# OpenDriveLab/kai0

Measured on AMD Instinct MI355X. Metric: train samples/sec pi0.5 full FT, higher is better.
Workload: dtype bf16; 1 GPU; pi0.5 full fine-tune bf16, batch 32 per MI355X, 3-cam 224x224 (BASELINE.json configs[1]); global_batch=32, seq_len=1018, parallelism=dp1

## Files before the change

### kai0_amd/csrc/gemm_bf16.hip

```cpp
#include "common.h"
#include "../../include/kai0hip.h"
#include <stdlib.h>
#include <algorithm>
#include <atomic>
#include <type_traits>

namespace {

constexpr int BK = 64;

#ifdef KAI0_ABLATE
#define KAI0_ABL(p) ((p).ablate)
#else
#define KAI0_ABL(p) 0
#endif

struct RowMap {
    int32_t rpb;
    int64_t bs, off;
    __device__ __forceinline__ int64_t operator()(int r) const {
        if (rpb == 0) return r;
        const int q = r / rpb;
        return (int64_t)q * bs + (r - q * rpb) + off;
    }
// ... 304 lines not shown
            if constexpr (A_KC) {
                off = kc_in ? a_off[j] + (uint32_t)k0 * 2 : OOB;
            } else {
                const int kr = k0 + (wave * NA + j) * A_RPP + lane / A_LPR;
                off = kr < kend ? a_off[j] + (uint32_t)p.amap(kr) * lda2 : OOB;
            }
            glds16(a_rsrc, off, sa + j * 1024);
        }
#pragma unroll
        for (int j = 0; j < NB; ++j) {
            uint32_t off;
            if constexpr (B_KC) {
                off = kc_in ? b_off[j] + (uint32_t)k0 * 2 : OOB;
            } else {
                const int kr = k0 + (wave * NB + j) * B_RPP + lane / B_LPR;
                off = kr < kend ? b_off[j] + (uint32_t)p.bmap(kr) * ldb2 : OOB;
            }
            glds16((B_KC && BK == 64 && pair && (((wave * NB + j) * KC_RPP) & 32)) ? b2_rsrc : b_rsrc, off, sb + j * 1024);
        }
    };

    auto piece_off = [&](int kt, int idx) -> uint32_t {
        const int k0 = kbeg + kt * BK;
        const bool kc_in = (k0 + kc_chunk) < kend;
        if (idx < NA) {
            if constexpr (A_KC) {
                return kc_in ? a_off[idx] + (uint32_t)k0 * 2 : OOB;
            } else {
                const int kr = k0 + (wave * NA + idx) * A_RPP + lane / A_LPR;
                return kr < kend ? a_off[idx] + (uint32_t)p.amap(kr) * lda2 : OOB;
            }
        } else {
            const int j = idx - NA;
            if constexpr (B_KC) {
                return kc_in ? b_off[j] + (uint32_t)k0 * 2 : OOB;
            } else {
                const int kr = k0 + (wave * NB + j) * B_RPP + lane / B_LPR;
                return kr < kend ? b_off[j] + (uint32_t)p.bmap(kr) * ldb2 : OOB;
            }
        }
    };
    auto piece_issue = [&](uint32_t off, int slot, int idx) {
        if (idx < NA) glds16(a_rsrc, off, smem + slot * STAGE + wave * (NA * 1024) + idx * 1024);
        else glds16(b_rsrc, off, smem + slot * STAGE + A_TILE + wave * (NB * 1024) + (idx - NA) * 1024);
    };

    const int l15 = lane & 15, g = lane >> 4;
    const int mc_keyv = (l15 >> 2) | ((g & 1) << 2);

    f32x4 acc[MT][NT];
#pragma unroll
    for (int i = 0; i < MT; ++i)
#pragma unroll
        for (int j = 0; j < NT; ++j) acc[i][j] = f32x4{0.f, 0.f, 0.f, 0.f};

    auto load_frag = [&](const char* tile, bool kc, int rowb, int col0, int ks) -> bf16x8 {
        if (kc) {
            const int row = col0 + l15;
            const int off = BK == 64 ? row * 128 + (((ks * 4 + g) ^ (row & 7)) << 4)
                                     : row * 64 + ((g ^ ((row & 8) ? 3 : 0)) << 4);
            return *reinterpret_cast<const bf16x8*>(tile + off);
        } else {
            const int chunk = (col0 >> 3) + ((l15 & 3) >> 1);
            const int sw = ((chunk ^ (mc_keyv << 1)) << 4) + (l15 & 1) * 8;
            const int r0 = ks * 32 + 8 * g + (l15 >> 2);
            bf16x4 lo = __builtin_amdgcn_ds_read_tr16_b64_v4bf16((LDS_PTR(bf16x4))(tile + r0 * rowb + sw));
            bf16x4 hi = __builtin_amdgcn_ds_read_tr16_b64_v4bf16((LDS_PTR(bf16x4))(tile + (r0 + 4) * rowb + sw));
            return __builtin_shufflevector(lo, hi, 0, 1, 2, 3, 4, 5, 6, 7);
        }
    };

    const int nk = (kend - kbeg + BK - 1) / BK;
    if constexpr (SCH == 3) {
        constexpr int NP = NA + NB;
        static_assert(NP == 4 && BK == 32, "ring schedule: 4 pieces per 32-deep sub-tile");
        const int grp = wm;
#pragma unroll
        for (int u = 0; u < 3; ++u)
#pragma unroll
            for (int pi = 0; pi < NP; ++pi) piece_issue(piece_off(u, pi), u, pi);
        asm volatile("s_waitcnt vmcnt(8)" ::: "memory");
        lds_barrier();
        if (grp == 1) lds_barrier();
        for (int u = 0; u < nk; ++u) {
            const int slot = u & 3, pslot = (u + 3) & 3;
            const char* ta = smem + slot * STAGE;
            const char* tb = ta + A_TILE;
            bf16x8 bfr[NT], af[MT];
#pragma unroll
            for (int t = 0; t < NT; ++t) bfr[t] = load_frag(tb, B_KC, B_ROWB, wn * (NT * 16) + t * 16, 0);
#pragma unroll
            for (int t = 0; t < MT; ++t) af[t] = load_frag(ta, A_KC, A_ROWB, wm * (MT * 16) + t * 16, 0);
            __builtin_amdgcn_sched_barrier(0);
            if (grp == 1) asm volatile("s_waitcnt vmcnt(4)" ::: "memory");
            lds_barrier();
            __builtin_amdgcn_s_setprio(1);
#pragma unroll
            for (int i = 0; i < MT; ++i) {
#pragma unroll
                for (int j = 0; j < NT; ++j)
                    acc[i][j] = __builtin_amdgcn_mfma_f32_16x16x32_bf16(af[i], bfr[j], acc[i][j], 0, 0, 0);
                if ((i & 1) == 0) {
                    __builtin_amdgcn_sched_barrier(0);
                    piece_issue(KAI0_ABL(p) == 1 ? OOB : piece_off(u + 3, i >> 1), pslot, i >> 1);
                    __builtin_amdgcn_sched_barrier(0);
                }
            }
            __builtin_amdgcn_s_setprio(0);
            if (grp == 0) asm volatile("s_waitcnt vmcnt(8)" ::: "memory");
            lds_barrier();
        }
        asm volatile("s_waitcnt vmcnt(0)" ::: "memory");
        if (grp == 0) lds_barrier();
        lds_barrier();
    } else if constexpr (SCH == 1) {
        const int grp = wm;
        uint32_t ha_off[4], hb_off[4];
        int ha_lds[4], hb_lds[4];
        int ha_kr[4], hb_kr[4];
#pragma unroll
        for (int h = 0; h < 2; ++h)
#pragma unroll
            for (int j = 0; j < 2; ++j) {
                const int q = 2 * wave + j, x = h * 2 + j;
                if constexpr (A_KC) {
                    const int ra = (q >> 3) * 128 + h * 64 + (q & 7) * 8, Ra = m0 + ra + (lane >> 3);
                    ha_lds[x] = ra * 128;
                    ha_kr[x] = 0;
                    ha_off[x] = Ra < p.M ? (uint32_t)((p.amap(Ra) * p.lda + kc_chunk) * 2) : OOB;
                } else {
                    const int r = q * 4 + (lane >> 4), key = (r & 3) | (((r >> 3) & 1) << 2);
                    const int col = m0 + h * 128 + (((lane & 15) ^ (key << 1)) * 8);
                    ha_lds[x] = h * 16384 + q * 1024;
                    ha_kr[x] = r;
                    ha_off[x] = col < p.M ? (uint32_t)(col * 2) : OOB;
                }
                if constexpr (B_KC) {
                    const int rb = (q >> 2) * 64 + h * 32 + (q & 3) * 8;
                    int Rb = n0 + rb + (lane >> 3);
                    bool ok = Rb < p.N;
                    if (pair) {
                        Rb = (n0 >> 1) + (q >> 2) * 32 + (q & 3) * 8 + (lane >> 3);
                        ok = Rb < (p.N >> 1);
                    }
                    hb_lds[x] = rb * 128;
                    hb_kr[x] = 0;
                    hb_off[x] = ok ? (uint32_t)((p.bmap(Rb) * p.ldb + kc_chunk) * 2) : OOB;
                } else {
                    const int r = q * 4 + (lane >> 4), key = (r & 3) | (((r >> 3) & 1) << 2);
                    const int col = n0 + h * 128 + (((lane & 15) ^ (key << 1)) * 8);
                    hb_lds[x] = h * 16384 + q * 1024;
                    hb_kr[x] = r;
                    hb_off[x] = col < p.N ? (uint32_t)(col * 2) : OOB;
                }
            }
        auto issue_half = [&](bool isb, int h, int t) {
            const int k0 = kbeg + t * BK;
            const bool kc_in = (k0 + kc_chunk) < kend;
            char* base = smem + (t & 1) * STAGE + (isb ? A_TILE : 0);
#pragma unroll
            for (int j = 0; j < 2; ++j) {
                const int x = h * 2 + j;
                const uint32_t o = isb ? hb_off[x] : ha_off[x];
                uint32_t off = OOB;
                if (isb ? B_KC : A_KC) {
                    if (kc_in && o != OOB) off = o + (uint32_t)k0 * 2;
                } else {
                    const int kr = k0 + (isb ? hb_kr[x] : ha_kr[x]);
                    if (kr < kend && o != OOB) off = o + (uint32_t)(isb ? p.bmap(kr) : p.amap(kr)) * (isb ? ldb2 : lda2);
                }
                if (KAI0_ABL(p) == 1) off = OOB;
                glds16(isb ? ((pair && h == 1) ? b2_rsrc : b_rsrc) : a_rsrc, off, base + (isb ? hb_lds[x] : ha_lds[x]));
            }
        };
        issue_half(false, 0, 0);
        issue_half(true, 1, 0);
        issue_half(true, 0, 0);
        issue_half(false, 1, 0);
        issue_half(false, 0, 1);
        issue_half(true, 1, 1);
        asm volatile("s_waitcnt vmcnt(6)" ::: "memory");
        lds_barrier();
        if (grp == 1) lds_barrier();
        bf16x8 af[4][2], bq[2][2];
        auto read_a = [&](const char* ta, int h) {
#pragma unroll
            for (int i = 0; i < 4; ++i)
#pragma unroll
                for (int ks = 0; ks < 2; ++ks)
                    af[i][ks] = A_KC ? load_frag(ta, true, A_ROWB, wm * 128 + (h * 4 + i) * 16, ks)
                                     : load_frag(ta + h * 16384, false, 256, wm * 64 + i * 16, ks);
        };
        auto read_b = [&](const char* tb, int h) {
#pragma unroll
            for (int j = 0; j < 2; ++j)
#pragma unroll
                for (int ks = 0; ks < 2; ++ks)
                    bq[j][ks] = B_KC ? load_frag(tb, true, B_ROWB, wn * 64 + (h * 2 + j) * 16, ks)
                                     : load_frag(tb + h * 16384, false, 256, wn * 32 + j * 16, ks);
        };
        auto quad = [&](auto ahc, auto bhc) {
            constexpr int ah = decltype(ahc)::value, bh = decltype(bhc)::value;
            __builtin_amdgcn_s_setprio(1);
#pragma unroll
            for (int ks = 0; ks < 2; ++ks)
#pragma unroll
                for (int i = 0; i < 4; ++i)
#pragma unroll
                    for (int j = 0; j < 2; ++j)
                        acc[ah * 4 + i][bh * 2 + j] =
                            __builtin_amdgcn_mfma_f32_16x16x32_bf16(af[i][ks], bq[j][ks], acc[ah * 4 + i][bh * 2 + j], 0, 0, 0);
            __builtin_amdgcn_s_setprio(0);
        };
        using I0 = std::integral_constant<int, 0>;
        using I1 = std::integral_constant<int, 1>;
        for (int t = 0; t < nk; ++t) {
            const char* ta = smem + (t & 1) * STAGE;
            const char* tb = ta + A_TILE;
            read_b(tb, 0);
            __builtin_amdgcn_sched_barrier(0);
            read_a(ta, 0);
            __builtin_amdgcn_sched_barrier(0);
            issue_half(true, 0, t + 1);
            lds_barrier();
            quad(I0{}, I0{});
            lds_barrier();
            read_b(tb, 1);
            __builtin_amdgcn_sched_barrier(0);
            issue_half(false, 1, t + 1);
            asm volatile("s_waitcnt vmcnt(8)" ::: "memory");
            lds_barrier();
            quad(I0{}, I1{});
            lds_barrier();
            read_a(ta, 1);
            __builtin_amdgcn_sched_barrier(0);
            issue_half(false, 0, t + 2);
            lds_barrier();
            quad(I1{}, I1{});
            lds_barrier();
            read_b(tb, 0);
            __builtin_amdgcn_sched_barrier(0);
            issue_half(true, 1, t + 2);
            asm volatile("s_waitcnt vmcnt(6)" ::: "memory");
            lds_barrier();
            quad(I1{}, I0{});
            lds_barrier();
        }
        asm volatile("s_waitcnt vmcnt(0)" ::: "memory");
        if (grp == 0) lds_barrier();
        lds_barrier();
    } else {
#pragma unroll
        for (int st = 0; st < NS - 1; ++st)
            if (st < nk) stage(st, st);
        int slot_c = 0, slot_p = NS - 1;
        for (int kt = 0; kt < nk; ++kt) {
            if constexpr (NS == 2) {
                asm volatile("s_waitcnt vmcnt(0)" ::: "memory");
            } else {
                if (kt + NS - 2 < nk) asm volatile("s_waitcnt vmcnt(%0)" ::"n"((NS - 2) * (NA + NB)) : "memory");
                else asm volatile("s_waitcnt vmcnt(0)" ::: "memory");
            }
            lds_barrier();
            if (kt + NS - 1 < nk && KAI0_ABL(p) != 1) stage(kt + NS - 1, slot_p);
            const char* ta = smem + slot_c * STAGE;
            const char* tb = ta + A_TILE;
    #pragma unroll
            for (int ks = 0; ks < BK / 32; ++ks) {
                bf16x8 bfr[NT];
    #pragma unroll
                for (int t = 0; t < NT; ++t) bfr[t] = load_frag(tb, B_KC, B_ROWB, wn * (NT * 16) + t * 16, ks);
    #pragma unroll
                for (int h = 0; h < MT / AH; ++h) {
                    bf16x8 af[AH];
    #pragma unroll
                    for (int t = 0; t < AH; ++t) af[t] = load_frag(ta, A_KC, A_ROWB, wm * (MT * 16) + (h * AH + t) * 16, ks);
    #pragma unroll
                    for (int i = 0; i < AH; ++i)
    #pragma unroll
                        for (int j = 0; j < NT; ++j)
                            acc[h * AH + i][j] = __builtin_amdgcn_mfma_f32_16x16x32_bf16(af[i], bfr[j], acc[h * AH + i][j], 0, 0, 0);
                }
            }
            slot_c = slot_c + 1 == NS ? 0 : slot_c + 1;
            slot_p = slot_p + 1 == NS ? 0 : slot_p + 1;
        }
        lds_barrier();
    }

    float* slab = reinterpret_cast<float*>(smem + wave * (AH * 4096));
    const int64_t cz = z1 * p.sC1 + z2 * p.sC2;
    const int64_t rz = z1 * p.sR1 + z2 * p.sR2;
    const int64_t vz = z1 * p.rv_s1 + z2 * p.rv_s2;
    constexpr bool ILM = SCH == 1 && !A_KC, ILN = SCH == 1 && !B_KC;
    const int ccol = ILN ? n0 + ((lane & 7) >> 2) * 128 + wn * 32 + ((lane & 7) & 3) * 8 : n0 + wn * 64 + (lane & 7) * 8;
    auto row_base = [&](int h) { return ILM ? m0 + h * 128 + wm * 64 : m0 + wm * (MT * 16) + h * 64; };
    const bool col_ok = ccol < ((p.N + 7) & ~7);
    const bool fused_fast = p.act >= 2 && p.split_k == 1 && p.bias == nullptr && p.gate == nullptr && p.residual == nullptr &&
                            !p.accumulate && !p.out_f32 && p.nseg == 0 && (p.act == 4 || p.scale == 1.0f) &&
                            (p.act != 3 || p.pre_out != nullptr);
    const bool plain_fast = p.act <= 1 && p.split_k == 1 && (p.bias != nullptr || p.residual != nullptr) && p.gate == nullptr &&
                            !p.accumulate && !p.out_f32 && p.nseg == 0 && (N_ALIGNED8(p.N));
    const bool simple_fast = MT == 8 && p.simple_epi && p.act <= 1 && p.split_k == 1 && p.gate == nullptr && !p.out_f32 && p.scale == 1.0f &&
                             p.cmap.rpb == 0 && (N_ALIGNED8(p.N));
    auto epi_half = [&](auto hc) {
        constexpr int h = decltype(hc)::value;
        if constexpr (((MT == 4 && WM == 2) || (MT == 2 && WM == 4)) && WN == 2 && A_KC && B_KC) if (p.act == 7) {
            const bool rot = n0 < p.rope_n_end;
            const int fi = ((n0 >> 7) & 1) * 64 + (lane & 7) * 8;
            const int rcol = rot ? (n0 >> 8) * 256 + wn * 128 + fi : n0 + wn * 64 + (lane & 7) * 8;
            const int rbase = row_base(h) + (lane >> 3);
            bf16x8 cs[AH * 2], sn[AH * 2];
#pragma unroll
            for (int it = 0; it < AH * 2; ++it) {
                const int64_t tr = (int64_t)min(rbase + it * 8, p.M - 1) * p.rope_half + fi;
                cs[it] = *reinterpret_cast<const bf16x8*>(p.rope_cos + (rot ? tr : 0));
                sn[it] = *reinterpret_cast<const bf16x8*>(p.rope_sin + (rot ? tr : 0));
            }
#pragma unroll
            for (int i = 0; i < AH; ++i)
#pragma unroll
                for (int j = 0; j < 4; ++j)
#pragma unroll
                    for (int r = 0; r < 4; ++r) slab[(i * 16 + 4 * g + r) * 64 + j * 16 + l15] = acc[i][j][r];
            lds_barrier();
            const float* pslab = reinterpret_cast<const float*>(smem + (wave ^ 1) * (AH * 4096));
            int si = 0;
            if (p.nseg > 1 && rcol >= p.seg_begin[1]) si = 1;
            if (p.nseg > 2 && rcol >= p.seg_begin[2]) si = 2;
            const bool rcol_ok = rcol < p.N;
#pragma unroll
            for (int it = 0; it < AH * 2; ++it) {
                const int lr = it * 8 + (lane >> 3);
                const int row = rbase + it * 8;
                const int so = lr * 64 + (lane & 7) * 8;
                const f32x4 v0 = *reinterpret_cast<const f32x4*>(slab + so), v1 = *reinterpret_cast<const f32x4*>(slab + so + 4);
                const f32x4 w0 = *reinterpret_cast<const f32x4*>(pslab + so), w1 = *reinterpret_cast<const f32x4*>(pslab + so + 4);
                if (row >= p.M || !rcol_ok) continue;
                const float x[8] = {v0[0], v0[1], v0[2], v0[3], v1[0], v1[1], v1[2], v1[3]};
                const float y[8] = {w0[0], w0[1], w0[2], w0[3], w1[0], w1[1], w1[2], w1[3]};
                bf16x8 ov;
#pragma unroll
                for (int e = 0; e < 8; ++e) {
                    const float xe = rbf(x[e]), ye = rbf(y[e]);
                    const float c = bf2f(cs[it][e]), sv = bf2f(sn[it][e]);
                    ov[e] = rot ? f2bf(rbf(xe * c) + rbf((wn == 0 ? -ye : ye) * sv)) : f2bf(xe);
                }
                const int64_t orow = p.cmap(row);
                bf16_t* cp = p.nseg > 0 ? p.seg_dst[si] + orow * p.seg_ld[si] + (rcol - p.seg_begin[si])
                                        : reinterpret_cast<bf16_t*>(p.C) + cz + orow * p.ldc + rcol;
                *reinterpret_cast<bf16x8*>(cp) = ov;
            }
            return;
        }
        if constexpr (MT != 2) if (pair) {
#pragma unroll
            for (int i = 0; i < 4; ++i)
#pragma unroll
                for (int j = 0; j < 4; ++j)
#pragma unroll
                    for (int r = 0; r < 4; ++r) slab[(i * 16 + 4 * g + r) * 64 + j * 16 + l15] = acc[h * 4 + i][j][r];
            asm volatile("s_waitcnt lgkmcnt(0)" ::: "memory");
            __builtin_amdgcn_wave_barrier();
            const int ocol = (n0 >> 1) + wn * 32 + (lane & 3) * 8;
            const bool ocol_ok = ocol < (p.N >> 1);
            bf16_t* cb = reinterpret_cast<bf16_t*>(p.C);
#pragma unroll
            for (int it = 0; it < 4; ++it) {
                const int lr = it * 16 + (lane >> 2);
                const int row = row_base(h) + lr;
                const float* sp = slab + lr * 64 + (lane & 3) * 8;
                const f32x4 g0 = *reinterpret_cast<const f32x4*>(sp), g1 = *reinterpret_cast<const f32x4*>(sp + 4);
                const f32x4 u0 = *reinterpret_cast<const f32x4*>(sp + 32), u1 = *reinterpret_cast<const f32x4*>(sp + 36);
                if (row >= p.M || !ocol_ok) continue;
                const float gv[8] = {g0[0], g0[1], g0[2], g0[3], g1[0], g1[1], g1[2], g1[3]};
                const float uv[8] = {u0[0], u0[1], u0[2], u0[3], u1[0], u1[1], u1[2], u1[3]};
                bf16x8 gb, ub, hb;
#pragma unroll
                for (int e = 0; e < 8; e += 2) {
                    const f32x2 gr = rbf2(f32x2{gv[e], gv[e + 1]}), ur = rbf2(f32x2{uv[e], uv[e + 1]});
                    const f32x2 hv = rbf2(gelu_tanh2(gr)) * ur;
                    gb[e] = f2bf(gr[0]);
                    gb[e + 1] = f2bf(gr[1]);
                    ub[e] = f2bf(ur[0]);
                    ub[e + 1] = f2bf(ur[1]);
                    hb[e] = f2bf(hv[0]);
                    hb[e + 1] = f2bf(hv[1]);
                }
                const int64_t o = cz + p.cmap(row) * p.ldc + ocol;
                *reinterpret_cast<bf16x8*>(cb + o) = hb;
                if (p.pre_out != nullptr) store_pre8(p.pre_out + o, gb, p.nt_pre);
                if (p.pre_out2 != nullptr) store_pre8(p.pre_out2 + o, ub, p.nt_pre);
            }
            asm volatile("s_waitcnt lgkmcnt(0)" ::: "memory");
            __builtin_amdgcn_wave_barrier();
            return;
        }
        if constexpr (MT != 2) if (fused_fast) {
            bf16x8 s0[8], s1[8];
            float ds[8];
            const int rbase = row_base(h) + (lane >> 3);
#pragma unroll
            for (int it = 0; it < 8; ++it) {
                const int row = rbase + it * 8;
                s0[it] = bf16x8{};
                s1[it] = bf16x8{};
                ds[it] = 0.f;
                if (row < p.M && col_ok) {
                    const int64_t o = cz + p.cmap(row) * p.ldc + ccol;
                    s0[it] = *reinterpret_cast<const bf16x8*>(p.aux1 + o);
                    if (p.act == 3) s1[it] = *reinterpret_cast<const bf16x8*>(p.aux2 + o);
                    if (p.act == 4) ds[it] = p.rowvec[vz + (int64_t)row * p.rv_ld];
                }
            }
#pragma unroll
            for (int i = 0; i < 4; ++i)
#pragma unroll
                for (int j = 0; j < 4; ++j)
#pragma unroll
                    for (int r = 0; r < 4; ++r) slab[(i * 16 + 4 * g + r) * 64 + j * 16 + l15] = acc[h * 4 + i][j][r];
            asm volatile("s_waitcnt lgkmcnt(0)" ::: "memory");
            __builtin_amdgcn_wave_barrier();
            bf16_t* cb = reinterpret_cast<bf16_t*>(p.C);
#pragma unroll
            for (int it = 0; it < 8; ++it) {
                const int row = rbase + it * 8;
                const float* sp = slab + (it * 8 + (lane >> 3)) * 64 + (lane & 7) * 8;
                const f32x4 v0 = *reinterpret_cast<const f32x4*>(sp);
                const f32x4 v1 = *reinterpret_cast<const f32x4*>(sp + 4);
                const float v[8] = {v0[0], v0[1], v0[2], v0[3], v1[0], v1[1], v1[2], v1[3]};
                if (row >= p.M || !col_ok) continue;
                const int64_t o = cz + p.cmap(row) * p.ldc + ccol;
                bf16x8 ov;
                if (p.act == 2) {
                    if (p.pre_out != nullptr) {
                        bf16x8 uv;
#pragma unroll
                        for (int e = 0; e < 8; ++e) uv[e] = f2bf(v[e]);
                        *reinterpret_cast<bf16x8*>(p.pre_out + o) = uv;
                    }
#pragma unroll
                    for (int e = 0; e < 8; e += 2) {
                        const f32x2 r = rbf2(gelu_tanh2(f32x2{bf2f(s0[it][e]), bf2f(s0[it][e + 1])})) * rbf2(f32x2{v[e], v[e + 1]});
                        ov[e] = f2bf(r[0]);
                        ov[e + 1] = f2bf(r[1]);
                    }
                } else if (p.act == 3) {
                    bf16x8 du;
#pragma unroll
                    for (int e = 0; e < 8; e += 2) {
                        const f32x2 dh = rbf2(f32x2{v[e], v[e + 1]});
                        f32x2 gl, gr;
                        gelu_tanh_both2(f32x2{bf2f(s0[it][e]), bf2f(s0[it][e + 1])}, gl, gr);
                        const f32x2 a = dh * rbf2(gl);
                        const f32x2 b = rbf2(dh * f32x2{bf2f(s1[it][e]), bf2f(s1[it][e + 1])}) * gr;
                        du[e] = f2bf(a[0]);
                        du[e + 1] = f2bf(a[1]);
                        ov[e] = f2bf(b[0]);
                        ov[e + 1] = f2bf(b[1]);
                    }
                    *reinterpret_cast<bf16x8*>(p.pre_out + o) = du;
                } else if (p.act == 5) {
#pragma unroll
                    for (int e = 0; e < 8; e += 2) {
                        f32x2 gl, gr;
                        gelu_tanh_both2(f32x2{bf2f(s0[it][e]), bf2f(s0[it][e + 1])}, gl, gr);
                        const f32x2 b = rbf2(f32x2{v[e], v[e + 1]}) * gr;
                        ov[e] = f2bf(b[0]);
                        ov[e + 1] = f2bf(b[1]);
                    }
                } else {
#pragma unroll
                    for (int e = 0; e < 8; ++e) ov[e] = f2bf((bf2f(s0[it][e]) * (v[e] - ds[it])) * p.scale);
                }
                *reinterpret_cast<bf16x8*>(cb + o) = ov;
            }
            asm volatile("s_waitcnt lgkmcnt(0)" ::: "memory");
            __builtin_amdgcn_wave_barrier();
            return;
        }
        if constexpr (MT <= 4) if (plain_fast) {
            float bv[8] = {0.f, 0.f, 0.f, 0.f, 0.f, 0.f, 0.f, 0.f};
            if (p.bias != nullptr && col_ok) {
                if (p.bias_f32) {
                    const f32x4 b0 = *reinterpret_cast<const f32x4*>(reinterpret_cast<const float*>(p.bias) + ccol);
                    const f32x4 b1 = *reinterpret_cast<const f32x4*>(reinterpret_cast<const float*>(p.bias) + ccol + 4);
#pragma unroll
                    for (int e = 0; e < 4; ++e) { bv[e] = b0[e]; bv[4 + e] = b1[e]; }
                } else {
                    const bf16x8 b = *reinterpret_cast<const bf16x8*>(reinterpret_cast<const bf16_t*>(p.bias) + ccol);
#pragma unroll
                    for (int e = 0; e < 8; ++e) bv[e] = bf2f(b[e]);
                }
            }
            bf16x8 rs[AH * 2];
            const int rbase = row_base(h) + (lane >> 3);
#pragma unroll
            for (int it = 0; it < AH * 2; ++it) {
                const int row = rbase + it * 8;
                rs[it] = bf16x8{};
                if (p.residual != nullptr && row < p.M && col_ok) rs[it] = *reinterpret_cast<const bf16x8*>(p.residual + rz + p.cmap(row) * p.ldr + ccol);
            }
#pragma unroll
            for (int i = 0; i < AH; ++i)
#pragma unroll
                for (int j = 0; j < 4; ++j)
#pragma unroll
                    for (int r = 0; r < 4; ++r) slab[(i * 16 + 4 * g + r) * 64 + j * 16 + l15] = acc[h * AH + i][j][r];
            asm volatile("s_waitcnt lgkmcnt(0)" ::: "memory");
            __builtin_amdgcn_wave_barrier();
            bf16_t* cb = reinterpret_cast<bf16_t*>(p.C);
#pragma unroll
            for (int it = 0; it < AH * 2; ++it) {
                const int row = rbase + it * 8;
                const float* sp = slab + (it * 8 + (lane >> 3)) * 64 + (lane & 7) * 8;
                const f32x4 v0 = *reinterpret_cast<const f32x4*>(sp);
                const f32x4 v1 = *reinterpret_cast<const f32x4*>(sp + 4);
                if (row >= p.M || !col_ok) continue;
                float v[8] = {v0[0], v0[1], v0[2], v0[3], v1[0], v1[1], v1[2], v1[3]};
                const int64_t o = cz + p.cmap(row) * p.ldc + ccol;
#pragma unroll
                for (int e = 0; e < 8; ++e) v[e] = rbf(v[e] + bv[e]);
                if (p.scale != 1.0f) {
#pragma unroll
                    for (int e = 0; e < 8; ++e) v[e] = rbf(v[e] * p.scale);
                }
                if (p.act == 1) {
                    if (p.pre_out != nullptr) {
                        bf16x8 pv;
#pragma unroll
                        for (int e = 0; e < 8; ++e) pv[e] = f2bf(v[e]);
                        store_pre8(p.pre_out + o, pv, p.nt_pre);
                    }
#pragma unroll
                    for (int e = 0; e < 8; e += 2) {
                        const f32x2 a = gelu_tanh2(f32x2{v[e], v[e + 1]});
                        v[e] = rbf(a[0]);
                        v[e + 1] = rbf(a[1]);
                    }
                }
                if (p.residual != nullptr) {
#pragma unroll
                    for (int e = 0; e < 8; ++e) v[e] = rbf(v[e] + bf2f(rs[it][e]));
                }
                bf16x8 ov;
#pragma unroll
                for (int e = 0; e < 8; ++e) ov[e] = f2bf(v[e]);
                *reinterpret_cast<bf16x8*>(cb + o) = ov;
            }
            asm volatile("s_waitcnt lgkmcnt(0)" ::: "memory");
            __builtin_amdgcn_wave_barrier();
            return;
        }
        if constexpr (MT == 8) if (simple_fast) {
            const bool has_bias = p.bias != nullptr, has_res = p.residual != nullptr, gelu = p.act == 1;
            const int M_ = p.M, nt_pre_ = p.nt_pre, nt_c_ = p.nt_c;
            const bf16_t* res_ = p.residual;
            bf16_t* pre_ = p.pre_out;
            const int64_t ldr_ = p.ldr, ldc_ = p.ldc;
            float bv[8] = {0.f, 0.f, 0.f, 0.f, 0.f, 0.f, 0.f, 0.f};
            if (has_bias && col_ok) {
                if (p.bias_f32) {
                    const f32x4 b0 = *reinterpret_cast<const f32x4*>(reinterpret_cast<const float*>(p.bias) + ccol);
                    const f32x4 b1 = *reinterpret_cast<const f32x4*>(reinterpret_cast<const float*>(p.bias) + ccol + 4);
#pragma unroll
                    for (int e = 0; e < 4; ++e) { bv[e] = b0[e]; bv[4 + e] = b1[e]; }
                } else {
                    const bf16x8 b = *reinterpret_cast<const bf16x8*>(reinterpret_cast<const bf16_t*>(p.bias) + ccol);
#pragma unroll
                    for (int e = 0; e < 8; ++e) bv[e] = bf2f(b[e]);
                }
            }
            bf16_t* cl = reinterpret_cast<bf16_t*>(p.C) + cz + ccol;
            int64_t ldl = p.ldc;
            if (p.nseg > 0) {
                cl = p.seg_dst[0] + (ccol - p.seg_begin[0]);
                ldl = p.seg_ld[0];
                if (p.nseg > 1 && ccol >= p.seg_begin[1]) {
                    cl = p.seg_dst[1] + (ccol - p.seg_begin[1]);
                    ldl = p.seg_ld[1];
                }
                if (p.nseg > 2 && ccol >= p.seg_begin[2]) {
                    cl = p.seg_dst[2] + (ccol - p.seg_begin[2]);
                    ldl = p.seg_ld[2];
                }
            }
            const int rbase = row_base(h) + (lane >> 3);
            auto res_row = [&](int it) -> bf16x8 {
                const int row = rbase + it * 8;
                return (has_res && row < M_ && col_ok) ? *reinterpret_cast<const bf16x8*>(res_ + rz + (int64_t)row * ldr_ + ccol) : bf16x8{};
            };
            const bool accum = p.accumulate != 0;
            auto old_row = [&](int it) -> bf16x8 {
                const int row = rbase + it * 8;
                return (accum && row < M_ && col_ok) ? *reinterpret_cast<const bf16x8*>(cl + (int64_t)row * ldl) : bf16x8{};
            };
            bf16x8 rnext = res_row(0), onext = old_row(0);
#pragma unroll
            for (int i = 0; i < 4; ++i)
#pragma unroll
                for (int j = 0; j < 4; ++j)
#pragma unroll
                    for (int r = 0; r < 4; ++r) slab[(i * 16 + 4 * g + r) * 64 + j * 16 + l15] = acc[h * 4 + i][j][r];
            asm volatile("s_waitcnt lgkmcnt(0)" ::: "memory");
            __builtin_amdgcn_wave_barrier();
#pragma unroll
            for (int it = 0; it < 8; ++it) {
                const int row = rbase + it * 8;
                const float* sp = slab + (it * 8 + (lane >> 3)) * 64 + (lane & 7) * 8;
                const f32x4 v0 = *reinterpret_cast<const f32x4*>(sp);
                const f32x4 v1 = *reinterpret_cast<const f32x4*>(sp + 4);
                const bf16x8 rv = rnext, ov0 = onext;
                if (it + 1 < 8) {
                    rnext = res_row(it + 1);
                    onext = old_row(it + 1);
                }
                if (row >= M_ || !col_ok) continue;
                float v[8] = {v0[0], v0[1], v0[2], v0[3], v1[0], v1[1], v1[2], v1[3]};
                if (has_bias) {
#pragma unroll
                    for (int e = 0; e < 8; ++e) v[e] += bv[e];
                }
#pragma unroll
                for (int e = 0; e < 8; ++e) v[e] = rbf(v[e]);
                if (gelu) {
                    if (pre_ != nullptr) {
                        bf16x8 pv;
#pragma unroll
                        for (int e = 0; e < 8; ++e) pv[e] = f2bf(v[e]);
                        store_pre8(pre_ + cz + (int64_t)row * ldc_ + ccol, pv, nt_pre_);
                    }
#pragma unroll
                    for (int e = 0; e < 8; e += 2) {
                        const f32x2 a = gelu_tanh2(f32x2{v[e], v[e + 1]});
                        v[e] = rbf(a[0]);
                        v[e + 1] = rbf(a[1]);
                    }
                }
                if (has_res) {
#pragma unroll
                    for (int e = 0; e < 8; ++e) v[e] = rbf(v[e] + bf2f(rv[e]));
                }
                if (accum) {
#pragma unroll
                    for (int e = 0; e < 8; ++e) v[e] += bf2f(ov0[e]);
                }
                bf16x8 ov;
#pragma unroll
                for (int e = 0; e < 8; ++e) ov[e] = f2bf(v[e]);
                store_pre8(cl + (int64_t)row * ldl, ov, nt_c_);
            }
            asm volatile("s_waitcnt lgkmcnt(0)" ::: "memory");
            __builtin_amdgcn_wave_barrier();
            return;
        }
#pragma unroll
        for (int i = 0; i < AH; ++i)
#pragma unroll
            for (int j = 0; j < 4; ++j)
#pragma unroll
                for (int r = 0; r < 4; ++r) slab[(i * 16 + 4 * g + r) * 64 + j * 16 + l15] = acc[h * AH + i][j][r];
        asm volatile("s_waitcnt lgkmcnt(0)" ::: "memory");
        __builtin_amdgcn_wave_barrier();
#pragma unroll 1
        for (int it = 0; it < AH * 2; ++it) {
            const int lr = it * 8 + (lane >> 3);
            const int row = row_base(h) + lr;
            if (row >= p.M || !col_ok) continue;
            const float* sp = slab + lr * 64 + (lane & 7) * 8;
            f32x4 v0 = *reinterpret_cast<const f32x4*>(sp);
            f32x4 v1 = *reinterpret_cast<const f32x4*>(sp + 4);
            float v[8] = {v0[0], v0[1], v0[2], v0[3], v1[0], v1[1], v1[2], v1[3]};
            if (p.split_k > 1) {
                float* wp = reinterpret_cast<float*>(p.ws) + ((int64_t)blockIdx.y * p.M + row) * p.N + ccol;
                *reinterpret_cast<f32x4*>(wp) = v0;
                *reinterpret_cast<f32x4*>(wp + 4) = v1;
            } else {
                epilogue8(p, v, row, ccol, cz, rz, vz, p.C, p.out_f32 != 0);
            }
        }
        asm volatile("s_waitcnt lgkmcnt(0)" ::: "memory");
        __builtin_amdgcn_wave_barrier();
    };
    epi_half(std::integral_constant<int, 0>{});
    if constexpr (MT / 4 > 1) epi_half(std::integral_constant<int, 1>{});
    if constexpr (MT / 4 > 2) epi_half(std::integral_constant<int, 2>{});
    static_assert(MT / 4 <= 3, "extend the epilogue parts");
}

constexpr int PS_SLOTS = 1024;
__device__ unsigned int g_ps_ctr[PS_SLOTS][16];

#ifdef KAI0_PS_TRACE
__device__ long long g_ps_trace[256][8];
#define PS_STAMP(i)                                              \
    do {                                                         \
        const long long n_ = __builtin_amdgcn_s_memrealtime();   \
        t_acc[i] += n_ - t_prev;                                 \
        t_prev = n_;                                             \
    } while (0)
#else
#define PS_STAMP(i) do { } while (0)
#endif

__global__ __launch_bounds__(512, 1) void gemm_nt_persistent_kernel(const GemmArgs p, unsigned int* __restrict__ ctr) {
    constexpr int TBM = 256, TBN = 256, A_TILE = TBM * BK * 2, STAGE = 2 * A_TILE, GROUP = 4, MT = 8;
    extern __shared__ __attribute__((aligned(16))) char smem[];
    const int tid = threadIdx.x, lane = tid & 63;
    const int wave = __builtin_amdgcn_readfirstlane(tid >> 6);
    const int wm = wave >> 2, wn = wave & 3, grp = wm;
    const int l15 = lane & 15, g = lane >> 4;
    int* mbox = reinterpret_cast<int*>(smem + 2 * STAGE);
    float* slab = reinterpret_cast<float*>(smem + 2 * STAGE + wave * 4096);
    const int ntile = p.tiles_m * p.tiles_n;
    const int qq = ntile >> 3, rr = ntile & 7;
    const int x0 = blockIdx.x & 7;
    auto draw = [&]() -> unsigned { return __hip_atomic_fetch_add(ctr + x0, 1u, __ATOMIC_RELAXED, __HIP_MEMORY_SCOPE_AGENT); };
    auto resolve = [&](unsigned t) -> int {
        for (int a = 0; a < 8; ++a) {
            const int x = (x0 + a) & 7;
            const int len = qq + (x < rr ? 1 : 0);
            if (a > 0) t = __hip_atomic_fetch_add(ctr + x, 1u, __ATOMIC_RELAXED, __HIP_MEMORY_SCOPE_AGENT);
            if ((int)t < len) return (x < rr ? x * (qq + 1) : rr * (qq + 1) + (x - rr) * qq) + (int)t;
        }
        return -1;
    };
    auto next_ticket = [&]() -> int { return resolve(draw()); };
    const __amdgpu_buffer_rsrc_t a_rsrc = __builtin_amdgcn_make_buffer_rsrc((void*)p.A, 0, (int)OOB, 0x00020000);
    const __amdgpu_buffer_rsrc_t b_rsrc = __builtin_amdgcn_make_buffer_rsrc((void*)p.B, 0, (int)OOB, 0x00020000);
    const bool pair = p.act == 6;
    const __amdgpu_buffer_rsrc_t b2_rsrc = __builtin_amdgcn_make_buffer_rsrc((void*)(pair ? p.B2 : p.B), 0, (int)OOB, 0x00020000);
    const int kc_chunk = ((lane & 7) ^ (lane >> 3)) * 8;
    const int nk = (p.K + BK - 1) / BK;

    const uint32_t lda2 = (uint32_t)p.lda * 2, ldb2 = (uint32_t)p.ldb * 2, kc2 = (uint32_t)kc_chunk * 2;
    auto arow_fix = [](int) -> uint32_t { return 0u; };
    int m0 = 0, n0 = 0;
    uint32_t ha_off[4], hb_off[4];
    int ha_lds[4], hb_lds[4];
#pragma unroll
    for (int h = 0; h < 2; ++h)
#pragma unroll
        for (int j = 0; j < 2; ++j) {
            const int q = 2 * wave + j, x = h * 2 + j;
            ha_lds[x] = ((q >> 3) * 128 + h * 64 + (q & 7) * 8) * 128;
            hb_lds[x] = ((q >> 2) * 64 + h * 32 + (q & 3) * 8) * 128;
        }
    auto setup = [&](int pid) {
        const int width = GROUP * p.tiles_n;
        const int group = pid / width, first_m = group * GROUP;
        const int gsz = min(p.tiles_m - first_m, GROUP);
        const int in_g = pid - group * width;
        m0 = (first_m + in_g % gsz) * TBM;
        n0 = (in_g / gsz) * TBN;
#pragma unroll
        for (int h = 0; h < 2; ++h)
#pragma unroll
            for (int j = 0; j < 2; ++j) {
                const int q = 2 * wave + j, x = h * 2 + j;
                const int Ra = m0 + (q >> 3) * 128 + h * 64 + (q & 7) * 8 + (lane >> 3);
                ha_off[x] = Ra < p.M ? (uint32_t)Ra * lda2 + kc2 + arow_fix(Ra) : OOB;
                int Rb = n0 + (q >> 2) * 64 + h * 32 + (q & 3) * 8 + (lane >> 3);
                bool ok = Rb < p.N;
                if (pair) {
                    Rb = (n0 >> 1) + (q >> 2) * 32 + (q & 3) * 8 + (lane >> 3);
                    ok = Rb < (p.N >> 1);
                }
                hb_off[x] = ok ? (uint32_t)Rb * ldb2 + kc2 : OOB;
            }
    };
    auto issue_half = [&](bool isb, int h, int t) {
        const int k0 = t * BK;
        const bool kc_in = (k0 + kc_chunk) < p.K;
        char* base = smem + (t & 1) * STAGE + (isb ? A_TILE : 0);
#pragma unroll
        for (int j = 0; j < 2; ++j) {
            const int x = h * 2 + j;
            const uint32_t o = isb ? hb_off[x] : ha_off[x];
            const uint32_t off = (kc_in && o != OOB) ? o + (uint32_t)k0 * 2 : OOB;
            glds16(isb ? ((pair && h == 1) ? b2_rsrc : b_rsrc) : a_rsrc, off, base + (isb ? hb_lds[x] : ha_lds[x]));
        }
    };
    auto prologue_issue = [&]() {
        issue_half(false, 0, 0);
        issue_half(true, 1, 0);
        issue_half(true, 0, 0);
        issue_half(false, 1, 0);
        issue_half(false, 0, 1);
        issue_half(true, 1, 1);
    };
    auto frag = [&](const char* tile, int row0, int ks) -> bf16x8 {
        const int row = row0 + l15;
        return *reinterpret_cast<const bf16x8*>(tile + row * 128 + (((ks * 4 + g) ^ (row & 7)) << 4));
    };

    if (tid == 0) {
        const int t0 = next_ticket();
        mbox[0] = t0;
        mbox[1] = t0 >= 0 ? next_ticket() : -1;
    }
    __syncthreads();
    int cur = mbox[0], nxt = mbox[1];
    __syncthreads();
    if (cur >= 0) {
        setup(cur);
        prologue_issue();
        asm volatile("s_waitcnt vmcnt(6)" ::: "memory");
        lds_barrier();
        if (grp == 1) lds_barrier();
    }
    const int64_t cz = 0, rz = 0, vz = 0;
#ifdef KAI0_PS_TRACE
    long long t_acc[5] = {0, 0, 0, 0, 0};
    long long t_prev = __builtin_amdgcn_s_memrealtime();
#endif
    while (cur >= 0) {
        f32x4 acc[MT][4];
#pragma unroll
        for (int i = 0; i < MT; ++i)
#pragma unroll
            for (int j = 0; j < 4; ++j) acc[i][j] = f32x4{0.f, 0.f, 0.f, 0.f};
        bf16x8 af[4][2], bq[2][2];
        auto read_a = [&](const char* ta, int h) {
#pragma unroll
            for (int i = 0; i < 4; ++i)
#pragma unroll
                for (int ks = 0; ks < 2; ++ks) af[i][ks] = frag(ta, wm * 128 + (h * 4 + i) * 16, ks);
        };
        auto read_b = [&](const char* tb, int h) {
#pragma unroll
            for (int j = 0; j < 2; ++j)
#pragma unroll
                for (int ks = 0; ks < 2; ++ks) bq[j][ks] = frag(tb, wn * 64 + (h * 2 + j) * 16, ks);
        };
        auto quad = [&](auto ahc, auto bhc) {
            constexpr int ah = decltype(ahc)::value, bh = decltype(bhc)::value;
            __builtin_amdgcn_s_setprio(1);
#pragma unroll
            for (int ks = 0; ks < 2; ++ks)
#pragma unroll
                for (int i = 0; i < 4; ++i)
#pragma unroll
                    for (int j = 0; j < 2; ++j)
                        acc[ah * 4 + i][bh * 2 + j] =
                            __builtin_amdgcn_mfma_f32_16x16x32_bf16(af[i][ks], bq[j][ks], acc[ah * 4 + i][bh * 2 + j], 0, 0, 0);
            __builtin_amdgcn_s_setprio(0);
        };
        using I0 = std::integral_constant<int, 0>;
        using I1 = std::integral_constant<int, 1>;
        PS_STAMP(0);
        for (int t = 0; t < nk; ++t) {
            const char* ta = smem + (t & 1) * STAGE;
            const char* tb = ta + A_TILE;
            read_b(tb, 0);
            __builtin_amdgcn_sched_barrier(0);
            read_a(ta, 0);
            __builtin_amdgcn_sched_barrier(0);
            issue_half(true, 0, t + 1);
            lds_barrier();
            quad(I0{}, I0{});
            lds_barrier();
            read_b(tb, 1);
            __builtin_amdgcn_sched_barrier(0);
            issue_half(false, 1, t + 1);
            asm volatile("s_waitcnt vmcnt(8)" ::: "memory");
            lds_barrier();
            quad(I0{}, I1{});
            lds_barrier();
            read_a(ta, 1);
            __builtin_amdgcn_sched_barrier(0);
            issue_half(false, 0, t + 2);
            lds_barrier();
            quad(I1{}, I1{});
            lds_barrier();
            read_b(tb, 0);
            __builtin_amdgcn_sched_barrier(0);
            issue_half(true, 1, t + 2);
            asm volatile("s_waitcnt vmcnt(6)" ::: "memory");
            lds_barrier();
            quad(I1{}, I0{});
            lds_barrier();
        }
        asm volatile("s_waitcnt vmcnt(0)" ::: "memory");
        if (grp == 0) lds_barrier();
        lds_barrier();

        PS_STAMP(1);
        const int m0c = m0, n0c = n0;
        int nn = -1;
        unsigned raw = 0;
        if (tid == 0 && nxt >= 0) raw = draw();
        if (nxt >= 0) {
            setup(nxt);
            prologue_issue();
        }
        const int ccol = n0c + wn * 64 + (lane & 7) * 8;
        const bool col_ok = ccol < ((p.N + 7) & ~7);
        const bool fused_fast = p.act >= 2 && p.act <= 5 && p.bias == nullptr && p.gate == nullptr && p.residual == nullptr && !p.accumulate &&
                                !p.out_f32 && p.nseg == 0 && (p.act == 4 || p.scale == 1.0f) && (p.act != 3 || p.pre_out != nullptr);
        const bool simple_fast = p.simple_epi && p.act <= 1 && p.split_k == 1 && p.gate == nullptr && !p.out_f32 && p.scale == 1.0f && p.cmap.rpb == 0 &&
                                 (N_ALIGNED8(p.N));
        auto to_slab = [&](int ti) {
            __builtin_amdgcn_wave_barrier();
#pragma unroll
            for (int j = 0; j < 4; ++j)
#pragma unroll
                for (int r = 0; r < 4; ++r) slab[(4 * g + r) * 64 + j * 16 + l15] = acc[ti][j][r];
            asm volatile("s_waitcnt lgkmcnt(0)" ::: "memory");
            __builtin_amdgcn_wave_barrier();
        };
        if (pair) {
            const int ocol = (n0c >> 1) + wn * 32 + (lane & 3) * 8;
            const bool ocol_ok = ocol < (p.N >> 1);
            bf16_t* cb = reinterpret_cast<bf16_t*>(p.C);
#pragma unroll
            for (int ti = 0; ti < MT; ++ti) {
                to_slab(ti);
                const int row = m0c + wm * 128 + ti * 16 + (lane >> 2);
                const float* sp = slab + (lane >> 2) * 64 + (lane & 3) * 8;
                const f32x4 g0 = *reinterpret_cast<const f32x4*>(sp), g1 = *reinterpret_cast<const f32x4*>(sp + 4);
                const f32x4 u0 = *reinterpret_cast<const f32x4*>(sp + 32), u1 = *reinterpret_cast<const f32x4*>(sp + 36);
                if (row < p.M && ocol_ok) {
                    const float gv[8] = {g0[0], g0[1], g0[2], g0[3], g1[0], g1[1], g1[2], g1[3]};
                    const float uv[8] = {u0[0], u0[1], u0[2], u0[3], u1[0], u1[1], u1[2], u1[3]};
                    bf16x8 gb, ub, hb;
#pragma unroll
                    for (int e = 0; e < 8; e += 2) {
                        const f32x2 gr = rbf2(f32x2{gv[e], gv[e + 1]}), ur = rbf2(f32x2{uv[e], uv[e + 1]});
                        const f32x2 hv = rbf2(gelu_tanh2(gr)) * ur;
                        gb[e] = f2bf(gr[0]); gb[e + 1] = f2bf(gr[1]);
                        ub[e] = f2bf(ur[0]); ub[e + 1] = f2bf(ur[1]);
                        hb[e] = f2bf(hv[0]); hb[e + 1] = f2bf(hv[1]);
                    }
                    const int64_t o = p.cmap(row) * p.ldc + ocol;
                    *reinterpret_cast<bf16x8*>(cb + o) = hb;
                    if (p.pre_out != nullptr) store_pre8(p.pre_out + o, gb, p.nt_pre);
                    if (p.pre_out2 != nullptr) store_pre8(p.pre_out2 + o, ub, p.nt_pre);
                }
            }
        } else if (fused_fast) {
            bf16_t* cb = reinterpret_cast<bf16_t*>(p.C);
#pragma unroll
            for (int h = 0; h < 2; ++h) {
                bf16x8 s0[8], s1[8];
                float ds[8];
                const int rbase = m0c + wm * 128 + h * 64 + (lane >> 3);
#pragma unroll
                for (int it = 0; it < 8; ++it) {
                    const int row = rbase + it * 8;
                    s0[it] = bf16x8{};
                    s1[it] = bf16x8{};
                    ds[it] = 0.f;
                    if (row < p.M && col_ok) {
                        const int64_t o = p.cmap(row) * p.ldc + ccol;
                        s0[it] = *reinterpret_cast<const bf16x8*>(p.aux1 + o);
                        if (p.act == 3) s1[it] = *reinterpret_cast<const bf16x8*>(p.aux2 + o);
                        if (p.act == 4) ds[it] = p.rowvec[(int64_t)row * p.rv_ld];
                    }
                }
#pragma unroll
                for (int i = 0; i < 4; ++i) {
                    to_slab(h * 4 + i);
#pragma unroll
                    for (int it2 = 0; it2 < 2; ++it2) {
                        const int it = 2 * i + it2;
                        const int row = rbase + it * 8;
                        const float* sp = slab + (it2 * 8 + (lane >> 3)) * 64 + (lane & 7) * 8;
                        const f32x4 v0 = *reinterpret_cast<const f32x4*>(sp), v1 = *reinterpret_cast<const f32x4*>(sp + 4);
                        const float v[8] = {v0[0], v0[1], v0[2], v0[3], v1[0], v1[1], v1[2], v1[3]};
                        if (row >= p.M || !col_ok) continue;
                        const int64_t o = p.cmap(row) * p.ldc + ccol;
                        bf16x8 ov;
                        if (p.act == 2) {
                            if (p.pre_out != nullptr) {
                                bf16x8 uv;
#pragma unroll
                                for (int e = 0; e < 8; ++e) uv[e] = f2bf(v[e]);
                                *reinterpret_cast<bf16x8*>(p.pre_out + o) = uv;
                            }
#pragma unroll
                            for (int e = 0; e < 8; e += 2) {
                                const f32x2 r = rbf2(gelu_tanh2(f32x2{bf2f(s0[it][e]), bf2f(s0[it][e + 1])})) * rbf2(f32x2{v[e], v[e + 1]});
                                ov[e] = f2bf(r[0]);
                                ov[e + 1] = f2bf(r[1]);
                            }
                        } else if (p.act == 3) {
                            bf16x8 du;
#pragma unroll
                            for (int e = 0; e < 8; e += 2) {
                                const f32x2 dh = rbf2(f32x2{v[e], v[e + 1]});
                                f32x2 gl, gr;
                                gelu_tanh_both2(f32x2{bf2f(s0[it][e]), bf2f(s0[it][e + 1])}, gl, gr);
                                const f32x2 a = dh * rbf2(gl);
                                const f32x2 b = rbf2(dh * f32x2{bf2f(s1[it][e]), bf2f(s1[it][e + 1])}) * gr;
                                du[e] = f2bf(a[0]); du[e + 1] = f2bf(a[1]);
                                ov[e] = f2bf(b[0]); ov[e + 1] = f2bf(b[1]);
                            }
                            *reinterpret_cast<bf16x8*>(p.pre_out + o) = du;
                        } else if (p.act == 5) {
#pragma unroll
                            for (int e = 0; e < 8; e += 2) {
                                f32x2 gl, gr;
                                gelu_tanh_both2(f32x2{bf2f(s0[it][e]), bf2f(s0[it][e + 1])}, gl, gr);
                                const f32x2 b = rbf2(f32x2{v[e], v[e + 1]}) * gr;
                                ov[e] = f2bf(b[0]); ov[e + 1] = f2bf(b[1]);
                            }
                        } else {
#pragma unroll
                            for (int e = 0; e < 8; ++e) ov[e] = f2bf((bf2f(s0[it][e]) * (v[e] - ds[it])) * p.scale);
                        }
                        *reinterpret_cast<bf16x8*>(cb + o) = ov;
                    }
                }
            }
        } else if (simple_fast) {
            const bool has_bias = p.bias != nullptr, has_res = p.residual != nullptr, gelu = p.act == 1;
            const int M_ = p.M, nt_pre_ = p.nt_pre, nt_c_ = p.nt_c;
            const bf16_t* res_ = p.residual;
            bf16_t* pre_ = p.pre_out;
            const int64_t ldr_ = p.ldr, ldc_ = p.ldc;
            float bv[8] = {0.f, 0.f, 0.f, 0.f, 0.f, 0.f, 0.f, 0.f};
            if (has_bias && col_ok) {
                if (p.bias_f32) {
                    const f32x4 b0 = *reinterpret_cast<const f32x4*>(reinterpret_cast<const float*>(p.bias) + ccol);
                    const f32x4 b1 = *reinterpret_cast<const f32x4*>(reinterpret_cast<const float*>(p.bias) + ccol + 4);
#pragma unroll
                    for (int e = 0; e < 4; ++e) { bv[e] = b0[e]; bv[4 + e] = b1[e]; }
                } else {
                    const bf16x8 b = *reinterpret_cast<const bf16x8*>(reinterpret_cast<const bf16_t*>(p.bias) + ccol);
#pragma unroll
                    for (int e = 0; e < 8; ++e) bv[e] = bf2f(b[e]);
                }
            }
            bf16_t* cl = reinterpret_cast<bf16_t*>(p.C) + ccol;
            int64_t ldl = p.ldc;
            if (p.nseg > 0) {
                cl = p.seg_dst[0] + (ccol - p.seg_begin[0]);
                ldl = p.seg_ld[0];
                if (p.nseg > 1 && ccol >= p.seg_begin[1]) {
                    cl = p.seg_dst[1] + (ccol - p.seg_begin[1]);
                    ldl = p.seg_ld[1];
                }
                if (p.nseg > 2 && ccol >= p.seg_begin[2]) {
                    cl = p.seg_dst[2] + (ccol - p.seg_begin[2]);
                    ldl = p.seg_ld[2];
                }
            }
            const int rbase = m0c + wm * 128 + (lane >> 3);
            auto res_row = [&](int k) -> bf16x8 {
                const int row = rbase + k * 8;
                return (has_res && row < M_ && col_ok) ? *reinterpret_cast<const bf16x8*>(res_ + (int64_t)row * ldr_ + ccol) : bf16x8{};
            };
            const bool accum = p.accumulate != 0;
            auto old_row = [&](int k) -> bf16x8 {
                const int row = rbase + k * 8;
                return (accum && row < M_ && col_ok) ? *reinterpret_cast<const bf16x8*>(cl + (int64_t)row * ldl) : bf16x8{};
            };
            bf16x8 rnext = res_row(0), onext = old_row(0);
#pragma unroll
            for (int ti = 0; ti < MT; ++ti) {
                to_slab(ti);
#pragma unroll
                for (int it2 = 0; it2 < 2; ++it2) {
                    const int k = ti * 2 + it2;
                    const int row = rbase + k * 8;
                    const float* sp = slab + (it2 * 8 + (lane >> 3)) * 64 + (lane & 7) * 8;
                    const f32x4 v0 = *reinterpret_cast<const f32x4*>(sp), v1 = *reinterpret_cast<const f32x4*>(sp + 4);
                    const bf16x8 rv = rnext, ov0 = onext;
                    if (k + 1 < 2 * MT) {
                        rnext = res_row(k + 1);
                        onext = old_row(k + 1);
                    }
                    if (row >= M_ || !col_ok) continue;
                    float v[8] = {v0[0], v0[1], v0[2], v0[3], v1[0], v1[1], v1[2], v1[3]};
                    if (has_bias) {
#pragma unroll
                        for (int e = 0; e < 8; ++e) v[e] += bv[e];
                    }
#pragma unroll
                    for (int e = 0; e < 8; ++e) v[e] = rbf(v[e]);
                    if (gelu) {
                        if (pre_ != nullptr) {
                            bf16x8 pv;
#pragma unroll
                            for (int e = 0; e < 8; ++e) pv[e] = f2bf(v[e]);
                            store_pre8(pre_ + (int64_t)row * ldc_ + ccol, pv, nt_pre_);
                        }
#pragma unroll
                        for (int e = 0; e < 8; e += 2) {
                            const f32x2 a = gelu_tanh2(f32x2{v[e], v[e + 1]});
                            v[e] = rbf(a[0]);
                            v[e + 1] = rbf(a[1]);
                        }
                    }
                    if (has_res) {
#pragma unroll
                        for (int e = 0; e < 8; ++e) v[e] = rbf(v[e] + bf2f(rv[e]));
                    }
                    if (accum) {
#pragma unroll
                        for (int e = 0; e < 8; ++e) v[e] += bf2f(ov0[e]);
                    }
                    bf16x8 ov;
#pragma unroll
                    for (int e = 0; e < 8; ++e) ov[e] = f2bf(v[e]);
                    store_pre8(cl + (int64_t)row * ldl, ov, nt_c_);
                }
            }
        } else {
#pragma unroll
            for (int ti = 0; ti < MT; ++ti) {
                to_slab(ti);
#pragma unroll 1
                for (int it2 = 0; it2 < 2; ++it2) {
                    const int lr = it2 * 8 + (lane >> 3);
                    const int row = m0c + wm * 128 + ti * 16 + lr;
                    if (row >= p.M || !col_ok) continue;
                    const float* sp = slab + lr * 64 + (lane & 7) * 8;
                    const f32x4 v0 = *reinterpret_cast<const f32x4*>(sp), v1 = *reinterpret_cast<const f32x4*>(sp + 4);
                    float v[8] = {v0[0], v0[1], v0[2], v0[3], v1[0], v1[1], v1[2], v1[3]};
                    epilogue8(p, v, row, ccol, cz, rz, vz, p.C, p.out_f32 != 0);
                }
            }
        }
        PS_STAMP(2);
        __builtin_amdgcn_wave_barrier();
        if (tid == 0) mbox[0] = nxt >= 0 ? resolve(raw) : -1;
        asm volatile("s_waitcnt vmcnt(0)" ::: "memory");
        lds_barrier();
        nn = mbox[0];
        cur = nxt;
        nxt = nn;
        lds_barrier();
        if (cur >= 0 && grp == 1) lds_barrier();
        PS_STAMP(3);
#ifdef KAI0_PS_TRACE
        t_acc[4] += 1;
#endif
    }
#ifdef KAI0_PS_TRACE
    if (tid == 0 && blockIdx.x < 256)
        for (int i = 0; i < 5; ++i) g_ps_trace[blockIdx.x][i] = t_acc[i];
#endif
    if (tid == 0) {
        __builtin_amdgcn_fence(__ATOMIC_RELEASE, "agent");
        const unsigned done = __hip_atomic_fetch_add(ctr + 8, 1u, __ATOMIC_RELAXED, __HIP_MEMORY_SCOPE_AGENT);
        if (done == gridDim.x - 1) {
#pragma unroll
            for (int i = 0; i < 9; ++i) __hip_atomic_store(ctr + i, 0u, __ATOMIC_RELAXED, __HIP_MEMORY_SCOPE_AGENT);
        }
    }
}

__global__ __launch_bounds__(256) void splitk_reduce_kernel(const GemmArgs p) {
    const int z = blockIdx.y;
    const int z1 = z / p.batch_inner, z2 = z - z1 * p.batch_inner;
    const int n8 = (p.N + 7) >> 3;
    const int64_t total = (int64_t)p.M * n8;
    const float* w0 = p.ws + (int64_t)z * p.split_k * p.M * p.N;
    const int64_t cz = z1 * p.sC1 + z2 * p.sC2, rz = z1 * p.sR1 + z2 * p.sR2, vz = z1 * p.rv_s1 + z2 * p.rv_s2;
    for (int64_t i = (int64_t)blockIdx.x * 256 + threadIdx.x; i < total; i += (int64_t)gridDim.x * 256) {
        const int row = (int)(i / n8);
        const int col = (int)(i - (int64_t)row * n8) * 8;
        float acc[8] = {0.f, 0.f, 0.f, 0.f, 0.f, 0.f, 0.f, 0.f};
        bf16x8 rpre = {};
        const bool has_res = p.residual != nullptr && p.act != 4;
        if (has_res) rpre = *reinterpret_cast<const bf16x8*>(p.residual + rz + p.cmap(row) * p.ldr + col);
        if (p.split_k <= 8) {
            f32x4 a[8], b[8];
#pragma unroll
            for (int sp = 0; sp < 8; ++sp) {
                const float* wp = w0 + ((int64_t)min(sp, p.split_k - 1) * p.M + row) * p.N + col;
                a[sp] = *reinterpret_cast<const f32x4*>(wp);
                b[sp] = *reinterpret_cast<const f32x4*>(wp + 4);
            }
#pragma unroll
            for (int sp = 0; sp < 8; ++sp) {
                const float m = sp < p.split_k ? 1.0f : 0.0f;
                acc[0] += m * a[sp][0]; acc[1] += m * a[sp][1]; acc[2] += m * a[sp][2]; acc[3] += m * a[sp][3];
                acc[4] += m * b[sp][0]; acc[5] += m * b[sp][1]; acc[6] += m * b[sp][2]; acc[7] += m * b[sp][3];
            }
        } else
        for (int sp = 0; sp < p.split_k; ++sp) {
            const float* wp = w0 + ((int64_t)sp * p.M + row) * p.N + col;
            f32x4 a = *reinterpret_cast<const f32x4*>(wp);
            f32x4 b = *reinterpret_cast<const f32x4*>(wp + 4);
            acc[0] += a[0]; acc[1] += a[1]; acc[2] += a[2]; acc[3] += a[3];
            acc[4] += b[0]; acc[5] += b[1]; acc[6] += b[2]; acc[7] += b[3];
        }
        epilogue8(p, acc, row, col, cz, rz, vz, p.C, p.out_f32 != 0, has_res ? &rpre : nullptr);
    }
}

template <int KIND>
__global__ __launch_bounds__(256) void splitk_reduce_norm_kernel(const GemmArgs p) {
    __shared__ float red[4];
    const int row = blockIdx.x;
    const int n8 = p.N >> 3;
    const bool live = (int)threadIdx.x < n8;
    const int col = min((int)threadIdx.x, n8 - 1) * 8;
    float wv[8], bv[8];
    if constexpr (KIND == 1) {
        const f32x4 w0 = *reinterpret_cast<const f32x4*>(reinterpret_cast<const float*>(p.norm_w) + col);
        const f32x4 w1 = *reinterpret_cast<const f32x4*>(reinterpret_cast<const float*>(p.norm_w) + col + 4);
#pragma unroll
        for (int e = 0; e < 4; ++e) { wv[e] = w0[e]; wv[4 + e] = w1[e]; bv[e] = bv[4 + e] = 0.f; }
    } else {
        const bf16x8 w8 = *reinterpret_cast<const bf16x8*>(reinterpret_cast<const bf16_t*>(p.norm_w) + col);
        const bf16x8 b8 = *reinterpret_cast<const bf16x8*>(p.norm_b + col);
#pragma unroll
        for (int e = 0; e < 8; ++e) { wv[e] = bf2f(w8[e]); bv[e] = bf2f(b8[e]); }
    }
    bf16x8 rpre = {};
    const bool has_res = p.residual != nullptr;
    if (has_res) rpre = *reinterpret_cast<const bf16x8*>(p.residual + p.cmap(row) * p.ldr + col);
    float acc[8] = {0.f, 0.f, 0.f, 0.f, 0.f, 0.f, 0.f, 0.f};
    if (p.split_k <= 8) {
        f32x4 a[8], b[8];
#pragma unroll
        for (int sp = 0; sp < 8; ++sp) {
            const float* wp = p.ws + ((int64_t)min(sp, p.split_k - 1) * p.M + row) * p.N + col;
            a[sp] = *reinterpret_cast<const f32x4*>(wp);
            b[sp] = *reinterpret_cast<const f32x4*>(wp + 4);
        }
#pragma unroll
        for (int sp = 0; sp < 8; ++sp) {
            const float m = sp < p.split_k ? 1.0f : 0.0f;
            acc[0] += m * a[sp][0]; acc[1] += m * a[sp][1]; acc[2] += m * a[sp][2]; acc[3] += m * a[sp][3];
            acc[4] += m * b[sp][0]; acc[5] += m * b[sp][1]; acc[6] += m * b[sp][2]; acc[7] += m * b[sp][3];
        }
    } else {
        for (int sp = 0; sp < p.split_k; ++sp) {
            const float* wp = p.ws + ((int64_t)sp * p.M + row) * p.N + col;
            const f32x4 a = *reinterpret_cast<const f32x4*>(wp), b = *reinterpret_cast<const f32x4*>(wp + 4);
            acc[0] += a[0]; acc[1] += a[1]; acc[2] += a[2]; acc[3] += a[3];
            acc[4] += b[0]; acc[5] += b[1]; acc[6] += b[2]; acc[7] += b[3];
        }
    }
    if (live) epilogue8(p, acc, row, col, 0, 0, 0, p.C, false, has_res ? &rpre : nullptr);
    float x[8];
#pragma unroll
    for (int e = 0; e < 8; ++e) x[e] = live ? rbf(acc[e]) : 0.f;
    float y[8];
    if constexpr (KIND == 1) {
        float ss = 0.f;
#pragma unroll
        for (int e = 0; e < 8; ++e) ss += x[e] * x[e];
        const float rstd = rsqrtf(block_sum<4>(ss, red) / (float)p.N + p.norm_eps);
#pragma unroll
        for (int e = 0; e < 8; ++e) y[e] = (x[e] * rstd) * (1.0f + wv[e]);
    } else {
        float sm = 0.f;
#pragma unroll
        for (int e = 0; e < 8; ++e) sm += x[e];
        const float mean = block_sum<4>(sm, red) / (float)p.N;
        float vs = 0.f;
#pragma unroll
        for (int e = 0; e < 8; ++e) {
            const float d = x[e] - mean;
            vs += live ? d * d : 0.f;
        }
        const float rstd = rsqrtf(block_sum<4>(vs, red) / (float)p.N + p.norm_eps);
#pragma unroll
        for (int e = 0; e < 8; ++e) y[e] = (x[e] - mean) * rstd * wv[e] + bv[e];
    }
    if (live) {
        bf16x8 o;
#pragma unroll
        for (int e = 0; e < 8; ++e) o[e] = f2bf(y[e]);
        *reinterpret_cast<bf16x8*>(p.norm_out + (int64_t)row * p.N + col) = o;
    }
}

constexpr int layout_bit(bool a_kc, bool b_kc) { return 1 << (2 * a_kc + b_kc); }
constexpr int L_NT = layout_bit(true, true), L_NN = layout_bit(true, false), L_TT = layout_bit(false, true), L_TN = layout_bit(false, false);
constexpr int L_ALL = L_NT | L_NN | L_TT | L_TN;

template <int LAYOUTS, int WM, int WN, int MT, int NT, bool PP, int NS = 2, int BKT = 64, int SCH = 0>
int launch_cfg(const kai0_gemm_desc* d, GemmArgs& p, int batch, hipStream_t s) {
    constexpr int TBM = WM * MT * 16, TBN = WN * NT * 16;
    constexpr int LDS = NS * (TBM + TBN) * BKT * 2;
    p.tiles_m = (d->M + TBM - 1) / TBM;
    p.tiles_n = (p.N + TBN - 1) / TBN;
    dim3 grid(p.tiles_m * p.tiles_n, batch * p.split_k, 1), block(WM * WN * 64, 1, 1);
#define KAI0_LAUNCH(AK, BK_)                                                                                      \
    if constexpr ((LAYOUTS & layout_bit(AK, BK_)) != 0)                                                          \
        if ((d->a_kc != 0) == AK && (d->b_kc != 0) == BK_) {                                                      \
            static bool attr_set = false;                                                                         \
            auto kern = gemm_bf16_kernel<AK, BK_, WM, WN, MT, NT, PP, NS, BKT, SCH>;                              \
            if (!attr_set) {                                                                                      \
                hipError_t e = hipFuncSetAttribute((const void*)kern, hipFuncAttributeMaxDynamicSharedMemorySize, LDS); \
                if (e != hipSuccess) {                                                                            \
                    kai0_set_error("kai0_gemm_bf16: cannot reserve %d B of LDS: %s", LDS, hipGetErrorString(e));  \
                    return -2;                                                                                    \
                }                                                                                                 \
                attr_set = true;                                                                                  \
            }                                                                                                     \
            hipLaunchKernelGGL(kern, grid, block, LDS, s, p);                                                     \
            return 0;                                                                                             \
        }
    KAI0_LAUNCH(true, true)
    KAI0_LAUNCH(true, false)
    KAI0_LAUNCH(false, true)
    KAI0_LAUNCH(false, false)
#undef KAI0_LAUNCH
    kai0_set_error("kai0_gemm_bf16: the %d x %d tile configuration (%d waves, %d stages) is not built for a_kc=%d b_kc=%d", TBM, TBN,
                   WM * WN, NS, d->a_kc, d->b_kc);
    return -3;
}

}

#ifdef KAI0_PS_TRACE
KAI0_API int kai0_debug_ps_trace(long long* host_out) {
    return (int)hipMemcpyFromSymbol(host_out, HIP_SYMBOL(g_ps_trace), sizeof(long long) * 256 * 8);
}
#endif

KAI0_API int kai0_gemm_bf16(const kai0_gemm_desc* d, kai0_stream_t stream) {
    KAI0_REQUIRE(d != nullptr, "kai0_gemm_bf16: null descriptor");
    KAI0_REQUIRE(d->M > 0 && d->N > 0 && d->K > 0, "kai0_gemm_bf16: empty problem M=%d N=%d K=%d", d->M, d->N,
                 d->K);
    KAI0_REQUIRE(d->A && d->B && d->C, "kai0_gemm_bf16: null operand");
    KAI0_REQUIRE((d->lda % 8) == 0 && (d->ldb % 8) == 0 && (d->ldc % 8) == 0,
                 "kai0_gemm_bf16: leading dims must be multiples of 8 (lda=%lld ldb=%lld ldc=%lld)",
                 (long long)d->lda, (long long)d->ldb, (long long)d->ldc);
    KAI0_REQUIRE((d->N % 8) == 0 || (d->b_kc && d->ldc >= ((d->N + 7) & ~7) && !d->bias && !d->gate && !d->residual &&
                                     !d->pre_out && !d->accumulate),
                 "kai0_gemm_bf16: N=%d not a multiple of 8 needs b_kc, padded C rows and a plain epilogue", d->N);
    KAI0_REQUIRE((d->K % 8) == 0 || (!d->a_kc && !d->b_kc), "kai0_gemm_bf16: K=%d must be a multiple of 8 for "
                 "K-contiguous operands", d->K);
    KAI0_REQUIRE(d->a_kc || (d->M % 8) == 0, "kai0_gemm_bf16: M=%d must be a multiple of 8 when A is [K][M]",
                 d->M);
    KAI0_REQUIRE(((uintptr_t)d->A % 16) == 0 && ((uintptr_t)d->B % 16) == 0 && ((uintptr_t)d->C % 16) == 0,
                 "kai0_gemm_bf16: operands must be 16-byte aligned");
    KAI0_REQUIRE(d->batch <= 1 || (((d->sA1 | d->sA2 | d->sB1 | d->sB2) & 7) == 0 && ((d->sC1 | d->sC2) & (d->out_f32 ? 3 : 7)) == 0),
                 "kai0_gemm_bf16: batch strides must be multiples of 8 elements (16 B)");
    KAI0_REQUIRE(d->gate == nullptr || d->gate_rpb > 0, "kai0_gemm_bf16: gate needs gate_rpb > 0");
    KAI0_REQUIRE(d->act >= 0 && d->act <= 7, "kai0_gemm_bf16: unknown act %d", d->act);
    KAI0_REQUIRE(d->persist >= 0 && d->persist <= 2 && d->small_w8 >= 0 && d->small_w8 <= 2 && d->general_epilogue >= 0 &&
                     d->general_epilogue <= 1,
                 "kai0_gemm_bf16: hook out of range (persist=%d, small_w8=%d: 0..2; general_epilogue=%d: 0..1)", d->persist, d->small_w8,
                 d->general_epilogue);
    KAI0_REQUIRE(d->act != 7 || (d->rope_cos && d->rope_sin && d->rope_half == 128 && d->rope_n_end > 0 && (d->rope_n_end % 256) == 0 &&
                                 d->rope_n_end <= d->N && (d->N % 128) == 0 && d->a_kc && d->b_kc && d->batch <= 1 && d->split_k <= 1 &&
                                 !d->out_f32 && !d->accumulate && !d->bias && !d->gate && !d->residual && !d->pre_out &&
                                 (d->scale == 0.0f || d->scale == 1.0f) && d->b_rpb == 0 && ((uintptr_t)d->rope_cos % 16) == 0 &&
                                 ((uintptr_t)d->rope_sin % 16) == 0),
                 "kai0_gemm_bf16: act=7 (RoPE epilogue) needs bf16 cos / sin tables [M][128], rope_n_end %% 256 == 0, N %% 128 == 0, K-contiguous "
                 "operands, one batch entry, no split-K, a plain bf16 output");
    KAI0_REQUIRE(d->act != 6 || (d->B2 && d->a_kc && d->b_kc && d->batch <= 1 && d->split_k <= 1 && !d->out_f32 && !d->accumulate &&
                                 d->nseg == 0 && !d->bias && !d->gate && !d->residual && (d->scale == 0.0f || d->scale == 1.0f) &&
                                 (d->N % 32) == 0 && d->b_rpb == 0 && ((uintptr_t)d->B2 % 16) == 0),
                 "kai0_gemm_bf16: act=6 (GeGLU pair) needs B2 = up weight, K-contiguous operands, N %% 32 == 0, one batch entry, a "
                 "plain bf16 output");
    KAI0_REQUIRE(d->norm_kind == 0 ||
                     ((d->norm_kind == 1 || d->norm_kind == 2) && d->split_k > 1 && d->norm_out && d->norm_w && (d->norm_kind == 1 || d->norm_b) &&
                      d->batch <= 1 && !d->out_f32 && d->nseg == 0 && (d->N % 8) == 0 && d->N <= 2048 && d->act == 0 && !d->gate &&
                      !d->rowvec && ((uintptr_t)d->norm_out % 16) == 0 && ((uintptr_t)d->norm_w % 16) == 0),
                 "kai0_gemm_bf16: a fused norm (norm_kind=%d) needs split_k > 1, norm_out / norm_w (/ norm_b), one batch entry, a plain "
                 "bf16 output with N %% 8 == 0, N <= 2048, no activation / gate", d->norm_kind);
    KAI0_REQUIRE(d->act != 5 || (d->aux1 && !d->out_f32 && !d->accumulate && d->nseg == 0 && (d->N % 8) == 0),
                 "kai0_gemm_bf16: act=5 (fused GELU backward) needs aux1 = pre-activation, plain bf16 output");
    KAI0_REQUIRE(d->act != 4 || (d->aux1 && d->rowvec && !d->out_f32 && !d->accumulate && d->nseg == 0 && (d->N % 8) == 0),
                 "kai0_gemm_bf16: act=4 (fused softmax backward) needs aux1 = P, rowvec = D, plain bf16 output");
    KAI0_REQUIRE(d->act < 2 || d->act >= 4 || ((d->pre_out || d->act == 2) && d->aux1 && (d->act == 2 || d->aux2) && !d->out_f32 && (d->N % 8) == 0),
                 "kai0_gemm_bf16: act=%d (fused GeGLU) needs pre_out and aux inputs, bf16 output", d->act);
    KAI0_REQUIRE(d->nseg >= 0 && d->nseg <= 3, "kai0_gemm_bf16: nseg=%d", d->nseg);
    if (d->nseg > 0) {
        KAI0_REQUIRE(!d->out_f32 && !d->accumulate && (d->batch <= 1) && (d->act < 2 || d->act == 7) && !d->pre_out && (d->N % 8) == 0,
                     "kai0_gemm_bf16: column segments need a plain bf16 epilogue, batch 1");
        KAI0_REQUIRE(d->act != 4, "kai0_gemm_bf16: column segments and act=4 are exclusive");
        for (int i = 0; i < d->nseg; ++i)
            KAI0_REQUIRE(d->seg[i].dst && (d->seg[i].ld % 8) == 0 && (d->seg[i].n_begin % 8) == 0 &&
                             ((uintptr_t)d->seg[i].dst % 16) == 0 && d->seg[i].n_begin == (i ? d->seg[i].n_begin : 0) &&
                             (i == 0 || d->seg[i].n_begin > d->seg[i - 1].n_begin),
                         "kai0_gemm_bf16: segment %d (dst, ld %% 8, ascending n_begin %% 8, first at 0)", i);
    }
    {
        const int64_t a_rows = d->a_rpb ? ((int64_t)((d->a_kc ? d->M : d->K) / d->a_rpb) + 1) * d->a_bs + d->a_off
                                        : (d->a_kc ? d->M : d->K);
        const int64_t b_rows = d->b_rpb ? ((int64_t)((d->b_kc ? d->N : d->K) / d->b_rpb) + 1) * d->b_bs + d->b_off
                                        : (d->b_kc ? d->N : d->K);
        KAI0_REQUIRE(a_rows * d->lda * 2 < (int64_t)0x7FFF0000 && b_rows * d->ldb * 2 < (int64_t)0x7FFF0000,
                     "kai0_gemm_bf16: an operand spans more than 2 GiB per batch entry (A %lld rows, B %lld rows)",
                     (long long)a_rows, (long long)b_rows);
    }
    const int batch = d->batch > 0 ? d->batch : 1;
    GemmArgs p;
    p.A = (const bf16_t*)d->A;
    p.B = (const bf16_t*)d->B;
    p.C = d->C;
    p.M = d->M; p.N = d->act == 6 ? 2 * d->N : d->N; p.K = d->K;
    p.B2 = (const bf16_t*)d->B2;
    p.pre_out2 = (bf16_t*)d->pre_out2;
    p.norm_out = (bf16_t*)d->norm_out;
    p.norm_w = d->norm_w;
    p.norm_b = (const bf16_t*)d->norm_b;
    p.norm_eps = d->norm_eps;
    p.norm_kind = d->norm_kind;
    p.rope_cos = (const bf16_t*)d->rope_cos;
    p.rope_sin = (const bf16_t*)d->rope_sin;
    p.rope_half = d->rope_half;
    p.rope_n_end = d->rope_n_end;
    p.lda = d->lda; p.ldb = d->ldb; p.ldc = d->ldc;
    p.batch_inner = d->batch_inner > 0 ? d->batch_inner : 1;
    p.sA1 = d->sA1; p.sA2 = d->sA2; p.sB1 = d->sB1; p.sB2 = d->sB2; p.sC1 = d->sC1; p.sC2 = d->sC2;
    p.amap = RowMap{d->a_rpb, d->a_bs, d->a_off};
    p.bmap = RowMap{d->b_rpb, d->b_bs, d->b_off};
// ... 97 lines not shown
```

### kai0_amd/model.py

```python

from __future__ import annotations

import dataclasses

import contextlib
import os

import logging
import math

import torch
from torch import nn

from . import _lib, ops
from .config import Pi0Config, SiglipConfig, get_config
from .preprocessing import IMAGE_KEYS, preprocess_observation

BF16, F32 = torch.bfloat16, torch.float32
INT_MAX = 2**31 - 1
logger = logging.getLogger("kai0_amd")


class Linear(nn.Module):

    def __init__(self, in_features: int, out_features: int, bias: bool = True):
        super().__init__()
        self.in_features, self.out_features = in_features, out_features
        self.weight = nn.Parameter(torch.empty(out_features, in_features))
        self.bias = nn.Parameter(torch.empty(out_features)) if bias else None
        nn.init.normal_(self.weight, std=0.02)
        if bias:
            nn.init.zeros_(self.bias)


class Embedding(nn.Module):
    def __init__(self, num: int, dim: int):
        super().__init__()
        self.weight = nn.Parameter(torch.empty(num, dim))
        nn.init.normal_(self.weight, std=0.02)


class Conv2dParams(nn.Module):
    def __init__(self, cin: int, cout: int, k: int):
        super().__init__()
        self.weight = nn.Parameter(torch.empty(cout, cin, k, k))
        self.bias = nn.Parameter(torch.zeros(cout))
        nn.init.normal_(self.weight, std=0.02)


class LayerNormParams(nn.Module):
    def __init__(self, dim: int, eps: float):
        super().__init__()
        self.eps = eps
        self.weight = nn.Parameter(torch.ones(dim))
        self.bias = nn.Parameter(torch.zeros(dim))


class GemmaRMSNorm(nn.Module):

    def __init__(self, dim: int, eps: float = 1e-6, cond_dim: int | None = None):
        super().__init__()
        self.eps, self.dim, self.cond_dim = eps, dim, cond_dim
        if cond_dim is not None:
            self.dense = Linear(cond_dim, dim * 3, bias=True)
            nn.init.zeros_(self.dense.weight)
        else:
            self.weight = nn.Parameter(torch.zeros(dim))
            self.dense = None


class GemmaMLP(nn.Module):
    def __init__(self, width: int, mlp_dim: int):
        super().__init__()
        self.gate_proj = Linear(width, mlp_dim, bias=False)
        self.up_proj = Linear(width, mlp_dim, bias=False)
        self.down_proj = Linear(mlp_dim, width, bias=False)


class GemmaAttention(nn.Module):
    def __init__(self, cfg):
        super().__init__()
        self.head_dim = cfg.head_dim
        self.num_heads = cfg.num_heads
        self.num_key_value_groups = cfg.num_heads // cfg.num_kv_heads
        self.scaling = cfg.head_dim**-0.5
        self.q_proj = Linear(cfg.width, cfg.num_heads * cfg.head_dim, bias=False)
        self.k_proj = Linear(cfg.width, cfg.num_kv_heads * cfg.head_dim, bias=False)
        self.v_proj = Linear(cfg.width, cfg.num_kv_heads * cfg.head_dim, bias=False)
        self.o_proj = Linear(cfg.num_heads * cfg.head_dim, cfg.width, bias=False)


class GemmaDecoderLayer(nn.Module):
    def __init__(self, cfg, cond_dim):
        super().__init__()
        self.self_attn = GemmaAttention(cfg)
        self.mlp = GemmaMLP(cfg.width, cfg.mlp_dim)
        self.input_layernorm = GemmaRMSNorm(cfg.width, cond_dim=cond_dim)
        self.post_attention_layernorm = GemmaRMSNorm(cfg.width, cond_dim=cond_dim)


class GemmaModel(nn.Module):
    def __init__(self, cfg, vocab: int, use_adarms: bool, with_embed: bool):
        super().__init__()
        self.cfg = cfg
        cond_dim = cfg.width if use_adarms else None
        self.embed_tokens = Embedding(vocab, cfg.width) if with_embed else None
        self.layers = nn.ModuleList([GemmaDecoderLayer(cfg, cond_dim) for _ in range(cfg.depth)])
        self.norm = GemmaRMSNorm(cfg.width, cond_dim=cond_dim)
        self.gradient_checkpointing = False
        hd = cfg.head_dim
        inv = 1.0 / (10000.0 ** (torch.arange(0, hd, 2, dtype=torch.int64).to(dtype=torch.float) / hd))
        self.register_buffer("inv_freq", inv, persistent=False)

    def rope_inv_freq(self) -> torch.Tensor:
        return self.inv_freq.to(torch.float32).contiguous()


class GemmaForCausalLM(nn.Module):
    def __init__(self, cfg, vocab: int, use_adarms: bool):
        super().__init__()
        self.model = GemmaModel(cfg, vocab, use_adarms, with_embed=False)
        self.lm_head = Linear(cfg.width, vocab, bias=False)


class SiglipVisionEmbeddings(nn.Module):
    def __init__(self, c: SiglipConfig):
        super().__init__()
        self.patch_size = c.patch_size
        self.patch_embedding = Conv2dParams(3, c.hidden_size, c.patch_size)
        self.num_patches = (c.image_size // c.patch_size) ** 2
        self.position_embedding = Embedding(self.num_patches, c.hidden_size)


class SiglipAttention(nn.Module):
    def __init__(self, c: SiglipConfig):
        super().__init__()
        self.num_heads = c.num_heads
        self.head_dim = c.hidden_size // c.num_heads
        self.k_proj = Linear(c.hidden_size, c.hidden_size)
        self.v_proj = Linear(c.hidden_size, c.hidden_size)
        self.q_proj = Linear(c.hidden_size, c.hidden_size)
        self.out_proj = Linear(c.hidden_size, c.hidden_size)


class SiglipMLP(nn.Module):
    def __init__(self, c: SiglipConfig):
        super().__init__()
        self.fc1 = Linear(c.hidden_size, c.intermediate_size)
        self.fc2 = Linear(c.intermediate_size, c.hidden_size)


class SiglipEncoderLayer(nn.Module):
    def __init__(self, c: SiglipConfig):
        super().__init__()
        self.layer_norm1 = LayerNormParams(c.hidden_size, c.layer_norm_eps)
        self.self_attn = SiglipAttention(c)
        self.layer_norm2 = LayerNormParams(c.hidden_size, c.layer_norm_eps)
        self.mlp = SiglipMLP(c)


class SiglipEncoder(nn.Module):
    def __init__(self, c: SiglipConfig):
        super().__init__()
        self.layers = nn.ModuleList([SiglipEncoderLayer(c) for _ in range(c.num_layers)])


class SiglipVisionTransformer(nn.Module):
    def __init__(self, c: SiglipConfig):
        super().__init__()
        self.embeddings = SiglipVisionEmbeddings(c)
        self.encoder = SiglipEncoder(c)
        self.post_layernorm = LayerNormParams(c.hidden_size, c.layer_norm_eps)


class SiglipVisionModel(nn.Module):
    def __init__(self, c: SiglipConfig):
        super().__init__()
        self.vision_model = SiglipVisionTransformer(c)
        self.gradient_checkpointing = False


class PaliGemmaMultiModalProjector(nn.Module):
    def __init__(self, c: SiglipConfig):
        super().__init__()
        self.linear = Linear(c.hidden_size, c.projection_dim, bias=True)


class PaliGemmaModel(nn.Module):
    def __init__(self, cfg, vocab: int, sc: SiglipConfig):
        super().__init__()
        self.vision_tower = SiglipVisionModel(sc)
        self.multi_modal_projector = PaliGemmaMultiModalProjector(sc)
        self.language_model = GemmaModel(cfg, vocab, use_adarms=False, with_embed=True)


class PaliGemmaForConditionalGeneration(nn.Module):
    def __init__(self, cfg, vocab: int, sc: SiglipConfig):
        super().__init__()
        self.model = PaliGemmaModel(cfg, vocab, sc)
        self.lm_head = Linear(cfg.width, vocab, bias=False)
        self.lm_head.weight = self.model.language_model.embed_tokens.weight

    @property
    def language_model(self):
        return self.model.language_model

    @property
    def vision_tower(self):
        return self.model.vision_tower


KEEP_F32_SELECTORS = (
    "vision_tower.vision_model.embeddings.patch_embedding.weight",
    "vision_tower.vision_model.embeddings.patch_embedding.bias",
    "vision_tower.vision_model.embeddings.position_embedding.weight",
    "input_layernorm",
    "post_attention_layernorm",
    "model.norm",
)


def _lin(x, mod: Linear, residual=None, act=0):
    return ops.linear(x, mod.weight, mod.bias, residual, act)


def build_mask_codes(pad_masks: torch.Tensor, att_masks: torch.Tensor):
    cum = torch.cumsum(att_masks.to(torch.int32), dim=1)
    pad = pad_masks.to(torch.bool)
    qcode = torch.where(pad, cum, torch.full_like(cum, -1)).to(torch.int32).contiguous()
    kcode = torch.where(pad, cum, torch.full_like(cum, INT_MAX)).to(torch.int32).contiguous()
    pos = (torch.cumsum(pad.to(torch.int32), dim=1) - 1).to(torch.int32).contiguous()
    return qcode, kcode, pos


_EXPERT_STREAM = os.environ.get("KAI0_EXPERT_STREAM", "1") != "0"
_SKIP_DEAD_PREFIX = True


def set_expert_stream(on: bool) -> bool:
    global _EXPERT_STREAM
    old, _EXPERT_STREAM = _EXPERT_STREAM, bool(on)
    return old


def set_skip_dead_prefix(on: bool) -> bool:
    global _SKIP_DEAD_PREFIX
    old, _SKIP_DEAD_PREFIX = _SKIP_DEAD_PREFIX, bool(on)
    return old


class _NoUnitHooks:

    def pre_forward(self, unit: str) -> bool:
        return False

    def post_forward(self, unit: str, *tensors):
        return tensors


class PaliGemmaWithExpertModel(nn.Module):

    def __init__(self, vlm_config, action_expert_config, use_adarms=None, precision: str = "bfloat16",
                 vocab: int = 257_152, siglip: SiglipConfig | None = None):
        super().__init__()
        if use_adarms is None:
            use_adarms = [False, False]
        if use_adarms[0]:
            raise NotImplementedError("adaRMS on the PaliGemma tower is not part of pi0.5")
        self.vlm_cfg, self.exp_cfg = vlm_config, action_expert_config
        self.siglip_cfg = siglip or SiglipConfig()
        if self.siglip_cfg.projection_dim != vlm_config.width:
            self.siglip_cfg = dataclasses.replace(self.siglip_cfg, projection_dim=vlm_config.width)
        self.paligemma = PaliGemmaForConditionalGeneration(vlm_config, vocab, self.siglip_cfg)
        self.gemma_expert = GemmaForCausalLM(action_expert_config, vocab, use_adarms[1])
        self.remat = False
        self.unit_hooks = _NoUnitHooks()
        self.to_bfloat16_for_selected_params(precision)

    def to_bfloat16_for_selected_params(self, precision: str = "bfloat16"):
        if precision == "bfloat16":
            self.to(dtype=BF16)
        elif precision == "float32":
            self.to(dtype=F32)
            return
        else:
            raise ValueError(f"Invalid precision: {precision}")
        for name, param in self.named_parameters():
            if any(sel in name for sel in KEEP_F32_SELECTORS):
                param.data = param.data.to(dtype=F32)

    def embed_image(self, image: torch.Tensor) -> torch.Tensor:
        n = image.shape[0]
        vt = self.paligemma.model.vision_tower.vision_model
        sc = self.siglip_cfg
        S = vt.embeddings.num_patches
        NH, HD = sc.num_heads, sc.hidden_size // sc.num_heads
        emb = vt.embeddings
        hk = self.unit_hooks
        hk.pre_forward("siglip.embed")
        x = ops.patch_embed(image.contiguous(), emb.patch_embedding.weight, emb.patch_embedding.bias,
                            emb.position_embedding.weight, sc.patch_size)
        (x,) = hk.post_forward("siglip.embed", x)

        def layer_fn(x, layer):
            x, h = ops.layernorm_res(x, layer.layer_norm1.weight, layer.layer_norm1.bias, layer.layer_norm1.eps)
            at = layer.self_attn
            q, k, v = ops.linear_multi(h, [at.q_proj.weight, at.k_proj.weight, at.v_proj.weight],
                                       [at.q_proj.bias, at.k_proj.bias, at.v_proj.bias])
            a = ops.siglip_attention(q, k, v, n, S, NH, HD)
            x = _lin(a, at.out_proj, residual=x)
            x, h = ops.layernorm_res(x, layer.layer_norm2.weight, layer.layer_norm2.bias, layer.layer_norm2.eps)
            m = layer.mlp
            return ops.gelu_mlp(h, m.fc1.weight, m.fc1.bias, m.fc2.weight, m.fc2.bias, residual=x)

        for l, layer in enumerate(vt.encoder.layers):
            hk.pre_forward(f"siglip.{l}")
            x = self._maybe_remat(layer_fn, x, layer)
            (x,) = hk.post_forward(f"siglip.{l}", x)
        hk.pre_forward("prefix")
        x = ops.layernorm(x, vt.post_layernorm.weight, vt.post_layernorm.bias, vt.post_layernorm.eps)
        x = _lin(x, self.paligemma.model.multi_modal_projector.linear)
        return x.view(n, S, -1)

    def embed_language_tokens(self, tokens: torch.Tensor) -> torch.Tensor:
        table = self.paligemma.model.language_model.embed_tokens.weight
        return ops.embed(table, tokens, 1.0).view(*tokens.shape, -1)

    def _maybe_remat(self, fn, *args):
        if self.remat and self.training and torch.is_grad_enabled():
            return torch.utils.checkpoint.checkpoint(fn, *args, use_reentrant=False, preserve_rng_state=False)
        return fn(*args)

    def forward_joint(self, prefix: torch.Tensor, suffix: torch.Tensor, qcode, kcode, pos, cond: torch.Tensor,
                      B: int, P: int, Hs: int) -> torch.Tensor:
        lm, ex = self.paligemma.model.language_model, self.gemma_expert.model
        cfg = self.vlm_cfg
        H, HD = cfg.num_heads, cfg.head_dim
        inv_freq = lm.rope_inv_freq()

        dual = (_EXPERT_STREAM and prefix.is_cuda and not (self.remat and self.training)
                and getattr(self.unit_hooks, "mode", "zero2") != "fsdp")
        main = torch.cuda.current_stream() if dual else None
        side = ops.side_stream(prefix.device) if dual else None

        def on_side():
            return torch.cuda.stream(side) if dual else contextlib.nullcontext()

        def hand(ts, to):
            if dual:
                for t in ts:
                    t.record_stream(to)

        n_layers = len(lm.layers)

        def layer_fn(xp, xs, lp, le, last=False):
            ap, ae = lp.self_attn, le.self_attn
            with on_side():
                mod1 = ops.linear_f32(cond, le.input_layernorm.dense.weight, le.input_layernorm.dense.bias)
                xs, hs, gate1 = ops.adarms_res(xs, mod1, Hs, le.input_layernorm.eps)
                qkv_s = ops.linear_multi(hs, [ae.q_proj.weight, ae.k_proj.weight, ae.v_proj.weight])
            xp, hp = ops.rmsnorm_res(xp, lp.input_layernorm.weight, lp.input_layernorm.eps)
            qkv_p = ops.linear_multi(hp, [ap.q_proj.weight, ap.k_proj.weight, ap.v_proj.weight])
            if dual:
                main.wait_stream(side)
                hand(qkv_s, main)
            att_p, att_s = ops.joint_attention(pos, qcode, kcode, inv_freq, H, HD, (P, Hs), (*qkv_p, *qkv_s))
            if dual:
                side.wait_stream(main)
                hand((att_s,), side)
            with on_side():
                xs = ops.gated_residual(xs, _lin(att_s, ae.o_proj), gate1, Hs)
                mod2 = ops.linear_f32(cond, le.post_attention_layernorm.dense.weight, le.post_attention_layernorm.dense.bias)
                xs, hs, gate2 = ops.adarms_res(xs, mod2, Hs, le.post_attention_layernorm.eps)
                ys = ops.geglu_mlp(hs, le.mlp.gate_proj.weight, le.mlp.up_proj.weight, le.mlp.down_proj.weight)
                xs = ops.gated_residual(xs, ys, gate2, Hs)
            if last and _SKIP_DEAD_PREFIX:
                return xp, xs
            xp = _lin(att_p, ap.o_proj, residual=xp)
            xp, hp = ops.rmsnorm_res(xp, lp.post_attention_layernorm.weight, lp.post_attention_layernorm.eps)
            xp = ops.geglu_mlp(hp, lp.mlp.gate_proj.weight, lp.mlp.up_proj.weight, lp.mlp.down_proj.weight, residual=xp)
            return xp, xs

        xp, xs = prefix, suffix
        hk = self.unit_hooks
        if dual:
            side.wait_stream(main)
            hand((xs, cond), side)
        for l, (lp, le) in enumerate(zip(lm.layers, ex.layers, strict=True)):
            gathered = hk.pre_forward(f"joint.{l}")
            if dual and gathered:
                side.wait_stream(main)
            xp, xs = self._maybe_remat(layer_fn, xp, xs, lp, le, l == n_layers - 1)
            xp, xs = hk.post_forward(f"joint.{l}", xp, xs)
        hk.pre_forward("head")
        if dual:
            main.wait_stream(side)
            hand((xs,), main)
        modf = ops.linear_f32(cond, ex.norm.dense.weight, ex.norm.dense.bias)
        out, _ = ops.adarms(xs, modf, Hs, ex.norm.eps)
        return out


class PI0Pytorch(nn.Module):

    def __init__(self, config: Pi0Config):
        super().__init__()
        self.config = config
        self.pi05 = config.pi05
        if not self.pi05:
            raise NotImplementedError("only the pi0.5 branch (pi05=True) is on the hot path")
        vlm = get_config(config.paligemma_variant)
        exp = get_config(config.action_expert_variant)
        siglip = getattr(config, "siglip", None) or SiglipConfig()
        self.paligemma_with_expert = PaliGemmaWithExpertModel(
            vlm, exp, use_adarms=[False, True], precision=config.dtype, vocab=getattr(config, "vocab_size", 257_152),
            siglip=siglip,
        )
        self.action_in_proj = Linear(config.action_dim, exp.width)
        self.action_out_proj = Linear(exp.width, config.action_dim)
        self.time_mlp_in = Linear(exp.width, exp.width)
        self.time_mlp_out = Linear(exp.width, exp.width)
        self.gradient_checkpointing_enabled = False
        self.train_augmentation = True
        self.trim_prompt_padding = False
        self.trim_prompt_padding_infer = False
        self.trim_prompt_granule_infer = 64
        self._engine = None

    _ENGINE_SLOTS = 4

    @property
    def _engine(self):
        return self.__dict__.get("_engine_cur")

    @_engine.setter
    def _engine(self, eng):
        if eng is None:
            self.__dict__["_engine_lru"] = {}
        self.__dict__["_engine_cur"] = eng

    def invalidate_inference_engine(self):
        self._engine = None

    def inference_is_stale(self) -> bool:
        eng = self._engine
        return eng is not None and eng.stale()

    def train(self, mode: bool = True):
        if mode:
            self._engine = None
        return super().train(mode)

    def _apply(self, fn, recurse=True):
        self._engine = None
        return super()._apply(fn, recurse)

    def load_state_dict(self, *args, **kwargs):
        self._engine = None
        return super().load_state_dict(*args, **kwargs)

    def sharding_units(self):
        pe = self.paligemma_with_expert
        vt = pe.paligemma.model.vision_tower.vision_model
        lm, ex = pe.paligemma.model.language_model, pe.gemma_expert.model
        units = [("siglip.embed", list(vt.embeddings.parameters()))]
        def siglip_layer(layer):
            at = layer.self_attn
            first = [at.q_proj.weight, at.k_proj.weight, at.v_proj.weight, at.q_proj.bias, at.k_proj.bias, at.v_proj.bias]
            ids = {id(p) for p in first}
            return first + [p for p in layer.parameters() if id(p) not in ids]

        units += [(f"siglip.{l}", siglip_layer(layer)) for l, layer in enumerate(vt.encoder.layers)]
        units.append(("prefix", [*vt.post_layernorm.parameters(), *pe.paligemma.model.multi_modal_projector.parameters(),
                                 lm.embed_tokens.weight, *self.action_in_proj.parameters(), *self.time_mlp_in.parameters(),
                                 *self.time_mlp_out.parameters()]))
        units += [(f"joint.{l}", [*lp.parameters(), *le.parameters()]) for l, (lp, le) in enumerate(zip(lm.layers, ex.layers))]
        taken = {id(p) for _, ps in units for p in ps}
        dead = pe.gemma_expert.lm_head.weight
        units.append(("head", [p for p in self.parameters() if id(p) not in taken and p is not dead]))
        return units

    def set_unit_hooks(self, hooks):
        self.paligemma_with_expert.unit_hooks = hooks if hooks is not None else _NoUnitHooks()

    def gradient_checkpointing_enable(self):
        self.gradient_checkpointing_enabled = True
        self.paligemma_with_expert.remat = True
        pe = self.paligemma_with_expert
        pe.paligemma.model.language_model.gradient_checkpointing = True
        pe.paligemma.model.vision_tower.gradient_checkpointing = True
        pe.gemma_expert.model.gradient_checkpointing = True
        logger.info("Enabled gradient checkpointing for PI0Pytorch model")

    def gradient_checkpointing_disable(self):
        self.gradient_checkpointing_enabled = False
        self.paligemma_with_expert.remat = False
        pe = self.paligemma_with_expert
        pe.paligemma.model.language_model.gradient_checkpointing = False
        pe.paligemma.model.vision_tower.gradient_checkpointing = False
        pe.gemma_expert.model.gradient_checkpointing = False

    def is_gradient_checkpointing_enabled(self):
        return self.gradient_checkpointing_enabled

    def sample_noise(self, shape, device):
        return torch.normal(mean=0.0, std=1.0, size=shape, dtype=F32, device=device)

    def sample_time(self, bsize, device):
        a = torch.as_tensor(1.5, dtype=F32, device=device)
        b = torch.as_tensor(1.0, dtype=F32, device=device)
        t = torch.distributions.Beta(a, b).sample((bsize,))
        return (t * 0.999 + 0.001).to(dtype=F32, device=device)

    def _preprocess_observation(self, observation, *, train=True):
        res = self.paligemma_with_expert.siglip_cfg.image_size
        obs = preprocess_observation(observation, train=train, image_resolution=(res, res))
        return (list(obs.images.values()), list(obs.image_masks.values()), obs.tokenized_prompt,
                obs.tokenized_prompt_mask, obs.state)

    @staticmethod
    def _trim_prompt(lang_tokens, lang_masks, granule: int = 8):
        m = lang_masks.to(torch.bool)
        T = m.shape[1]
        idx = torch.arange(1, T + 1, device=m.device, dtype=torch.int32)
        last = int((m * idx).max().item()) if m.numel() else 0
        keep = min(T, max(granule, (last + granule - 1) // granule * granule))
        if keep == T:
            return lang_tokens, lang_masks
        return lang_tokens[:, :keep].contiguous(), lang_masks[:, :keep].contiguous()

    def embed_prefix(self, images, img_masks, lang_tokens, lang_masks):
        pe = self.paligemma_with_expert
        B = lang_tokens.shape[0]
        ncam = len(images)
        feats = pe.embed_image(torch.cat(images, dim=0))
        n_img = feats.shape[1]
        D = feats.shape[2]
        lang = ops.embed(pe.paligemma.model.language_model.embed_tokens.weight, lang_tokens, ops.sqrt_scale(D))
        T = lang_tokens.shape[1]
        P = ncam * n_img + T
        embs = PrefixAssembleFn.apply(feats.reshape(ncam * B * n_img, D), lang, B, ncam, n_img, T)
        pad = torch.cat([m[:, None].expand(B, n_img) for m in img_masks] + [lang_masks.to(torch.bool)], dim=1)
        att = torch.zeros((B, P), dtype=torch.bool, device=pad.device)
        return embs.view(B, P, D), pad, att

    def embed_suffix(self, state, noisy_actions, timestep):
        B, Hs, A = noisy_actions.shape
        De = self.action_in_proj.out_features
        te = torch.empty((B, De), dtype=F32, device=noisy_actions.device)
        _lib.call("kai0_time_sincos", timestep.contiguous().data_ptr(), te.data_ptr(), B, De, 4e-3, 4.0, ops._stream())
        x = ops.silu_f32(ops.linear_f32(te, self.time_mlp_in.weight, self.time_mlp_in.bias))
        cond = ops.silu_f32(ops.linear_f32(x, self.time_mlp_out.weight, self.time_mlp_out.bias))
        a = ops.linear_f32(noisy_actions.reshape(B * Hs, A).contiguous(), self.action_in_proj.weight, self.action_in_proj.bias)
        pad = torch.ones((B, Hs), dtype=torch.bool, device=a.device)
        att = torch.zeros((B, Hs), dtype=torch.bool, device=a.device)
        att[:, 0] = True
        return a.view(B, Hs, De), pad, att, cond

    def _trunk(self, images, img_masks, lang_tokens, lang_masks, state, actions, noise, time, x_t=None):
        u_t = None
        if x_t is None:
            actions = actions.to(F32).contiguous()
            x_t, u_t = ops.flow_mix(noise.to(F32).contiguous(), actions, time.to(F32).contiguous())
        else:
            x_t = x_t.to(F32).contiguous()
        if self.trim_prompt_padding:
            lang_tokens, lang_masks = self._trim_prompt(lang_tokens, lang_masks)
        prefix, ppad, patt = self.embed_prefix(images, img_masks, lang_tokens, lang_masks)
        suffix, spad, satt, cond = self.embed_suffix(state, x_t, time)
        prefix, suffix, cond = self.paligemma_with_expert.unit_hooks.post_forward("prefix", prefix, suffix, cond)
        B, P, Dp = prefix.shape
        Hs, De = suffix.shape[1], suffix.shape[2]
        qcode, kcode, pos = build_mask_codes(torch.cat([ppad, spad], dim=1), torch.cat([patt, satt], dim=1))
        suffix_bf = ops.cast_ag(suffix.reshape(B * Hs, De), BF16)
        out = self.paligemma_with_expert.forward_joint(prefix.reshape(B * P, Dp), suffix_bf, qcode, kcode, pos, cond, B, P, Hs)
        out32 = ops.cast_ag(out, F32)
        v_t = ops.linear_f32(out32, self.action_out_proj.weight, self.action_out_proj.bias)
        return (u_t.view(B * Hs, -1) if u_t is not None else None), out32, v_t

    def forward(self, observation, actions, noise=None, time=None) -> torch.Tensor:
        images, img_masks, lang_tokens, lang_masks, state = self._preprocess_observation(
            observation, train=self.train_augmentation
        )
        if noise is None:
            noise = self.sample_noise(actions.shape, actions.device)
        if time is None:
            time = self.sample_time(actions.shape[0], actions.device)
        B, Hs = actions.shape[0], actions.shape[1]
        u_t, _, v_t = self._trunk(images, img_masks, lang_tokens, lang_masks, state, actions, noise, time)
        return ops.mse_loss(u_t, v_t).view(B, Hs, -1)

    @torch.no_grad()
    def sample_actions(self, device, observation, noise=None, num_steps=10) -> torch.Tensor:
        from .infer import InferenceEngine

        bsize = observation.state.shape[0]
        if noise is None:
            noise = self.sample_noise((bsize, self.config.action_horizon, self.config.action_dim), device)
        images, img_masks, lang_tokens, lang_masks, state = self._preprocess_observation(observation, train=False)
        wait = getattr(self.paligemma_with_expert.unit_hooks, "wait_params", None)
        if wait is not None:
            wait()
        if self.trim_prompt_padding_infer:
            lang_tokens, lang_masks = self._trim_prompt(lang_tokens, lang_masks, granule=self.trim_prompt_granule_infer)
        key = (bsize, lang_tokens.shape[1], len(images))
        eng = self._engine
        if eng is not None and eng.stale():
            self._engine = eng = None
            self.__dict__.pop("_engine_lru", None)
        if eng is not None and eng.shape_matches(*key):
            out = eng.replay_then_verify(images, img_masks, lang_tokens, lang_masks, noise.to(F32), num_steps)
            if out is not None:
                return out
        if eng is None or not eng.compatible(*key):
            lru = self.__dict__.setdefault("_engine_lru", {})
            eng = lru.pop(key, None)
            if eng is None or not eng.compatible(*key):
                eng = InferenceEngine(self, *key)
            lru[key] = eng
            while len(lru) > self._ENGINE_SLOTS:
                lru.pop(next(iter(lru)))
            self.__dict__["_engine_cur"] = eng
        return eng.sample_actions(images, img_masks, lang_tokens, lang_masks, noise.to(F32), num_steps)


class AdvantageEstimator(PI0Pytorch):

    def __init__(self, config):
        super().__init__(config)
        self.loss_value_weight = getattr(config, "loss_value_weight", 0.0)
        self.loss_action_weight = getattr(config, "loss_action_weight", 1.0)
        w = self.action_in_proj.out_features
        self.value_head = nn.Sequential(Linear(w, w), nn.Identity(), Linear(w, w), nn.Identity(), Linear(w, 1), nn.Identity())

    def _preprocess_observation(self, observation, *, train=True, return_full_obs=False):
        from .preprocessing import preprocess_observation_custom

        res = self.paligemma_with_expert.siglip_cfg.image_size
        obs = preprocess_observation_custom(observation, train=train, image_resolution=(res, res), apply_aug=False)
        full = (list(obs.images.values()), list(obs.image_masks.values()), obs.tokenized_prompt, obs.tokenized_prompt_mask,
                obs.state, obs)
        return full if return_full_obs else full[:-1]

    def _value(self, out32, B: int, Hs: int):
        vh = self.value_head
        deep = out32.view(B, Hs, -1)[:, 0, :].contiguous()
        x = ops.silu_f32(ops.linear_f32(deep, vh[0].weight, vh[0].bias))
        x = ops.silu_f32(ops.linear_f32(x, vh[2].weight, vh[2].bias))
        return torch.tanh(ops.linear_f32(x, vh[4].weight, vh[4].bias))

    def forward(self, observation, actions, noise=None, time=None, return_loss_dict=False):
        images, img_masks, lang_tokens, lang_masks, state, obs_full = self._preprocess_observation(
            observation, train=self.training, return_full_obs=True
        )
        if noise is None:
            noise = self.sample_noise(actions.shape, actions.device)
        if time is None:
            time = self.sample_time(actions.shape[0], actions.device)
        B, Hs = actions.shape[0], actions.shape[1]
        u_t, out32, v_t = self._trunk(images, img_masks, lang_tokens, lang_masks, state, actions, noise, time)
        loss_action = ops.mse_loss(u_t, v_t).view(B, Hs, -1).mean(dim=-1)
        loss = loss_action * self.loss_action_weight
        value = self._value(out32, B, Hs)
        target = torch.clamp(obs_full.progress.float(), -1.0, 1.0).unsqueeze(1)
        value_loss = (value - target) ** 2 * self.loss_value_weight
        aux = {"loss_action": loss_action.detach().mean(), "loss_value": value_loss.detach().mean()}
        loss = loss + value_loss
        return (loss, aux) if return_loss_dict else loss

# ... 42 lines not shown
```

### kai0_amd/ops.py

```python

from __future__ import annotations

import contextlib
import ctypes as C
import os
import math

import torch

from . import _lib
from ._lib import AttnBwdDesc, AttnDesc, GemmDesc

BF16 = torch.bfloat16
F32 = torch.float32

NORM_PARTIAL_BLOCKS = 512
COLSUM_BLOCKS = 256


def _stream() -> int:
    return torch.cuda.current_stream().cuda_stream


def _p(t: torch.Tensor | None) -> int | None:
    return None if t is None else t.data_ptr()


def _chk(t: torch.Tensor, dtype, name: str) -> None:
    if not t.is_cuda:
        raise _lib.Kai0HipError(f"{name}: expected a CUDA (HIP) tensor; the product path has no CPU fallback")
    if t.dtype != dtype:
        raise TypeError(f"{name}: expected {dtype}, got {t.dtype}")
    if not t.is_contiguous():
        raise ValueError(f"{name}: expected a contiguous tensor")


GEMM_TUNING = {"persist": {"0": 1, "2": 2}.get(os.environ.get("KAI0_GEMM_PERSIST", "1"), 0), "general_epilogue": 0,
               "small_w8": {"0": 1, "2": 2}.get(os.environ.get("KAI0_GEMM_W8", "1"), 0)}


@contextlib.contextmanager
def gemm_tuning(**kw):
    unknown = set(kw) - set(GEMM_TUNING)
    if unknown:
        raise KeyError(f"gemm_tuning: unknown hook(s) {sorted(unknown)}")
    old = dict(GEMM_TUNING)
    GEMM_TUNING.update(kw)
    try:
        yield
    finally:
        GEMM_TUNING.update(old)


def gemm(
    A: torch.Tensor, B: torch.Tensor, out: torch.Tensor, *, M: int, N: int, K: int, a_kc: bool = True,
    b_kc: bool = True, lda: int, ldb: int, ldc: int, batch: int = 1, batch_inner: int = 1,
    sA=(0, 0), sB=(0, 0), sC=(0, 0), a_map=None, b_map=None, c_map=None, bias: torch.Tensor | None = None,
    scale: float = 1.0, act: int = 0, pre_out: torch.Tensor | None = None, gate: torch.Tensor | None = None,
    gate_rpb: int = 0, gate_ld: int = 0, residual: torch.Tensor | None = None, ldr: int = 0, sR=(0, 0),
    accumulate: bool = False, a_off_elems: int = 0, b_off_elems: int = 0, c_off_elems: int = 0, split_k: int = 1,
    aux1: torch.Tensor | None = None, aux2: torch.Tensor | None = None, segs=None, rowvec=None, rv=(0, 0, 1),
    B2: torch.Tensor | None = None, pre_out2: torch.Tensor | None = None, norm=None, nt_out: bool = False, rope=None,
) -> torch.Tensor:
    for t in (A, B, out):
        if not t.is_cuda:
            raise _lib.Kai0HipError("gemm: expected CUDA (HIP) tensors; the product path has no CPU fallback")
    if A.dtype != BF16 or B.dtype != BF16:
        raise TypeError(f"gemm: bf16 operands expected, got {A.dtype} / {B.dtype}")
    d = GemmDesc()
    d.A = A.data_ptr() + 2 * a_off_elems
    d.B = B.data_ptr() + 2 * b_off_elems
    out_f32 = out.dtype == F32
    d.C = out.data_ptr() + (4 if out_f32 else 2) * c_off_elems
    d.M, d.N, d.K = M, N, K
    d.a_kc, d.b_kc = int(a_kc), int(b_kc)
    d.lda, d.ldb, d.ldc = lda, ldb, ldc
    d.batch, d.batch_inner = batch, batch_inner
    d.sA1, d.sA2 = sA
    d.sB1, d.sB2 = sB
    d.sC1, d.sC2 = sC
    if a_map:
        d.a_rpb, d.a_bs, d.a_off = a_map
    if b_map:
        d.b_rpb, d.b_bs, d.b_off = b_map
    if c_map:
        d.c_rpb, d.c_bs, d.c_off = c_map
    if bias is not None:
        d.bias = bias.data_ptr()
        d.bias_f32 = int(bias.dtype == F32)
    d.scale = scale
    d.act = act
    d.out_f32 = int(out_f32)
    d.pre_out = _p(pre_out)
    d.aux1, d.aux2 = _p(aux1), _p(aux2)
    if rope is not None:
        rc, rs, half, n_end = rope
        if rc.dtype != BF16 or rs.dtype != BF16 or not rc.is_contiguous() or not rs.is_contiguous() or rc.shape != (M, half) or rs.shape != (M, half):
            raise TypeError("gemm: rope tables must be contiguous bf16 [M, half]")
        d.rope_cos, d.rope_sin, d.rope_half, d.rope_n_end = rc.data_ptr(), rs.data_ptr(), half, n_end
    if B2 is not None:
        if B2.dtype != BF16 or not B2.is_cuda:
            raise TypeError("gemm: B2 must be a bf16 HIP tensor")
        d.B2 = B2.data_ptr()
    d.pre_out2 = _p(pre_out2)
    if gate is not None:
        d.gate = gate.data_ptr()
        d.gate_rpb = gate_rpb
        d.gate_ld = gate_ld
    if residual is not None:
        d.residual = residual.data_ptr()
        d.ldr = ldr
        d.sR1, d.sR2 = sR
    d.accumulate = int(accumulate)
    d.c_nontemporal = int(nt_out)
    if rowvec is not None:
        if rowvec.dtype != F32:
            raise TypeError("gemm: rowvec must be f32")
        d.rowvec = rowvec.data_ptr()
        d.rv_s1, d.rv_s2, d.rv_ld = rv
    if segs:
        d.nseg = len(segs)
        for i, (dst, ld, nb) in enumerate(segs):
            d.seg[i].dst, d.seg[i].ld, d.seg[i].n_begin = dst.data_ptr(), ld, nb
    if split_k > 1:
        ws = _workspace(batch * split_k * M * N * 4, A.device)
        d.split_k, d.workspace, d.workspace_bytes = split_k, ws.data_ptr(), ws.numel()
    if norm is not None:
        kind, nout, nw, nb, neps = norm
        _chk(nout, BF16, "gemm: norm_out")
        _chk(nw, F32 if kind == 1 else BF16, "gemm: norm weight")
        d.norm_kind, d.norm_out, d.norm_w, d.norm_eps = int(kind), nout.data_ptr(), nw.data_ptr(), float(neps)
        if nb is not None:
            _chk(nb, BF16, "gemm: norm bias")
            d.norm_b = nb.data_ptr()
    d.persist, d.general_epilogue, d.small_w8 = GEMM_TUNING["persist"], GEMM_TUNING["general_epilogue"], GEMM_TUNING["small_w8"]
    _lib.call("kai0_gemm_bf16", C.byref(d), _stream())
    return out


def skinny_split_k(N: int, K: int) -> int:
    if K % 512:
        raise _lib.Kai0HipError(f"skinny gemm: K={K} must be a multiple of 512")
    tiles = N // 32
    if K % 1024 == 0 and tiles * (K // 1024) >= 190:
        return K // 1024
    return K // 512


def skinny_workspace(M: int, N: int, split_k: int, device) -> torch.Tensor:
    return torch.empty((max(split_k, 1), M, N), dtype=F32, device=device)


def skinny_gemm(A, W, *, M: int, N: int, K: int, lda: int, ldw: int, mode: int = 0, pair_stride: int = 16, segs=None,
                split_k: int = 1, workspace=None, a_map=None, c_map=None, gate=None, gate_rpb: int = 0, gate_ld: int = 0,
                residual=None, ldr: int = 0, rope_cos=None, rope_sin=None, rope_half: int = 0, mod=None, mod_ld: int = 0,
                mod_rpb: int = 0, eps: float = 1e-6, w_packed: bool = False, rowsq_in=None, rowsq_parts: int = 0, cvec=None,
                rowsq_out=None):
    for t in (A, W):
        if not t.is_cuda or t.dtype != BF16:
            raise _lib.Kai0HipError("skinny_gemm: expected bf16 CUDA (HIP) tensors; the product path has no CPU fallback")
    d = _lib.SkinnyDesc()
    d.A, d.W, d.lda, d.ldw = A.data_ptr(), W.data_ptr(), lda, ldw
    d.M, d.N, d.K = M, N, K
    d.pair_stride, d.mode, d.split_k = pair_stride, mode, split_k
    d.w_packed = int(w_packed)
    if a_map:
        d.a_rpb, d.a_bs, d.a_off = a_map
    if c_map:
        d.c_rpb, d.c_bs, d.c_off = c_map
    d.nseg = len(segs or ())
    for i, (dst, ld, nb, ne, rope) in enumerate(segs or ()):
        if not dst.is_cuda or dst.dtype != BF16:
            raise _lib.Kai0HipError("skinny_gemm: destinations must be bf16 CUDA (HIP) tensors")
        d.seg[i].dst, d.seg[i].ld, d.seg[i].n_begin, d.seg[i].n_end, d.seg[i].rope = dst.data_ptr(), ld, nb, ne, int(rope)
    if gate is not None:
        d.gate, d.gate_rpb, d.gate_ld = gate.data_ptr(), gate_rpb, gate_ld
    if residual is not None:
        d.residual, d.ldr = residual.data_ptr(), ldr
    if rope_cos is not None:
        d.rope_cos, d.rope_sin, d.rope_half = rope_cos.data_ptr(), rope_sin.data_ptr(), rope_half
    if split_k > 1:
        if workspace is None or workspace.dtype != F32:
            raise _lib.Kai0HipError("skinny_gemm: split_k > 1 writes f32 partial products into `workspace` (skinny_workspace)")
        d.workspace, d.workspace_bytes = workspace.data_ptr(), workspace.numel() * 4
    elif split_k == -1 and workspace is not None:
        d.workspace, d.workspace_bytes = workspace.data_ptr(), workspace.numel() * workspace.element_size()
    if mod is not None:
        if mod.dtype != F32 or not mod.is_cuda or mod.stride(-1) != 1:
            raise _lib.Kai0HipError("skinny_gemm: mod must be an f32 CUDA (HIP) tensor with unit inner stride")
        d.mod, d.mod_ld, d.mod_rpb, d.eps = mod.data_ptr(), mod_ld, mod_rpb, eps
    if rowsq_in is not None:
        _chk(rowsq_in, F32, "rowsq_in")
        _chk(cvec, F32, "cvec")
        d.rowsq_in, d.cvec, d.rowsq_parts, d.rowsq_ld, d.eps = rowsq_in.data_ptr(), cvec.data_ptr(), rowsq_parts, rowsq_in.stride(0), eps
    if rowsq_out is not None:
        _chk(rowsq_out, F32, "rowsq_out")
        d.rowsq_out, d.rowsq_out_ld = rowsq_out.data_ptr(), rowsq_out.stride(0)
    _lib.call("kai0_gemm_skinny_bf16", C.byref(d), _stream())


def pack_skinny_weight(w: torch.Tensor) -> torch.Tensor:
    N, K = w.shape
    if N % 16 or K % 32:
        raise ValueError(f"pack_skinny_weight: N % 16 == 0 and K % 32 == 0 required, got {tuple(w.shape)}")
    return w.view(N // 16, 16, K // 32, 4, 8).permute(0, 2, 3, 1, 4).contiguous().view(N, K)


def adarms_combine(partials, gate_prev, residual, mod, rows_per_batch: int, eps: float = 1e-6):
    S, rows, D = partials.shape
    Bn = rows // rows_per_batch
    dev = partials.device
    x = torch.empty((rows, D), dtype=BF16, device=dev)
    y = torch.empty((rows, D), dtype=BF16, device=dev)
    gate = torch.empty((Bn, D), dtype=BF16, device=dev)
    _lib.call("kai0_adarms_combine", partials.data_ptr(), S, rows * D, _p(gate_prev), _p(residual), x.data_ptr(),
              mod.data_ptr(), y.data_ptr(), gate.data_ptr(), rows, rows_per_batch, D, eps, _stream())
    return x, y, gate


def attn_decode(Q, K, Vt, O, qcode, kcode, *, batch, rows, H, HD, Sk, q0, q_bs, k_bs, k_ld, k_rows, vt_bs, vt_ld, scale):
    for t in (Q, K, Vt, O):
        if not t.is_cuda or t.dtype != BF16:
            raise _lib.Kai0HipError("attn_decode: expected bf16 CUDA (HIP) tensors; the product path has no CPU fallback")
    ws = _workspace(int(_lib.load().kai0_attn_decode_workspace_bytes(batch, rows)), Q.device)
    _lib.call("kai0_attn_decode", Q.data_ptr(), K.data_ptr(), Vt.data_ptr(), O.data_ptr(), _p(qcode), _p(kcode), batch, rows,
              H, HD, Sk, q0, q_bs, k_bs, k_ld, k_rows, vt_bs, vt_ld, qcode.stride(0) if qcode is not None else 0,
              kcode.stride(0) if kcode is not None else 0, scale, ws.data_ptr(), ws.numel(), _stream())


def transpose_strided(src, dst, *, R, C, src_ld, dst_ld, batch=1, src_bs=0, dst_bs=0):
    _lib.call("kai0_transpose_strided_bf16", src.data_ptr(), dst.data_ptr(), R, C, src_ld, dst_ld, batch, src_bs, dst_bs,
              _stream())


def rowdot(a, b, D: int):
    if a.dtype != BF16 or b.dtype != BF16 or not a.is_contiguous() or not b.is_contiguous() or a.numel() != b.numel():
        raise _lib.Kai0HipError("rowdot: two contiguous bf16 tensors of the same size expected")
    rows = a.numel() // D
    out = torch.empty((rows,), dtype=F32, device=a.device)
    _lib.call("kai0_rowdot_bf16", a.data_ptr(), b.data_ptr(), out.data_ptr(), rows, D, _stream())
    return out


def rope_permutation(n_total: int, n_rope_end: int, half: int = 128) -> torch.Tensor:
    if half != 128 or n_rope_end % 256 != 0 or n_rope_end > n_total:
        raise ValueError("rope_permutation: head_dim 256 (half 128), rotated range a whole number of heads")
    pc = torch.arange(n_total)
    real = (pc // 256) * 256 + ((pc % 128) // 64) * 128 + 64 * ((pc % 256) // 128) + pc % 64
    return torch.where(pc < n_rope_end, real, pc)


def rope_table(pos, inv_freq, bf16: bool = False):
    pos = pos.contiguous()
    if pos.dtype != torch.int32:
        raise TypeError("rope_table: pos must be int32")
    rows, half = pos.numel(), inv_freq.numel()
    cos = torch.empty((rows, half), dtype=BF16 if bf16 else F32, device=pos.device)
    sin = torch.empty((rows, half), dtype=BF16 if bf16 else F32, device=pos.device)
    _lib.call("kai0_rope_table", pos.data_ptr(), inv_freq.data_ptr(), cos.data_ptr(), sin.data_ptr(), rows, half, int(bf16), _stream())
    return cos, sin


def prefix_codes(img_masks, lang_mask, n_img: int, Hs: int):
    B, T = lang_mask.shape
    ms = [m.contiguous() for m in img_masks]
    lm = lang_mask.contiguous()
    for m in (*ms, lm):
        if m.dtype != torch.bool or not m.is_cuda:
            raise TypeError("prefix_codes: bool CUDA (HIP) masks expected")
    if any(m.shape != (B,) for m in ms):
        raise ValueError("prefix_codes: camera masks must be [B]")
    S = len(ms) * n_img + T + Hs
    q, k, p = (torch.empty((B, S), dtype=torch.int32, device=lm.device) for _ in range(3))
    ptrs = (C.c_void_p * len(ms))(*[m.data_ptr() for m in ms])
    _lib.call("kai0_prefix_codes", C.addressof(ptrs), len(ms), lm.data_ptr(), B, n_img, T, Hs, q.data_ptr(), k.data_ptr(), p.data_ptr(), _stream())
    return q, k, p


_WS: dict = {}


def _workspace(nbytes: int, device) -> torch.Tensor:
    key = (device.index, _stream())
    ws = _WS.get(key)
    if ws is None or ws.numel() < nbytes:
        ws = torch.empty(max(nbytes, 64 << 20), dtype=torch.uint8, device=device)
        _WS[key] = ws
    return ws


def pick_split_k(M: int, N: int, K: int, batch: int = 1) -> int:
    tiles = ((M + 127) // 128) * ((N + 127) // 128) * batch
    if tiles >= 384 or K < 512:
        return 1
    if M <= 128:
        return max(1, min(32, 768 // tiles, K // 128))
    return max(1, min(round(400 / tiles), K // 768))


_WGRAD_SPLIT = {(1152, 4304, 24576): 3, (4304, 1152, 24576): 3, (3456, 1152, 24576): 2, (1152, 1152, 24576): 6,
                (2560, 2048, 30976): 3, (2048, 2048, 30976): 4}


def pick_split_k_wgrad(M: int, N: int, K: int) -> int:
    t256 = ((M + 255) // 256) * ((N + 255) // 256)
    if t256 >= 200 or K < 4096:
        return pick_split_k(M, N, K)
    return _WGRAD_SPLIT.get((M, N, K)) or max(1, min(6, 256 // t256, K // 2048))


def linear_fwd(x, w, bias=None, residual=None, act=0, want_pre=False, gate=None, gate_rpb=0, out=None):
    M, K = x.shape
    N = w.shape[0]
    if out is None:
        out = torch.empty((M, N), dtype=BF16, device=x.device)
    pre = torch.empty((M, N), dtype=BF16, device=x.device) if want_pre else None
    gemm(x, w, out, M=M, N=N, K=K, lda=K, ldb=K, ldc=N, bias=bias, act=act, pre_out=pre, residual=residual, ldr=N,
         gate=gate, gate_rpb=gate_rpb, gate_ld=N, split_k=pick_split_k(M, N, K))
    return (out, pre) if want_pre else out


def gemm_f32(A, sam, sak, Bm, sbk, sbn, out, M, N, K, bias=None, accumulate=False, split_k=None):
    for t in (A, Bm, out):
        if not t.is_cuda or t.dtype != F32:
            raise _lib.Kai0HipError("gemm_f32: expected f32 CUDA (HIP) tensors; the product path has no CPU fallback")
    if split_k is None:
        tiles = ((M + 63) // 64) * ((N + 63) // 64)
        split_k = 1 if (tiles >= 512 or K < 512) else max(1, min(64, 1024 // tiles, K // 128))
    ws = _workspace(split_k * M * N * 4, A.device) if split_k > 1 else None
    _lib.call("kai0_gemm_f32", A.data_ptr(), sam, sak, Bm.data_ptr(), sbk, sbn, out.data_ptr(), out.stride(0), M, N, K,
              _p(bias), int(accumulate), split_k, _p(ws), ws.numel() if ws is not None else 0, _stream())
    return out


def _grad_dst(param, dtype):
    dst = getattr(param, "_kai0_grad_out", None)
    if dst is not None and dst.shape == param.shape and dst.dtype == dtype:
        ensure = getattr(param, "_kai0_grad_ensure", None)
        if ensure is not None:
            ensure()
        return dst
    return torch.empty(param.shape, dtype=dtype, device=param.device)


def _grad_ret(param, g):
    if g is None or param is None:
        return g
    dst = getattr(param, "_kai0_grad_out", None)
    if dst is not None and g.data_ptr() == dst.data_ptr():
        if _DUAL:
            _note_side_gradient(param)
        param._kai0_grad_done()
        return None
    return g


_DUAL: dict = {}
_JOIN_PENDING: dict = {}


def side_stream(device):
    idx = device.index if device.index is not None else torch.cuda.current_device()
    main = torch.cuda.current_stream(idx)
    pair = _DUAL.get(idx)
    if pair is None or pair[0] != main:
        pair = _DUAL[idx] = (main, pair[1] if pair is not None else torch.cuda.Stream(device=idx))
    return pair[1]


def stream_pair(device):
    idx = device.index if device.index is not None else torch.cuda.current_device()
    return _DUAL.get(idx)


def join_streams(device) -> None:
    pair = stream_pair(device)
    if pair is not None:
        cur = torch.cuda.current_stream(pair[0].device_index)
        for st in pair:
            if st != cur:
                cur.wait_stream(st)
    flush_deferred(device.index if device.index is not None else torch.cuda.current_device())


def reset_backward_state() -> None:
    _DEFERRED.clear()
    for idx in list(_JOIN_PENDING):
        if _JOIN_PENDING[idx]:
            _JOIN_PENDING[idx] = False
            pair = _DUAL.get(idx)
            if pair is not None:
                pair[0].wait_stream(pair[1])


def _note_side_gradient(param) -> None:
    pair = stream_pair(param.device)
    if pair is None or torch.cuda.current_stream(pair[0].device_index) != pair[1]:
        return
    idx = pair[0].device_index
    if _JOIN_PENDING.get(idx):
        return

    def join():
        _JOIN_PENDING[idx] = False
        pair[0].wait_stream(pair[1])

    try:
        torch.autograd.Variable._execution_engine.queue_callback(join)
        _JOIN_PENDING[idx] = True
    except RuntimeError:
        pair[0].wait_stream(pair[1])


_DEFER_REDUCE = True
_DEFERRED: dict = {}


def _reduce_partials(param, part, nb: int, ncols: int, ld: int, out, col0: int = 0):
    src = part.data_ptr() + 4 * col0
    f32 = int(out.dtype == F32)
    dst = getattr(param, "_kai0_grad_out", None)
    if not (_DEFER_REDUCE and dst is not None and out.data_ptr() == dst.data_ptr() and out.is_cuda):
        _lib.call("kai0_reduce_partials", src, nb, ncols, ld, out.data_ptr(), f32, _stream())
        return
    idx = out.device.index
    q = _DEFERRED.setdefault(idx, [])
    q.append(((src, out.data_ptr(), ld, nb, ncols, f32, 0), (part, out), torch.cuda.current_stream(idx)))
    if len(q) == 1:
        try:
            torch.autograd.Variable._execution_engine.queue_callback(lambda: flush_deferred(idx))
        except RuntimeError:
            flush_deferred(idx)


def flush_deferred(idx=None) -> None:
    for i in list(_DEFERRED) if idx is None else [idx]:
        q = _DEFERRED.get(i)
        if not q:
            continue
        _DEFERRED[i] = []
        cur = torch.cuda.current_stream(i)
        for st in {e[2] for e in q}:
            if st != cur:
                cur.wait_stream(st)
        items = (_lib.ReduceItem * len(q))(*[_lib.ReduceItem(*e[0]) for e in q])
        with torch.cuda.device(i):
            _lib.call("kai0_reduce_partials_batch", C.addressof(items), len(q), cur.cuda_stream)
        for e in q:
            if e[2] != cur:
                e[1][0].record_stream(cur)


def _bias_grads(dy, M: int, N: int, ld: int, biases):
    scratch = torch.empty((COLSUM_BLOCKS, N), dtype=F32, device=dy.device)
    used = C.c_int(0)
    _lib.call("kai0_colsum_partials_bf16", dy.data_ptr(), M, N, ld, scratch.data_ptr(), COLSUM_BLOCKS, C.addressof(used), _stream())
    out = []
    for b, c0, width in biases:
        db = _grad_dst(b, b.dtype)
        _reduce_partials(b, scratch, used.value, width, N, db, col0=c0)
        out.append(_grad_ret(b, db))
    return out


class LinearFn(torch.autograd.Function):

    @staticmethod
    def forward(ctx, x, w, bias, residual, act: int):
        _chk(x, BF16, "linear.x")
        _chk(w, BF16, "linear.w")
        need_pre = act == 1 and (x.requires_grad or w.requires_grad)
        r = linear_fwd(x, w, bias, residual, act, want_pre=need_pre)
        out, pre = r if need_pre else (r, None)
        ctx.save_for_backward(x, w, pre)
        ctx.bias = bias
        ctx.has_bias = bias is not None
        ctx.bias_dtype = bias.dtype if bias is not None else None
        ctx.has_res = residual is not None
        ctx.act = act
        return out

    @staticmethod
    def backward(ctx, dout):
        x, w, pre = ctx.saved_tensors
        dout = dout.contiguous()
        M, K = x.shape
        N = w.shape[0]
        dres = dout if ctx.has_res else None
        dy = dout
        if ctx.act == 1:
            dy = torch.empty_like(dout)
            _lib.call("kai0_gelu_bwd", dout.data_ptr(), pre.data_ptr(), dy.data_ptr(), dout.numel(), _stream())
        dx = dw = db = None
        if ctx.needs_input_grad[0]:
            dx = torch.empty((M, K), dtype=BF16, device=x.device)
            if M >= 4096 and N % 8 == 0 and K % 8 == 0:
                wt = transpose(w)
                gemm(dy, wt, dx, M=M, N=K, K=N, a_kc=True, b_kc=True, lda=N, ldb=N, ldc=K)
                del wt
            else:
                gemm(dy, w, dx, M=M, N=K, K=N, a_kc=True, b_kc=False, lda=N, ldb=K, ldc=K, split_k=pick_split_k(M, K, N))
        if ctx.needs_input_grad[1]:
            dw = _grad_dst(w, BF16)
            gemm(dy, x, dw, M=N, N=K, K=M, a_kc=False, b_kc=False, lda=N, ldb=K, ldc=K, split_k=pick_split_k_wgrad(N, K, M), nt_out=True)
        if ctx.has_bias and ctx.needs_input_grad[2]:
            (db,) = _bias_grads(dy, M, N, N, [(ctx.bias, 0, N)])
        return dx, _grad_ret(w, dw), db, dres, None


def transpose(x: torch.Tensor) -> torch.Tensor:
    _chk(x, BF16, "transpose.x")
    R, Cc = x.shape
    y = torch.empty((Cc, R), dtype=BF16, device=x.device)
    _lib.call("kai0_transpose_bf16", x.data_ptr(), y.data_ptr(), R, Cc, _stream())
    return y


def linear(x, w, bias=None, residual=None, act=0):
    return LinearFn.apply(x, w, bias, residual, act)


def fused_columns(rows: int, widths, device):
    buf = torch.empty((rows, sum(widths)), dtype=BF16, device=device)
    out, c = [], 0
    for w in widths:
        out.append(buf[:, c : c + w])
        c += w
    return out


def _as_fused(ts, widths):
    t0 = ts[0]
    if t0 is None or t0.dim() != 2:
        return None
    total = sum(widths)
    off = t0.storage_offset()
    for t, w in zip(ts, widths):
        if (t is None or t.dtype != t0.dtype or t.dim() != 2 or t.shape != (t0.shape[0], w) or t.stride() != (total, 1)
                or t.untyped_storage().data_ptr() != t0.untyped_storage().data_ptr() or t.storage_offset() != off):
            return None
        off += w
    return t0.as_strided((t0.shape[0], total), (total, 1), t0.storage_offset())


_FUSE_MULTI = True


class LinearMultiFn(torch.autograd.Function):

    @staticmethod
    def forward(ctx, x, n: int, *wb):
        _chk(x, BF16, "linear_multi.x")
        ws, bs = wb[:n], wb[n:]
        widths = tuple(int(w.shape[0]) for w in ws)
        has_b = [b is not None for b in bs]
        fuse = (_FUSE_MULTI and 2 <= n <= 3 and all(w % 8 == 0 for w in widths) and (all(has_b) or not any(has_b))
                and (not any(has_b) or len({b.dtype for b in bs}) == 1))
        ctx.n, ctx.biases, ctx.widths, ctx.fuse = n, bs, widths, fuse
        if not fuse:
            outs = tuple(linear_fwd(x, w, b) for w, b in zip(ws, bs))
            ctx.save_for_backward(x, *ws)
            return outs
        M, K = x.shape
        Nt = sum(widths)
        wcat = _as_rows([w.detach() for w in ws])
        if wcat is None:
            wcat = torch.cat(ws, dim=0)
        bcat = None
        if all(has_b):
            bcat = _as_rows([b.detach() for b in bs])
            if bcat is None:
                bcat = torch.cat(bs, dim=0)
        outs = tuple(torch.empty((M, w), dtype=BF16, device=x.device) for w in widths)
        segs, c = [], 0
        for o, w in zip(outs, widths):
            segs.append((o, w, c))
            c += w
        gemm(x, wcat, outs[0], M=M, N=Nt, K=K, lda=K, ldb=K, ldc=widths[0], bias=bcat, segs=segs, split_k=pick_split_k(M, Nt, K))
        ctx.save_for_backward(x, wcat, *ws)
        return outs

    @staticmethod
    def backward(ctx, *douts):
        n, bs, widths = ctx.n, ctx.biases, ctx.widths
        if not ctx.fuse or any(d is None for d in douts):
            x, *rest = ctx.saved_tensors
            ws = rest[1:] if ctx.fuse else rest
            return LinearMultiFn._backward_separate(ctx, x, ws, douts)
        x, wcat, *ws = ctx.saved_tensors
        M, K = x.shape
        Nt = sum(widths)
        dev = x.device
        dy = _as_fused(douts, widths)
        if dy is None:
            dy = torch.cat([d if d.dtype == BF16 else d.to(BF16) for d in douts], dim=1)
        dx = None
        if ctx.needs_input_grad[0]:
            dx = torch.empty((M, K), dtype=BF16, device=dev)
            if M >= 4096:
                wt = transpose(wcat)
                gemm(dy, wt, dx, M=M, N=K, K=Nt, lda=Nt, ldb=Nt, ldc=K)
                del wt
            else:
                gemm(dy, wcat, dx, M=M, N=K, K=Nt, a_kc=True, b_kc=False, lda=Nt, ldb=K, ldc=K)
        dws, dbs = [None] * n, [None] * n
        if any(ctx.needs_input_grad[2 + i] for i in range(n)):
            dsts = [_grad_dst(w, BF16) for w in ws]
            dwcat = _as_rows(dsts)
            tmp = dwcat is None
            if tmp:
                dwcat = torch.empty((Nt, K), dtype=BF16, device=dev)
            gemm(dy, x, dwcat, M=Nt, N=K, K=M, a_kc=False, b_kc=False, lda=Nt, ldb=K, ldc=K, split_k=pick_split_k_wgrad(Nt, K, M))
            r = 0
            for i, (w, dst) in enumerate(zip(ws, dsts)):
                if tmp:
                    dst.copy_(dwcat[r : r + widths[i]])
                r += widths[i]
                dws[i] = _grad_ret(w, dst)
        if bs[0] is not None and any(ctx.needs_input_grad[2 + n + i] for i in range(n)):
            offs = [sum(widths[:i]) for i in range(n)]
            dbs = _bias_grads(dy, M, Nt, Nt, [(b, offs[i], widths[i]) for i, b in enumerate(bs)])
        return (dx, None, *dws, *dbs)

    @staticmethod
    def _backward_separate(ctx, x, ws, douts):
        n, bs = ctx.n, ctx.biases
        M, K = x.shape
        dev = x.device
        dws, dbs = [None] * n, [None] * n
        dx = torch.empty((M, K), dtype=BF16, device=dev) if ctx.needs_input_grad[0] else None
        first = True
        for i, (w, b, dy) in enumerate(zip(ws, bs, douts)):
            if dy is None:
                continue
            dy = dy.contiguous()
            N = w.shape[0]
            if dx is not None:
                if M >= 4096 and N % 8 == 0:
                    wt = transpose(w)
                    gemm(dy, wt, dx, M=M, N=K, K=N, lda=N, ldb=N, ldc=K, accumulate=not first)
                    del wt
                else:
                    gemm(dy, w, dx, M=M, N=K, K=N, a_kc=True, b_kc=False, lda=N, ldb=K, ldc=K, accumulate=not first)
                first = False
            if ctx.needs_input_grad[2 + i]:
                dw = _grad_dst(w, BF16)
                gemm(dy, x, dw, M=N, N=K, K=M, a_kc=False, b_kc=False, lda=N, ldb=K, ldc=K, split_k=pick_split_k_wgrad(N, K, M), nt_out=True)
                dws[i] = _grad_ret(w, dw)
            if b is not None and ctx.needs_input_grad[2 + n + i]:
                (dbs[i],) = _bias_grads(dy, M, N, N, [(b, 0, N)])
        if dx is not None and first:
            dx.zero_()
        return (dx, None, *dws, *dbs)


def _as_rows(ts):
    t0 = ts[0]
    ptr = t0.data_ptr()
    for t in ts:
        if (not t.is_contiguous() or t.dtype != t0.dtype or t.shape[1:] != t0.shape[1:] or t.data_ptr() != ptr
                or t.untyped_storage().data_ptr() != t0.untyped_storage().data_ptr()):
            return None
        ptr += t.numel() * t.element_size()
    return t0.as_strided((sum(t.shape[0] for t in ts), *t0.shape[1:]), t0.stride(), t0.storage_offset())


def linear_multi(x, weights, biases=None):
    n = len(weights)
    biases = list(biases) if biases is not None else [None] * n
    return LinearMultiFn.apply(x, n, *weights, *biases)


class LinearF32Fn(torch.autograd.Function):

    @staticmethod
    def forward(ctx, x, w, bias):
        _chk(x, F32, "linear_f32.x")
        _chk(w, F32, "linear_f32.w")
        M, K = x.shape
        N = w.shape[0]
        out = torch.empty((M, N), dtype=F32, device=x.device)
        if M <= 16 and K % 4 == 0:
            _lib.call("kai0_linear_rows_f32", x.data_ptr(), w.data_ptr(), _p(bias), out.data_ptr(), N, M, N, K, _stream())
        else:
            gemm_f32(x, K, 1, w, 1, K, out, M, N, K, bias=bias)
        ctx.save_for_backward(x, w)
        ctx.bias = bias
        ctx.has_bias = bias is not None
        return out

    @staticmethod
    def backward(ctx, dout):
        x, w = ctx.saved_tensors
        dout = dout.contiguous()
        M, K = x.shape
        N = w.shape[0]
        dx = dw = db = None
        if ctx.needs_input_grad[0]:
            dx = torch.empty((M, K), dtype=F32, device=x.device)
            gemm_f32(dout, N, 1, w, K, 1, dx, M, K, N)
        if ctx.needs_input_grad[1]:
            dw = _grad_dst(w, F32)
            gemm_f32(dout, 1, N, x, K, 1, dw, N, K, M)
        if ctx.has_bias and ctx.needs_input_grad[2]:
            db = _grad_dst(ctx.bias, F32)
            ones = torch.ones((1, M), dtype=F32, device=x.device)
            gemm_f32(ones, M, 1, dout, N, 1, db.view(1, N), 1, N, M)
        return dx, _grad_ret(w, dw), _grad_ret(ctx.bias, db)


def linear_f32(x, w, bias=None):
    return LinearF32Fn.apply(x, w, bias)


class RMSNormFn(torch.autograd.Function):

    @staticmethod
    def forward(ctx, x, w, eps: float):
        _chk(x, BF16, "rmsnorm.x")
        _chk(w, F32, "rmsnorm.w")
        rows, D = x.shape
        y = torch.empty_like(x)
        rstd = torch.empty((rows,), dtype=F32, device=x.device)
        _lib.call("kai0_rmsnorm_fwd", x.data_ptr(), w.data_ptr(), y.data_ptr(), rstd.data_ptr(), rows, D, eps, _stream())
        ctx.save_for_backward(x, w, rstd)
        return x.view_as(x), y

    @staticmethod
    def backward(ctx, dres, dy):
        x, w, rstd = ctx.saved_tensors
        rows, D = x.shape
        if dy is None:
            return dres, None, None
        dy = dy.contiguous()
        dres = dres.contiguous() if dres is not None else None
        dx = torch.empty_like(x)
        nb = NORM_PARTIAL_BLOCKS
        part = torch.empty((nb, D), dtype=F32, device=x.device)
        _lib.call("kai0_rmsnorm_bwd", dy.data_ptr(), x.data_ptr(), w.data_ptr(), rstd.data_ptr(), dx.data_ptr(),
                  part.data_ptr(), nb, _p(dres), rows, D, _stream())
        dw = None
        if ctx.needs_input_grad[1]:
            dw = _grad_dst(w, F32)
            _reduce_partials(w, part, nb, D, D, dw)
        return dx, _grad_ret(w, dw), None


def rmsnorm_res(x, w, eps=1e-6):
    return RMSNormFn.apply(x, w, eps)


def rmsnorm(x, w, eps=1e-6):
    return RMSNormFn.apply(x, w, eps)[1]


class AdaRMSFn(torch.autograd.Function):

    @staticmethod
    def forward(ctx, x, mod, rows_per_batch: int, eps: float):
        _chk(x, BF16, "adarms.x")
        _chk(mod, F32, "adarms.mod")
        rows, D = x.shape
        Bn = rows // rows_per_batch
        y = torch.empty_like(x)
        gate = torch.empty((Bn, D), dtype=BF16, device=x.device)
        rstd = torch.empty((rows,), dtype=F32, device=x.device)
        _lib.call("kai0_adarms_fwd", x.data_ptr(), mod.data_ptr(), y.data_ptr(), gate.data_ptr(), rstd.data_ptr(), rows,
                  rows_per_batch, D, eps, _stream())
        ctx.save_for_backward(x, mod, rstd)
        ctx.rpb = rows_per_batch
        return x.view_as(x), y, gate

    @staticmethod
    def backward(ctx, dres, dy, dgate):
        x, mod, rstd = ctx.saved_tensors
        rows, D = x.shape
        if dy is None:
            dy = torch.zeros_like(x)
        dy = dy.contiguous()
        dgate = dgate.contiguous() if dgate is not None else None
        dres = dres.contiguous() if dres is not None else None
        dx = torch.empty_like(x)
        dmod = torch.empty_like(mod)
        _lib.call("kai0_adarms_bwd", dy.data_ptr(), _p(dgate), x.data_ptr(), mod.data_ptr(), rstd.data_ptr(),
                  dx.data_ptr(), dmod.data_ptr(), _p(dres), rows, ctx.rpb, D, _stream())
        return dx, dmod, None, None


def adarms_res(x, mod, rows_per_batch, eps=1e-6):
    return AdaRMSFn.apply(x, mod, rows_per_batch, eps)


def adarms(x, mod, rows_per_batch, eps=1e-6):
    _, y, gate = AdaRMSFn.apply(x, mod, rows_per_batch, eps)
    return y, gate


class LayerNormFn(torch.autograd.Function):

    @staticmethod
    def forward(ctx, x, w, b, eps: float):
        _chk(x, BF16, "layernorm.x")
        rows, D = x.shape
        y = torch.empty_like(x)
        mean = torch.empty((rows,), dtype=F32, device=x.device)
        rstd = torch.empty((rows,), dtype=F32, device=x.device)
        _lib.call("kai0_layernorm_fwd", x.data_ptr(), w.data_ptr(), b.data_ptr(), y.data_ptr(), mean.data_ptr(),
                  rstd.data_ptr(), rows, D, eps, _stream())
        ctx.save_for_backward(x, w, b, mean, rstd)
        return x.view_as(x), y

    @staticmethod
    def backward(ctx, dres, dy):
        x, w, b, mean, rstd = ctx.saved_tensors
        if dy is None:
            return dres, None, None, None
        dy = dy.contiguous()
        dres = dres.contiguous() if dres is not None else None
        rows, D = x.shape
        dx = torch.empty_like(x)
        nb = NORM_PARTIAL_BLOCKS
        part = torch.empty((nb, 2 * D), dtype=F32, device=x.device)
        _lib.call("kai0_layernorm_bwd", dy.data_ptr(), x.data_ptr(), w.data_ptr(), mean.data_ptr(), rstd.data_ptr(),
                  dx.data_ptr(), part.data_ptr(), nb, _p(dres), rows, D, _stream())
        dw, db = _grad_dst(w, w.dtype), _grad_dst(b, b.dtype)
        _reduce_partials(w, part, nb, D, 2 * D, dw)
        _reduce_partials(b, part, nb, D, 2 * D, db, col0=D)
        return dx, _grad_ret(w, dw), _grad_ret(b, db), None


def layernorm_res(x, w, b, eps=1e-6):
    return LayerNormFn.apply(x, w, b, eps)


def layernorm(x, w, b, eps=1e-6):
    return LayerNormFn.apply(x, w, b, eps)[1]


class GegluFn(torch.autograd.Function):
    @staticmethod
    def forward(ctx, g, u):
        _chk(g, BF16, "geglu.g")
        _chk(u, BF16, "geglu.u")
        h = torch.empty_like(g)
        _lib.call("kai0_geglu_fwd", g.data_ptr(), u.data_ptr(), h.data_ptr(), g.numel(), _stream())
        ctx.save_for_backward(g, u)
        return h

    @staticmethod
    def backward(ctx, dh):
        g, u = ctx.saved_tensors
        dh = dh.contiguous()
        dg = torch.empty_like(g)
        du = torch.empty_like(u)
        _lib.call("kai0_geglu_bwd", dh.data_ptr(), g.data_ptr(), u.data_ptr(), dg.data_ptr(), du.data_ptr(), g.numel(),
                  _stream())
        return dg, du


def geglu(g, u):
    return GegluFn.apply(g, u)


_GEGLU_PAIR = True


def set_geglu_pair(on: bool) -> bool:
    global _GEGLU_PAIR
    old, _GEGLU_PAIR = _GEGLU_PAIR, bool(on)
    return old


class GegluMlpFn(torch.autograd.Function):

    @staticmethod
    def forward(ctx, x, wg, wu, wd, residual):
        _chk(x, BF16, "geglu_mlp.x")
        M, D = x.shape
        F = wg.shape[0]
        u = torch.empty((M, F), dtype=BF16, device=x.device)
        h = torch.empty((M, F), dtype=BF16, device=x.device)
        if _GEGLU_PAIR and F % 32 == 0:
            g = torch.empty((M, F), dtype=BF16, device=x.device)
            gemm(x, wg, h, M=M, N=F, K=D, lda=D, ldb=D, ldc=F, act=6, B2=wu, pre_out=g, pre_out2=u)
        else:
            g = linear_fwd(x, wg)
            gemm(x, wu, h, M=M, N=F, K=D, lda=D, ldb=D, ldc=F, act=2, pre_out=u, aux1=g, split_k=1)
        out = linear_fwd(h, wd, residual=residual)
        ctx.save_for_backward(x, wg, wu, wd, g, u, h)
        ctx.has_res = residual is not None
        return out

    @staticmethod
    def backward(ctx, dout):
        x, wg, wu, wd, g, u, h = ctx.saved_tensors
        dout = dout.contiguous()
        M, D = x.shape
        F = wg.shape[0]
        dev = x.device

        def wgrad(dy, inp, w, n, k):
            dw = _grad_dst(w, BF16)
            gemm(dy, inp, dw, M=n, N=k, K=M, a_kc=False, b_kc=False, lda=n, ldb=k, ldc=k, split_k=pick_split_k_wgrad(n, k, M), nt_out=True)
            return dw

        dwd = wgrad(dout, h, wd, D, F) if ctx.needs_input_grad[3] else None
        dg = torch.empty((M, F), dtype=BF16, device=dev)
        du = torch.empty((M, F), dtype=BF16, device=dev)
        wdt = transpose(wd)
        gemm(dout, wdt, dg, M=M, N=F, K=D, lda=D, ldb=D, ldc=F, act=3, pre_out=du, aux1=g, aux2=u)
        del wdt
        dwg = wgrad(dg, x, wg, F, D) if ctx.needs_input_grad[1] else None
        dwu = wgrad(du, x, wu, F, D) if ctx.needs_input_grad[2] else None
        dx = None
        if ctx.needs_input_grad[0]:
            dx = torch.empty((M, D), dtype=BF16, device=dev)
            wgt = transpose(wg)
            gemm(dg, wgt, dx, M=M, N=D, K=F, lda=F, ldb=F, ldc=D, split_k=1)
            wut = transpose(wu)
            gemm(du, wut, dx, M=M, N=D, K=F, lda=F, ldb=F, ldc=D, accumulate=True, split_k=1)
            del wgt, wut
        return dx, _grad_ret(wg, dwg), _grad_ret(wu, dwu), _grad_ret(wd, dwd), (dout if ctx.has_res else None)


_PAD_MLP_ROWS = True


class GeluMlpFn(torch.autograd.Function):

    @staticmethod
    def forward(ctx, x, w1, b1, w2, b2, residual):
        _chk(x, BF16, "gelu_mlp.x")
        M, D = x.shape
        F = w1.shape[0]
        ldh = round_up(F, 64) if _PAD_MLP_ROWS else F
        dev = x.device
        pre = torch.empty((M, ldh), dtype=BF16, device=dev)
        h = torch.empty((M, ldh), dtype=BF16, device=dev)
        gemm(x, w1, h, M=M, N=F, K=D, lda=D, ldb=D, ldc=ldh, bias=b1, act=1, pre_out=pre, split_k=1)
        out = torch.empty((M, w2.shape[0]), dtype=BF16, device=dev)
        gemm(h, w2, out, M=M, N=w2.shape[0], K=F, lda=ldh, ldb=F, ldc=w2.shape[0], bias=b2, residual=residual,
             ldr=w2.shape[0], split_k=pick_split_k(M, w2.shape[0], F))
        ctx.save_for_backward(x, w1, w2, pre, h)
        ctx.biases = (b1, b2)
        ctx.has_res = residual is not None
        return out

    @staticmethod
    def backward(ctx, dout):
        x, w1, w2, pre, h = ctx.saved_tensors
        b1, b2 = ctx.biases
        dout = dout.contiguous()
        M, D = x.shape
        F, Do = w1.shape[0], w2.shape[0]
        ldh = pre.shape[1]
        dev = x.device
        big = M >= 4096

        def colsum(dy, N, ld, b):
            return _bias_grads(dy, M, N, ld, [(b, 0, N)])[0]

        dw2 = db2 = dw1 = db1 = dx = None
        if ctx.needs_input_grad[3]:
            dw2 = _grad_dst(w2, BF16)
            gemm(dout, h, dw2, M=Do, N=F, K=M, a_kc=False, b_kc=False, lda=Do, ldb=ldh, ldc=F, split_k=pick_split_k_wgrad(Do, F, M), nt_out=True)
            dw2 = _grad_ret(w2, dw2)
        if b2 is not None and ctx.needs_input_grad[4]:
            db2 = colsum(dout, Do, Do, b2)
        dpre = torch.empty((M, ldh), dtype=BF16, device=dev)
        if big:
            w2t = transpose(w2)
            gemm(dout, w2t, dpre, M=M, N=F, K=Do, lda=Do, ldb=Do, ldc=ldh, act=5, aux1=pre)
            del w2t
# ... 5 lines not shown
            dw1 = _grad_ret(w1, dw1)
        if b1 is not None and ctx.needs_input_grad[2]:
            db1 = colsum(dpre, F, ldh, b1)
        if ctx.needs_input_grad[0]:
            dx = torch.empty((M, D), dtype=BF16, device=dev)
            if big:
                w1t = transpose(w1)
                gemm(dpre, w1t, dx, M=M, N=D, K=F, lda=ldh, ldb=F, ldc=D)
                del w1t
            else:
                gemm(dpre, w1, dx, M=M, N=D, K=F, a_kc=True, b_kc=False, lda=ldh, ldb=D, ldc=D, split_k=pick_split_k(M, D, F))
        return dx, dw1, db1, dw2, db2, (dout if ctx.has_res else None)


def gelu_mlp(x, w1, b1, w2, b2, residual=None):
    return GeluMlpFn.apply(x, w1, b1, w2, b2, residual)


def geglu_mlp(x, wg, wu, wd, residual=None):
    return GegluMlpFn.apply(x, wg, wu, wd, residual)


class GatedResidualFn(torch.autograd.Function):

    @staticmethod
    def forward(ctx, x, y, gate, rows_per_batch: int):
        rows, D = x.shape
        out = torch.empty_like(x)
        _lib.call("kai0_gated_fwd", x.data_ptr(), y.data_ptr(), gate.data_ptr(), out.data_ptr(), rows, rows_per_batch, D,
                  _stream())
        ctx.save_for_backward(y, gate)
        ctx.rpb = rows_per_batch
        return out

    @staticmethod
    def backward(ctx, dout):
        y, gate = ctx.saved_tensors
        dout = dout.contiguous()
        rows, D = y.shape
        dy = torch.empty_like(y)
        dgate = torch.empty_like(gate)
        _lib.call("kai0_gated_bwd", dout.data_ptr(), y.data_ptr(), gate.data_ptr(), dy.data_ptr(), dgate.data_ptr(), rows,
                  ctx.rpb, D, _stream())
        return dout, dy, dgate, None


def gated_residual(x, y, gate, rows_per_batch):
    return GatedResidualFn.apply(x, y, gate, rows_per_batch)


class SiluF32Fn(torch.autograd.Function):
    @staticmethod
    def forward(ctx, x):
        _chk(x, F32, "silu.x")
        y = torch.empty_like(x)
        _lib.call("kai0_silu_fwd_f32", x.data_ptr(), y.data_ptr(), x.numel(), _stream())
        ctx.save_for_backward(x)
        return y

    @staticmethod
    def backward(ctx, dy):
        (x,) = ctx.saved_tensors
        dy = dy.contiguous()
        dx = torch.empty_like(x)
        _lib.call("kai0_silu_bwd_f32", dy.data_ptr(), x.data_ptr(), dx.data_ptr(), x.numel(), _stream())
        return dx


def silu_f32(x):
    return SiluF32Fn.apply(x)


class CastFn(torch.autograd.Function):

    @staticmethod
    def forward(ctx, x, to_bf16: bool):
        ctx.to_bf16 = to_bf16
        return cast(x, BF16 if to_bf16 else F32)

    @staticmethod
    def backward(ctx, dy):
        return cast(dy.contiguous(), F32 if ctx.to_bf16 else BF16), None


def cast(x: torch.Tensor, dtype) -> torch.Tensor:
    if x.dtype == dtype:
        return x
    y = torch.empty(x.shape, dtype=dtype, device=x.device)
    if dtype == BF16:
        _chk(x, F32, "cast.x")
        _lib.call("kai0_cast_f32_to_bf16", x.data_ptr(), y.data_ptr(), x.numel(), _stream())
    else:
        _chk(x, BF16, "cast.x")
        _lib.call("kai0_cast_bf16_to_f32", x.data_ptr(), y.data_ptr(), x.numel(), _stream())
    return y


def cast_ag(x, dtype):
    if x.dtype == dtype:
        return x
    return CastFn.apply(x, dtype == BF16)


class EmbedFn(torch.autograd.Function):

    @staticmethod
    def forward(ctx, table, tokens, scale: float):
        _chk(table, BF16, "embed.table")
        if tokens.dtype != torch.int64:
            raise TypeError("embed.tokens must be int64")
        Bn, T = tokens.shape
        D = table.shape[1]
        out = torch.empty((Bn * T, D), dtype=BF16, device=table.device)
        _lib.call("kai0_embed_gather", table.data_ptr(), tokens.data_ptr(), out.data_ptr(), Bn, T, D, scale, T * D, 0, D,
                  _stream())
        ctx.save_for_backward(tokens)
        ctx.table = table
        ctx.shape = table.shape
        ctx.scale = scale
        return out

    @staticmethod
    def backward(ctx, dout):
        (tokens,) = ctx.saved_tensors
        dout = dout.contiguous()
        Bn, T = tokens.shape
        V, D = ctx.shape
        dst = getattr(ctx.table, "_kai0_grad_out", None)
        if dst is not None and dst.shape == (V, D) and dst.dtype == BF16:
            dtable = _grad_dst(ctx.table, BF16)
            ctx.table._kai0_grad_accumulates = True
        else:
            dtable = torch.zeros((V, D), dtype=BF16, device=dout.device)
        _lib.call("kai0_embed_grad", dout.data_ptr(), tokens.data_ptr(), dtable.data_ptr(), Bn, T, D, ctx.scale, T * D, 0,
                  D, _stream())
        return _grad_ret(ctx.table, dtable), None, None


def embed(table, tokens, scale):
    if tokens.dtype in (torch.int32, torch.int16, torch.uint8):
        tokens = tokens.to(torch.int64)
    return EmbedFn.apply(table, tokens.contiguous(), scale)


class PatchEmbedFn(torch.autograd.Function):

    @staticmethod
    def forward(ctx, img, w, b, pos, patch: int):
        _chk(img, F32, "patch_embed.img")
        _chk(w, F32, "patch_embed.weight")
        n, Cc, HW, _ = img.shape
        D = w.shape[0]
        G = HW // patch
        Kd = Cc * patch * patch
        rows = n * G * G
        cols = torch.empty((rows, Kd), dtype=F32, device=img.device)
        _lib.call("kai0_patch_im2col", img.data_ptr(), cols.data_ptr(), n, Cc, HW, patch, _stream())
        pe = torch.empty((rows, D), dtype=F32, device=img.device)
        w2 = w.view(D, Kd)
        gemm_f32(cols, Kd, 1, w2, 1, Kd, pe, rows, D, Kd, bias=b)
        out = torch.empty((rows, D), dtype=BF16, device=img.device)
        _lib.call("kai0_add_pos_cast", pe.data_ptr(), pos.data_ptr(), out.data_ptr(), rows, G * G, D, _stream())
        ctx.save_for_backward(cols)
        ctx.params = (w, b, pos)
        ctx.dims = (n, G, D, Kd, tuple(w.shape))
        return out

    @staticmethod
    def backward(ctx, dout):
        (cols,) = ctx.saved_tensors
        n, G, D, Kd, wshape = ctx.dims
        rows = n * G * G
        d32 = cast(dout.contiguous(), F32)
        pw, pb, ppos = ctx.params
        dw = _grad_dst(pw, F32).view(D, Kd)
        gemm_f32(d32, 1, D, cols, Kd, 1, dw, D, Kd, rows)
        db = _grad_dst(pb, F32)
        ones = torch.ones((1, rows), dtype=F32, device=dout.device)
        gemm_f32(ones, rows, 1, d32, D, 1, db.view(1, D), 1, D, rows)
        GG = G * G
        dpos = _grad_dst(ppos, F32)
        if n == 1:
            dpos.copy_(d32)
        else:
            ones_n = torch.ones((1, n), dtype=F32, device=dout.device)
            gemm_f32(ones_n, n, 1, d32.view(n, GG * D), GG * D, 1, dpos.view(1, GG * D), 1, GG * D, n)
        return None, _grad_ret(pw, dw.view(wshape)), _grad_ret(pb, db), _grad_ret(ppos, dpos), None


def patch_embed(img, w, b, pos, patch):
    return PatchEmbedFn.apply(img, w, b, pos, patch)


def _copy_rows(src, dst, Bn, rows, D, sbs, sr0, sld, dbs, dr0, dld):
    _lib.call("kai0_copy_rows_bf16", src.data_ptr(), dst.data_ptr(), Bn, rows, D, sbs, sr0, sld, dbs, dr0, dld, _stream())


def rope_(x, pos, inv_freq, Bn, S, s_ld, row0, H, HD, inverse=False):
    _lib.call("kai0_rope_inplace", x.data_ptr(), pos.data_ptr(), inv_freq.data_ptr(), Bn, S, s_ld, row0, H, HD,
              int(inverse), _stream())


def rope2_(x, H, x2, H2, pos, inv_freq, Bn, S, s_ld, row0, HD):
    _lib.call("kai0_rope_inplace2", x.data_ptr(), H, x2.data_ptr(), H2, pos.data_ptr(), inv_freq.data_ptr(), Bn, S, s_ld, row0, HD,
              _stream())


def rope_copy(src_t, dst_t, pos, inv_freq, Bn, S, H, HD, *, src, dst, pos_bs, pos_off=0, inverse=False):
    sbs, sld, sr0 = src
    dbs, dld, dr0 = dst
    _lib.call("kai0_rope_copy", src_t.data_ptr() + 2 * sr0 * sld, dst_t.data_ptr() + 2 * dr0 * dld, pos.data_ptr() + 4 * pos_off,
              inv_freq.data_ptr(), Bn, S, H, HD, sbs, sld, dbs, dld, pos_bs, int(inverse), _stream())


def pack_rows(parts, HD: int, pos=None, pos_bs: int = 0, inv_freq=None):
    for c0 in range(0, len(parts), 12):
        chunk = parts[c0 : c0 + 12]
        arr = (_lib.PackPart * len(chunk))()
        for a, (src, soff, dst, doff, (sbs, sld), (dbs, dld), Bn, rows, cols, mode, pos_off) in zip(arr, chunk):
            a.src = None if src is None else src.data_ptr() + 2 * soff
            a.dst = dst.data_ptr() + 2 * doff
            a.src_bs, a.src_ld, a.dst_bs, a.dst_ld = sbs, sld, dbs, dld
            a.B, a.rows, a.cols, a.mode, a.pos_off = Bn, rows, cols, mode, pos_off
        _lib.call("kai0_pack_rows", C.addressof(arr), len(chunk), _p(pos), pos_bs, _p(inv_freq), HD, _stream())


def round_up(x: int, m: int) -> int:
    return (x + m - 1) // m * m


def attn_fwd_keysplit(Q, K, V, O, *, rows, Sk, HD, H, q0, ldk, ldv, qcode, kcode, scale, q_off, o_off, parts: int = 4):
    if Sk % parts != 0:
        raise ValueError("attn_fwd_keysplit: Sk must be a multiple of the number of key ranges")
    rng = Sk // parts
    dev = Q.device
    o_parts = torch.empty((parts, rows, HD), dtype=BF16, device=dev)
    lse = torch.empty((parts, rows), dtype=torch.float32, device=dev)
    d = AttnDesc()
    d.Q, d.K, d.V, d.O = Q.data_ptr() + 2 * q_off, K.data_ptr(), V.data_ptr(), o_parts.data_ptr()
    d.qcode, d.kcode = _p(qcode), _p(kcode)
    d.rows, d.Sk, d.HD, d.H, d.q0, d.batch, d.batch_inner = rows, rng, HD, H, q0, parts, 1
    d.ldq, d.ldk, d.ldv, d.ldo = HD, ldk, ldv, HD
    d.sQ1, d.sK1, d.sV1, d.sO1 = 0, rng * ldk, rng * ldv, rows * HD
    d.qcode_ld, d.kcode_ld = 0, rng
    d.scale = scale
    d.online = 1
    d.lse, d.s_lse = lse.data_ptr(), rows
    _lib.call("kai0_attn_fwd", C.byref(d), _stream())
    _lib.call("kai0_attn_combine", o_parts.data_ptr(), lse.data_ptr(), O.data_ptr() + 2 * o_off, parts, rows, HD, HD, rows * HD, rows, _stream())


def attn_fwd(Q, K, V, O, P, *, rows, Sk, HD, H=1, q0=0, batch=1, batch_inner=1, ldq, ldk, ldv, ldo, ldp=0, sQ=(0, 0),
             sK=(0, 0), sV=(0, 0), sO=(0, 0), sP=0, qcode=None, kcode=None, scale, q_off=0, o_off=0, lse=None, online=0):
    d = AttnDesc()
    d.Q, d.K, d.V, d.O = Q.data_ptr() + 2 * q_off, K.data_ptr(), V.data_ptr(), O.data_ptr() + 2 * o_off
    d.P = _p(P)
    d.qcode, d.kcode = _p(qcode), _p(kcode)
    d.rows, d.Sk, d.HD, d.H, d.q0, d.batch, d.batch_inner = rows, Sk, HD, H, q0, batch, batch_inner
    d.ldq, d.ldk, d.ldv, d.ldo, d.ldp = ldq, ldk, ldv, ldo, ldp
    d.sQ1, d.sQ2 = sQ
    d.sK1, d.sK2 = sK
    d.sV1, d.sV2 = sV
    d.sO1, d.sO2 = sO
    d.sP = sP
    if qcode is not None:
        d.qcode_ld, d.kcode_ld = qcode.stride(0), kcode.stride(0)
    d.scale = scale
    d.online = online
    if lse is not None:
        _chk(lse, torch.float32, "lse")
        d.lse, d.s_lse = lse.data_ptr(), lse.stride(0)
    _lib.call("kai0_attn_fwd", C.byref(d), _stream())


_ATTN_STORE_P = os.environ.get("KAI0_ATTN_STORE_P", "0") == "1"


def mqa_attention_fwd(q_all, k_all, v_all, qcode, kcode, Bn, Sq, q0, Sk, S_ld, H, HD, scale, want_probs=True, want_lse=False):
    dev = q_all.device
    M = Sq * H
    if want_lse:
        lse = torch.empty((Bn, M), dtype=torch.float32, device=dev)
        att = torch.empty((Bn, S_ld, H * HD), dtype=BF16, device=dev)
        attn_fwd(q_all, k_all, v_all, att, None, rows=M, Sk=Sk, HD=HD, H=H, q0=q0, batch=Bn, ldq=HD, ldk=HD, ldv=HD, ldo=HD,
                 sQ=(S_ld * H * HD, 0), sK=(S_ld * HD, 0), sV=(S_ld * HD, 0), sO=(S_ld * H * HD, 0), qcode=qcode, kcode=kcode,
                 scale=scale, q_off=q0 * H * HD, o_off=q0 * H * HD, lse=lse)
        return att, lse
    probs = torch.empty((Bn, M, S_ld), dtype=BF16, device=dev) if want_probs else None
    att = torch.empty((Bn, S_ld, H * HD), dtype=BF16, device=dev)
    attn_fwd(q_all, k_all, v_all, att, probs, rows=M, Sk=Sk, HD=HD, H=H, q0=q0, batch=Bn, ldq=HD, ldk=HD, ldv=HD, ldo=HD,
             ldp=S_ld, sQ=(S_ld * H * HD, 0), sK=(S_ld * HD, 0), sV=(S_ld * HD, 0), sO=(S_ld * H * HD, 0), sP=M * S_ld,
             qcode=qcode, kcode=kcode, scale=scale, q_off=q0 * H * HD, o_off=q0 * H * HD)
    return att, probs


def _attn_bwd_split(Bn: int, S_ld: int, HD: int, M: int) -> int:
    t256 = ((S_ld + 255) // 256) * ((HD + 255) // 256) * Bn
    if t256 >= 160 or M < 4096:
        return 1
    return max(1, min(8, -(-256 // t256), M // 2048))


def _joint_attention_grads(cfg, pos, inv_freq, dq_all, dk_all, dv_all):
    Bn, S, S_ld, H, HD, seg_lens, scale, recompute = cfg
    dev = dq_all.device
    grads, parts = [], []
    r0 = 0
    for Li in seg_lens:
        W3 = (H + 2) * HD
        dq, dk, dv = fused_columns(Bn * Li, (H * HD, HD, HD), dev)
        parts.append((dq_all, r0 * H * HD, dq, 0, (S_ld * H * HD, H * HD), (Li * W3, W3), Bn, Li, H * HD, 2, r0))
        parts.append((dk_all, r0 * HD, dk, 0, (dk_all.stride(0), HD), (Li * W3, W3), Bn, Li, HD, 2, r0))
        parts.append((dv_all, r0 * HD, dv, 0, (dv_all.stride(0), HD), (Li * W3, W3), Bn, Li, HD, 0, 0))
        grads += [dq, dk, dv]
        r0 += Li
    pack_rows(parts, HD, pos, S, inv_freq)
    return (None, None, None, None, None, None, None, *grads)


class JointAttentionFn(torch.autograd.Function):

    @staticmethod
    def forward(ctx, pos, qcode, kcode, inv_freq, H: int, HD: int, seg_lens: tuple, *qkv):
        nseg = len(seg_lens)
        qs, ks, vs = qkv[0::3], qkv[1::3], qkv[2::3]
        dev = qs[0].device
        S = sum(seg_lens)
        Bn = qs[0].shape[0] // seg_lens[0]
        S_ld = round_up(S, 8)
        q_all = torch.empty((Bn, S_ld, H * HD), dtype=BF16, device=dev)
        k_all = torch.empty((Bn, S_ld, HD), dtype=BF16, device=dev)
        v_all = torch.empty((Bn, S_ld, HD), dtype=BF16, device=dev)
        parts = []
        r0 = 0
        for i in range(nseg):
            Li = seg_lens[i]
            parts.append((qs[i], 0, q_all, r0 * H * HD, (Li * qs[i].stride(0), qs[i].stride(0)), (S_ld * H * HD, H * HD), Bn, Li, H * HD, 1, r0))
            parts.append((ks[i], 0, k_all, r0 * HD, (Li * ks[i].stride(0), ks[i].stride(0)), (S_ld * HD, HD), Bn, Li, HD, 1, r0))
            parts.append((vs[i], 0, v_all, r0 * HD, (Li * vs[i].stride(0), vs[i].stride(0)), (S_ld * HD, HD), Bn, Li, HD, 0, 0))
            r0 += Li
        if S_ld > S:
            parts.append((None, 0, q_all, S * H * HD, (0, 0), (S_ld * H * HD, H * HD), Bn, S_ld - S, H * HD, 3, 0))
            parts.append((None, 0, k_all, S * HD, (0, 0), (S_ld * HD, HD), Bn, S_ld - S, HD, 3, 0))
            parts.append((None, 0, v_all, S * HD, (0, 0), (S_ld * HD, HD), Bn, S_ld - S, HD, 3, 0))
        pack_rows(parts, HD, pos, S, inv_freq)
        scale = HD**-0.5
        recompute = not _ATTN_STORE_P and S <= 2048
        att, probs = mqa_attention_fwd(q_all, k_all, v_all, qcode, kcode, Bn, S, 0, S, S_ld, H, HD, scale, want_lse=recompute)
        outs, parts = [], []
        r0 = 0
        for i in range(nseg):
            Li = seg_lens[i]
            o = torch.empty((Bn * Li, H * HD), dtype=BF16, device=dev)
            parts.append((att, r0 * H * HD, o, 0, (S_ld * H * HD, H * HD), (Li * H * HD, H * HD), Bn, Li, H * HD, 0, 0))
            outs.append(o)
            r0 += Li
        pack_rows(parts, HD)
        ctx.save_for_backward(q_all, k_all, v_all, probs, pos, inv_freq, att, qcode, kcode)
        ctx.cfg = (Bn, S, S_ld, H, HD, seg_lens, scale, recompute)
        return tuple(outs)

    @staticmethod
    def backward(ctx, *douts):
        q_all, k_all, v_all, probs, pos, inv_freq, att, qcode, kcode = ctx.saved_tensors
        Bn, S, S_ld, H, HD, seg_lens, scale, recompute = ctx.cfg
        dev = q_all.device
        M = S * H
        dq_all = torch.empty((Bn, S_ld, H * HD), dtype=BF16, device=dev)
        if recompute:
            pd = torch.empty((2, Bn, M, S_ld), dtype=BF16, device=dev)
            lse, probs, dscores = probs, pd[0], pd[1]
        datt = torch.empty((Bn, S_ld, H * HD), dtype=BF16, device=dev)
        parts = []
        r0 = 0
        for i, Li in enumerate(seg_lens):
            parts.append((douts[i].contiguous(), 0, datt, r0 * H * HD, (Li * H * HD, H * HD), (S_ld * H * HD, H * HD), Bn, Li, H * HD, 0, 0))
            r0 += Li
        if S_ld > S:
            parts.append((None, 0, datt, S * H * HD, (0, 0), (S_ld * H * HD, H * HD), Bn, S_ld - S, H * HD, 3, 0))
        pack_rows(parts, HD)
        if recompute:
            d = AttnBwdDesc()
            d.dO, d.O, d.Q, d.K, d.V = datt.data_ptr(), att.data_ptr(), q_all.data_ptr(), k_all.data_ptr(), v_all.data_ptr()
            d.lse, d.qcode, d.kcode = lse.data_ptr(), _p(qcode), _p(kcode)
            d.P, d.dS, d.dQ = probs.data_ptr(), dscores.data_ptr(), dq_all.data_ptr()
            d.batch, d.rows, d.Sk, d.HD, d.H = Bn, M, S, HD, H
            d.ldo, d.ldk, d.ldv, d.ldp = HD, HD, HD, S_ld
            d.sO, d.sK, d.sV, d.sP, d.s_lse = S_ld * H * HD, S_ld * HD, S_ld * HD, M * S_ld, lse.stride(0)
            if qcode is not None:
                d.qcode_ld, d.kcode_ld = qcode.stride(0), kcode.stride(0)
            d.scale = scale
            _lib.call("kai0_attn_bwd_dq2", C.byref(d), _stream())
        if recompute and (q_all.data_ptr() - datt.data_ptr()) % 16 == 0:
            dkv = torch.empty((2, Bn, S_ld, HD), dtype=BF16, device=dev)
            gemm(pd, datt, dkv, M=S_ld, N=HD, K=M, a_kc=False, b_kc=False, lda=S_ld, ldb=HD, ldc=HD, batch=2 * Bn, batch_inner=Bn,
                 sA=(Bn * M * S_ld, M * S_ld), sB=((q_all.data_ptr() - datt.data_ptr()) // 2, S_ld * H * HD),
                 sC=(Bn * S_ld * HD, S_ld * HD), split_k=_attn_bwd_split(2 * Bn, S_ld, HD, M))
            dv_all, dk_all = dkv[0], dkv[1]
            return _joint_attention_grads(ctx.cfg, pos, inv_freq, dq_all, dk_all, dv_all)
        kv_split = _attn_bwd_split(Bn, S_ld, HD, M)
        dv_all = torch.empty((Bn, S_ld, HD), dtype=BF16, device=dev)
        gemm(probs, datt, dv_all, M=S_ld, N=HD, K=M, a_kc=False, b_kc=False, lda=S_ld, ldb=HD, ldc=HD, batch=Bn,
             sA=(M * S_ld, 0), sB=(S_ld * H * HD, 0), sC=(S_ld * HD, 0), split_k=kv_split)
        if not recompute:
            dscores = torch.empty_like(probs)
            _lib.call("kai0_attn_bwd_dq", datt.data_ptr(), att.data_ptr(), probs.data_ptr(), k_all.data_ptr(), v_all.data_ptr(),
                      dscores.data_ptr(), dq_all.data_ptr(), Bn, M, S, HD, HD, HD, HD, S_ld, S_ld * H * HD, S_ld * HD, S_ld * HD,
                      M * S_ld, scale, _stream())
        dk_all = torch.empty((Bn, S_ld, HD), dtype=BF16, device=dev)
        gemm(dscores, q_all, dk_all, M=S_ld, N=HD, K=M, a_kc=False, b_kc=False, lda=S_ld, ldb=HD, ldc=HD, batch=Bn,
             sA=(M * S_ld, 0), sB=(S_ld * H * HD, 0), sC=(S_ld * HD, 0), split_k=kv_split)
        return _joint_attention_grads(ctx.cfg, pos, inv_freq, dq_all, dk_all, dv_all)


def joint_attention(pos, qcode, kcode, inv_freq, H, HD, seg_lens, qkv):
    return JointAttentionFn.apply(pos, qcode, kcode, inv_freq, H, HD, tuple(seg_lens), *qkv)


_SIGLIP_BWD_FUSED = True
_SIGLIP_FWD_DEDICATED = True


def siglip_attn_fwd(q, k, v, out, *, n_img, S, NH, HD, ld_qkv, ld_out, lse=None):
    _lib.call("kai0_siglip_attn_fwd", q.data_ptr(), k.data_ptr(), v.data_ptr(), out.data_ptr(), _p(lse), n_img, S, NH, HD, ld_qkv,
              ld_qkv, ld_qkv, ld_out, S * ld_qkv, S * ld_qkv, S * ld_qkv, S * ld_out, HD**-0.5, _stream())


class SiglipAttentionFn(torch.autograd.Function):

    @staticmethod
    def forward(ctx, q, k, v, n_img: int, S: int, NH: int, HD: int):
        dev = q.device
        E = NH * HD
        S_ld = round_up(S, 8)
        scale = HD**-0.5
        out = torch.empty((n_img * S, E), dtype=BF16, device=dev)
        recompute = S == 256 and HD == 72 and S_ld == 256 and _SIGLIP_BWD_FUSED and not _ATTN_STORE_P
        if recompute and _SIGLIP_FWD_DEDICATED and q.stride(0) == k.stride(0) == v.stride(0):
            probs = torch.empty((n_img * NH, S), dtype=torch.float32, device=dev)
            siglip_attn_fwd(q, k, v, out, n_img=n_img, S=S, NH=NH, HD=HD, ld_qkv=q.stride(0), ld_out=E, lse=probs)
        elif recompute:
            probs = torch.empty((n_img * NH, S), dtype=torch.float32, device=dev)
            attn_fwd(q, k, v, out, None, rows=S, Sk=S, HD=HD, H=1, batch=n_img * NH, batch_inner=NH, ldq=E, ldk=E, ldv=E, ldo=E,
                     sQ=(S * E, HD), sK=(S * E, HD), sV=(S * E, HD), sO=(S * E, HD), scale=scale, lse=probs)
        else:
            probs = torch.empty((n_img * NH, S, S_ld), dtype=BF16, device=dev)
            attn_fwd(q, k, v, out, probs, rows=S, Sk=S, HD=HD, H=1, batch=n_img * NH, batch_inner=NH, ldq=E, ldk=E, ldv=E,
                     ldo=E, ldp=S_ld, sQ=(S * E, HD), sK=(S * E, HD), sV=(S * E, HD), sO=(S * E, HD), sP=S * S_ld, scale=scale)
        ctx.save_for_backward(q, k, v, probs, out)
        ctx.cfg = (n_img, S, S_ld, NH, HD, scale, recompute)
        return out

    @staticmethod
    def backward(ctx, dout):
        q, k, v, probs, out = ctx.saved_tensors
        n_img, S, S_ld, NH, HD, scale, recompute = ctx.cfg
        dev = q.device
        E = NH * HD
        dout = dout.contiguous()
        if recompute:
            dq, dk, dv = fused_columns(q.shape[0], (E, E, E), dev)
            _lib.call("kai0_siglip_attn_bwd2", q.data_ptr(), k.data_ptr(), v.data_ptr(), dout.data_ptr(), out.data_ptr(),
                      probs.data_ptr(), dq.data_ptr(), dk.data_ptr(), dv.data_ptr(), n_img, S, NH, HD, 3 * E, scale, _stream())
            return dq, dk, dv, None, None, None, None
        if S == 256 and HD == 72 and S_ld == 256 and _SIGLIP_BWD_FUSED:
            dq, dk, dv = fused_columns(q.shape[0], (E, E, E), dev)
            _lib.call("kai0_siglip_attn_bwd", q.data_ptr(), k.data_ptr(), v.data_ptr(), dout.data_ptr(), out.data_ptr(),
                      probs.data_ptr(), dq.data_ptr(), dk.data_ptr(), dv.data_ptr(), n_img, S, NH, HD, S_ld, 3 * E, scale,
                      _stream())
            return dq, dk, dv, None, None, None, None
        nb = n_img * NH
        sP = (NH * S * S_ld, S * S_ld)
        sE = (S * E, HD)
        dv = torch.empty_like(v)
        gemm(probs, dout, dv, M=S, N=HD, K=S, a_kc=False, b_kc=False, lda=S_ld, ldb=E, ldc=E, batch=nb, batch_inner=NH,
             sA=sP, sB=sE, sC=sE)
        dsum = rowdot(dout, out, HD)
        dprobs = torch.zeros_like(probs) if S_ld != S else torch.empty_like(probs)
        gemm(dout, v, dprobs, M=S, N=S, K=HD, lda=E, ldb=E, ldc=S_ld, batch=nb, batch_inner=NH, sA=sE, sB=sE, sC=sP, act=4,
             aux1=probs, rowvec=dsum, rv=(S * NH, 1, NH), scale=scale)
        dq = torch.empty_like(q)
        gemm(dprobs, k, dq, M=S, N=HD, K=S, a_kc=True, b_kc=False, lda=S_ld, ldb=E, ldc=E, batch=nb, batch_inner=NH,
             sA=sP, sB=sE, sC=sE)
        dk = torch.empty_like(k)
        gemm(dprobs, q, dk, M=S, N=HD, K=S, a_kc=False, b_kc=False, lda=S_ld, ldb=E, ldc=E, batch=nb, batch_inner=NH,
             sA=sP, sB=sE, sC=sE)
        return dq, dk, dv, None, None, None, None


def siglip_attention(q, k, v, n_img, S, NH, HD):
    return SiglipAttentionFn.apply(q, k, v, n_img, S, NH, HD)


def flow_mix(noise, actions, time):
    Bn = actions.shape[0]
    HA = actions.numel() // Bn
    x_t = torch.empty_like(actions)
    u_t = torch.empty_like(actions)
    _lib.call("kai0_flow_mix", noise.data_ptr(), actions.data_ptr(), time.data_ptr(), x_t.data_ptr(), u_t.data_ptr(), Bn,
              HA, _stream())
    return x_t, u_t


class MseFn(torch.autograd.Function):

    @staticmethod
    def forward(ctx, u, v):
        _chk(u, F32, "mse.u")
        _chk(v, F32, "mse.v")
        loss = torch.empty_like(v)
        _lib.call("kai0_mse_fwd", u.data_ptr(), v.data_ptr(), loss.data_ptr(), v.numel(), _stream())
        ctx.save_for_backward(u, v)
        return loss

    @staticmethod
    def backward(ctx, dl):
        u, v = ctx.saved_tensors
        dl = dl.contiguous()
        dv = torch.empty_like(v)
        _lib.call("kai0_mse_bwd", u.data_ptr(), v.data_ptr(), dl.data_ptr(), dv.data_ptr(), v.numel(), _stream())
        return None, dv


def mse_loss(u, v):
    return MseFn.apply(u, v)


def denoise_glue(x_t, *, xs=None, mod=None, mod_ld=0, rows_per_batch=1, eps=1e-6, w_out=None, b_out=None, dt=0.0, w_in=None,
                 b_in=None, xs_next=None, rowsq_next=None):
    rows, A = x_t.shape[0], x_t.shape[1]
    D = (xs if xs is not None else xs_next).shape[1]
    for t in (x_t, w_out, b_out, w_in, b_in, mod):
        if t is not None and t.dtype != F32:
            raise TypeError("denoise_glue: x_t, weights, biases and modulations are f32")
    _lib.call("kai0_denoise_glue", _p(xs), _p(mod), mod_ld, rows_per_batch, eps, _p(w_out), _p(b_out), x_t.data_ptr(), dt, _p(w_in),
              _p(b_in), _p(xs_next), rows, D, A, _p(rowsq_next), _stream())


def euler_step_(x, v, dt: float):
    _lib.call("kai0_euler_step", x.data_ptr(), v.data_ptr(), dt, x.numel(), _stream())
    return x


def sqrt_scale(dim: int) -> float:
    return float(torch.tensor(math.sqrt(dim), dtype=torch.float32))
```

Baseline: 68.84 samples/s.

## Skip dead prefix queries in last layer and write joint attention outputs in place

Result: no change. 69.24 samples/s, median of 6 (+0.6%).

```diff
diff --git a/kai0_amd/csrc/gemm_bf16.hip b/kai0_amd/csrc/gemm_bf16.hip
--- a/kai0_amd/csrc/gemm_bf16.hip
+++ b/kai0_amd/csrc/gemm_bf16.hip
@@ -630,7 +630,7 @@
     const bool plain_fast = p.act <= 1 && p.split_k == 1 && (p.bias != nullptr || p.residual != nullptr) && p.gate == nullptr &&
                             !p.accumulate && !p.out_f32 && p.nseg == 0 && (N_ALIGNED8(p.N));
     const bool simple_fast = MT == 8 && p.simple_epi && p.act <= 1 && p.split_k == 1 && p.gate == nullptr && !p.out_f32 && p.scale == 1.0f &&
-                             p.cmap.rpb == 0 && (N_ALIGNED8(p.N));
+                             (N_ALIGNED8(p.N));
     auto epi_half = [&](auto hc) {
         constexpr int h = decltype(hc)::value;
         if constexpr (((MT == 4 && WM == 2) || (MT == 2 && WM == 4)) && WN == 2 && A_KC && B_KC) if (p.act == 7) {
@@ -914,16 +914,21 @@
                 }
             }
             const int rbase = row_base(h) + (lane >> 3);
-            auto res_row = [&](int it) -> bf16x8 {
+            const int crpb_ = p.cmap.rpb;
+            const int64_t cdel_ = crpb_ != 0 ? p.cmap.bs - crpb_ : 0, coff_ = crpb_ != 0 ? p.cmap.off : 0;
+            auto map_q = [&](int it) -> int { return crpb_ != 0 ? (rbase + it * 8) / crpb_ : 0; };
+            auto map_row = [&](int it, int q) -> int64_t { return (int64_t)(rbase + it * 8) + q * cdel_ + coff_; };
+            auto res_row = [&](int it, int64_t orow) -> bf16x8 {
                 const int row = rbase + it * 8;
-                return (has_res && row < M_ && col_ok) ? *reinterpret_cast<const bf16x8*>(res_ + rz + (int64_t)row * ldr_ + ccol) : bf16x8{};
+                return (has_res && row < M_ && col_ok) ? *reinterpret_cast<const bf16x8*>(res_ + rz + orow * ldr_ + ccol) : bf16x8{};
             };
             const bool accum = p.accumulate != 0;
-            auto old_row = [&](int it) -> bf16x8 {
+            auto old_row = [&](int it, int64_t orow) -> bf16x8 {
                 const int row = rbase + it * 8;
-                return (accum && row < M_ && col_ok) ? *reinterpret_cast<const bf16x8*>(cl + (int64_t)row * ldl) : bf16x8{};
+                return (accum && row < M_ && col_ok) ? *reinterpret_cast<const bf16x8*>(cl + orow * ldl) : bf16x8{};
             };
-            bf16x8 rnext = res_row(0), onext = old_row(0);
+            int qnext = map_q(0);
+            bf16x8 rnext = res_row(0, map_row(0, qnext)), onext = old_row(0, map_row(0, qnext));
 #pragma unroll
             for (int i = 0; i < 4; ++i)
 #pragma unroll
@@ -939,9 +944,12 @@
                 const f32x4 v0 = *reinterpret_cast<const f32x4*>(sp);
                 const f32x4 v1 = *reinterpret_cast<const f32x4*>(sp + 4);
                 const bf16x8 rv = rnext, ov0 = onext;
+                const int64_t orow = map_row(it, qnext);
                 if (it + 1 < 8) {
-                    rnext = res_row(it + 1);
-                    onext = old_row(it + 1);
+                    qnext = map_q(it + 1);
+                    const int64_t mnext = map_row(it + 1, qnext);
+                    rnext = res_row(it + 1, mnext);
+                    onext = old_row(it + 1, mnext);
                 }
                 if (row >= M_ || !col_ok) continue;
                 float v[8] = {v0[0], v0[1], v0[2], v0[3], v1[0], v1[1], v1[2], v1[3]};
@@ -956,7 +964,7 @@
                         bf16x8 pv;
 #pragma unroll
                         for (int e = 0; e < 8; ++e) pv[e] = f2bf(v[e]);
-                        store_pre8(pre_ + cz + (int64_t)row * ldc_ + ccol, pv, nt_pre_);
+                        store_pre8(pre_ + cz + orow * ldc_ + ccol, pv, nt_pre_);
                     }
 #pragma unroll
                     for (int e = 0; e < 8; e += 2) {
@@ -976,7 +984,7 @@
                 bf16x8 ov;
 #pragma unroll
                 for (int e = 0; e < 8; ++e) ov[e] = f2bf(v[e]);
-                store_pre8(cl + (int64_t)row * ldl, ov, nt_c_);
+                store_pre8(cl + orow * ldl, ov, nt_c_);
             }
             asm volatile("s_waitcnt lgkmcnt(0)" ::: "memory");
             __builtin_amdgcn_wave_barrier();
@@ -1226,8 +1234,7 @@
         const bool col_ok = ccol < ((p.N + 7) & ~7);
         const bool fused_fast = p.act >= 2 && p.act <= 5 && p.bias == nullptr && p.gate == nullptr && p.residual == nullptr && !p.accumulate &&
                                 !p.out_f32 && p.nseg == 0 && (p.act == 4 || p.scale == 1.0f) && (p.act != 3 || p.pre_out != nullptr);
-        const bool simple_fast = p.simple_epi && p.act <= 1 && p.split_k == 1 && p.gate == nullptr && !p.out_f32 && p.scale == 1.0f && p.cmap.rpb == 0 &&
-                                 (N_ALIGNED8(p.N));
+        const bool simple_fast = p.simple_epi && p.act <= 1 && p.split_k == 1 && p.gate == nullptr && !p.out_f32 && p.scale == 1.0f && (N_ALIGNED8(p.N));
         auto to_slab = [&](int ti) {
             __builtin_amdgcn_wave_barrier();
 #pragma unroll
@@ -1375,16 +1382,21 @@
                 }
             }
             const int rbase = m0c + wm * 128 + (lane >> 3);
-            auto res_row = [&](int k) -> bf16x8 {
+            const int crpb_ = p.cmap.rpb;
+            const int64_t cdel_ = crpb_ != 0 ? p.cmap.bs - crpb_ : 0, coff_ = crpb_ != 0 ? p.cmap.off : 0;
+            auto map_q = [&](int k) -> int { return crpb_ != 0 ? (rbase + k * 8) / crpb_ : 0; };
+            auto map_row = [&](int k, int q) -> int64_t { return (int64_t)(rbase + k * 8) + q * cdel_ + coff_; };
+            auto res_row = [&](int k, int64_t orow) -> bf16x8 {
                 const int row = rbase + k * 8;
-                return (has_res && row < M_ && col_ok) ? *reinterpret_cast<const bf16x8*>(res_ + (int64_t)row * ldr_ + ccol) : bf16x8{};
+                return (has_res && row < M_ && col_ok) ? *reinterpret_cast<const bf16x8*>(res_ + orow * ldr_ + ccol) : bf16x8{};
             };
             const bool accum = p.accumulate != 0;
-            auto old_row = [&](int k) -> bf16x8 {
+            auto old_row = [&](int k, int64_t orow) -> bf16x8 {
                 const int row = rbase + k * 8;
-                return (accum && row < M_ && col_ok) ? *reinterpret_cast<const bf16x8*>(cl + (int64_t)row * ldl) : bf16x8{};
+                return (accum && row < M_ && col_ok) ? *reinterpret_cast<const bf16x8*>(cl + orow * ldl) : bf16x8{};
             };
-            bf16x8 rnext = res_row(0), onext = old_row(0);
+            int qnext = map_q(0);
+            bf16x8 rnext = res_row(0, map_row(0, qnext)), onext = old_row(0, map_row(0, qnext));
 #pragma unroll
             for (int ti = 0; ti < MT; ++ti) {
                 to_slab(ti);
@@ -1395,9 +1407,12 @@
                     const float* sp = slab + (it2 * 8 + (lane >> 3)) * 64 + (lane & 7) * 8;
                     const f32x4 v0 = *reinterpret_cast<const f32x4*>(sp), v1 = *reinterpret_cast<const f32x4*>(sp + 4);
                     const bf16x8 rv = rnext, ov0 = onext;
+                    const int64_t orow = map_row(k, qnext);
                     if (k + 1 < 2 * MT) {
-                        rnext = res_row(k + 1);
-                        onext = old_row(k + 1);
+                        qnext = map_q(k + 1);
+                        const int64_t mnext = map_row(k + 1, qnext);
+                        rnext = res_row(k + 1, mnext);
+                        onext = old_row(k + 1, mnext);
                     }
                     if (row >= M_ || !col_ok) continue;
                     float v[8] = {v0[0], v0[1], v0[2], v0[3], v1[0], v1[1], v1[2], v1[3]};
@@ -1412,7 +1427,7 @@
                             bf16x8 pv;
 #pragma unroll
                             for (int e = 0; e < 8; ++e) pv[e] = f2bf(v[e]);
-                            store_pre8(pre_ + (int64_t)row * ldc_ + ccol, pv, nt_pre_);
+                            store_pre8(pre_ + orow * ldc_ + ccol, pv, nt_pre_);
                         }
 #pragma unroll
                         for (int e = 0; e < 8; e += 2) {
@@ -1432,7 +1447,7 @@
                     bf16x8 ov;
 #pragma unroll
                     for (int e = 0; e < 8; ++e) ov[e] = f2bf(v[e]);
-                    store_pre8(cl + (int64_t)row * ldl, ov, nt_c_);
+                    store_pre8(cl + orow * ldl, ov, nt_c_);
                 }
             }
         } else {
diff --git a/kai0_amd/model.py b/kai0_amd/model.py
--- a/kai0_amd/model.py
+++ b/kai0_amd/model.py
@@ -235,6 +235,7 @@
 
 _EXPERT_STREAM = os.environ.get("KAI0_EXPERT_STREAM", "1") != "0"
 _SKIP_DEAD_PREFIX = True
+_SKIP_DEAD_QUERIES = True
 
 
 def set_expert_stream(on: bool) -> bool:
@@ -246,6 +247,12 @@
 def set_skip_dead_prefix(on: bool) -> bool:
     global _SKIP_DEAD_PREFIX
     old, _SKIP_DEAD_PREFIX = _SKIP_DEAD_PREFIX, bool(on)
+    return old
+
+
+def set_skip_dead_queries(on: bool) -> bool:
+    global _SKIP_DEAD_QUERIES
+    old, _SKIP_DEAD_QUERIES = _SKIP_DEAD_QUERIES, bool(on)
     return old
 
 
@@ -360,11 +367,17 @@
                 xs, hs, gate1 = ops.adarms_res(xs, mod1, Hs, le.input_layernorm.eps)
                 qkv_s = ops.linear_multi(hs, [ae.q_proj.weight, ae.k_proj.weight, ae.v_proj.weight])
             xp, hp = ops.rmsnorm_res(xp, lp.input_layernorm.weight, lp.input_layernorm.eps)
-            qkv_p = ops.linear_multi(hp, [ap.q_proj.weight, ap.k_proj.weight, ap.v_proj.weight])
+            dead_q = last and _SKIP_DEAD_PREFIX and _SKIP_DEAD_QUERIES and ops.joint_attention_recomputes(P + Hs)
+            if dead_q:
+                kv_p = ops.linear_multi(hp, [ap.k_proj.weight, ap.v_proj.weight], wgrad_as=ap.q_proj.weight.shape[0])
+                qkv_p = (None, *kv_p)
+            else:
+                qkv_p = ops.linear_multi(hp, [ap.q_proj.weight, ap.k_proj.weight, ap.v_proj.weight])
             if dual:
                 main.wait_stream(side)
                 hand(qkv_s, main)
-            att_p, att_s = ops.joint_attention(pos, qcode, kcode, inv_freq, H, HD, (P, Hs), (*qkv_p, *qkv_s))
+            att_p, att_s = ops.joint_attention(pos, qcode, kcode, inv_freq, H, HD, (P, Hs), (*qkv_p, *qkv_s), in_place=None,
+                                               q_seg0=1 if dead_q else 0)
             if dual:
                 side.wait_stream(main)
                 hand((att_s,), side)
diff --git a/kai0_amd/ops.py b/kai0_amd/ops.py
--- a/kai0_amd/ops.py
+++ b/kai0_amd/ops.py
@@ -309,14 +309,15 @@
     return _WGRAD_SPLIT.get((M, N, K)) or max(1, min(6, 256 // t256, K // 2048))
 
 
-def linear_fwd(x, w, bias=None, residual=None, act=0, want_pre=False, gate=None, gate_rpb=0, out=None):
-    M, K = x.shape
+def linear_fwd(x, w, bias=None, residual=None, act=0, want_pre=False, gate=None, gate_rpb=0, out=None, a_map=None):
+    K = x.shape[-1]
+    M = x.numel() // K
     N = w.shape[0]
     if out is None:
         out = torch.empty((M, N), dtype=BF16, device=x.device)
     pre = torch.empty((M, N), dtype=BF16, device=x.device) if want_pre else None
     gemm(x, w, out, M=M, N=N, K=K, lda=K, ldb=K, ldc=N, bias=bias, act=act, pre_out=pre, residual=residual, ldr=N,
-         gate=gate, gate_rpb=gate_rpb, gate_ld=N, split_k=pick_split_k(M, N, K))
+         gate=gate, gate_rpb=gate_rpb, gate_ld=N, split_k=pick_split_k(M, N, K), a_map=a_map)
     return (out, pre) if want_pre else out
 
 
@@ -385,6 +386,7 @@
 
 def reset_backward_state() -> None:
     _DEFERRED.clear()
+    _JOINT_GRADS.clear()
     for idx in list(_JOIN_PENDING):
         if _JOIN_PENDING[idx]:
             _JOIN_PENDING[idx] = False
@@ -467,10 +469,12 @@
 
     @staticmethod
     def forward(ctx, x, w, bias, residual, act: int):
-        _chk(x, BF16, "linear.x")
+        rmap = _rows_map(x, "linear.x") if x.dim() == 3 else None
+        if rmap is None:
+            _chk(x, BF16, "linear.x")
         _chk(w, BF16, "linear.w")
         need_pre = act == 1 and (x.requires_grad or w.requires_grad)
-        r = linear_fwd(x, w, bias, residual, act, want_pre=need_pre)
+        r = linear_fwd(x, w, bias, residual, act, want_pre=need_pre, a_map=rmap)
         out, pre = r if need_pre else (r, None)
         ctx.save_for_backward(x, w, pre)
         ctx.bias = bias
@@ -478,13 +482,16 @@
         ctx.bias_dtype = bias.dtype if bias is not None else None
         ctx.has_res = residual is not None
         ctx.act = act
+        ctx.rmap = rmap
         return out
 
     @staticmethod
     def backward(ctx, dout):
         x, w, pre = ctx.saved_tensors
         dout = dout.contiguous()
-        M, K = x.shape
+        rmap = ctx.rmap
+        K = x.shape[-1]
+        M = x.numel() // K
         N = w.shape[0]
         dres = dout if ctx.has_res else None
         dy = dout
@@ -493,19 +500,71 @@
             _lib.call("kai0_gelu_bwd", dout.data_ptr(), pre.data_ptr(), dy.data_ptr(), dout.numel(), _stream())
         dx = dw = db = None
         if ctx.needs_input_grad[0]:
-            dx = torch.empty((M, K), dtype=BF16, device=x.device)
+            dx, cmap = (torch.empty((M, K), dtype=BF16, device=x.device), None) if rmap is None else _joint_grad_rows(x, rmap)
             if M >= 4096 and N % 8 == 0 and K % 8 == 0:
                 wt = transpose(w)
-                gemm(dy, wt, dx, M=M, N=K, K=N, a_kc=True, b_kc=True, lda=N, ldb=N, ldc=K)
+                gemm(dy, wt, dx, M=M, N=K, K=N, a_kc=True, b_kc=True, lda=N, ldb=N, ldc=K, c_map=cmap)
                 del wt
             else:
-                gemm(dy, w, dx, M=M, N=K, K=N, a_kc=True, b_kc=False, lda=N, ldb=K, ldc=K, split_k=pick_split_k(M, K, N))
+                gemm(dy, w, dx, M=M, N=K, K=N, a_kc=True, b_kc=False, lda=N, ldb=K, ldc=K, split_k=pick_split_k(M, K, N), c_map=cmap)
         if ctx.needs_input_grad[1]:
             dw = _grad_dst(w, BF16)
-            gemm(dy, x, dw, M=N, N=K, K=M, a_kc=False, b_kc=False, lda=N, ldb=K, ldc=K, split_k=pick_split_k_wgrad(N, K, M), nt_out=True)
+            gemm(dy, x, dw, M=N, N=K, K=M, a_kc=False, b_kc=False, lda=N, ldb=K, ldc=K, split_k=pick_split_k_wgrad(N, K, M), nt_out=True,
+                 b_map=rmap)
         if ctx.has_bias and ctx.needs_input_grad[2]:
             (db,) = _bias_grads(dy, M, N, N, [(ctx.bias, 0, N)])
         return dx, _grad_ret(w, dw), db, dres, None
+
+
+def _rows_map(x, name: str):
+    if not x.is_cuda:
+        raise _lib.Kai0HipError(f"{name}: expected a CUDA (HIP) tensor; the product path has no CPU fallback")
+    if x.dtype != BF16:
+        raise TypeError(f"{name}: expected {BF16}, got {x.dtype}")
+    Bn, L, K = x.shape
+    sb, sr, sc = x.stride()
+    if sc != 1 or sr != K or sb % K != 0 or sb < L * K or x.data_ptr() % 16 != 0:
+        raise ValueError(f"{name}: a 3-D input must be a row range [Bn, L, K] of a [Bn, S_ld, K] buffer (strides {x.stride()})")
+    return (L, sb // K, 0)
+
+
+_JOINT_GRADS: dict = {}
+
+
+def _joint_grad_rows(x, rmap):
+    st = x.untyped_storage()
+    n = st.nbytes() // x.element_size()
+    cur = torch.cuda.current_stream(x.device)
+    ent = _JOINT_GRADS.get(st.data_ptr())
+    if ent is None or ent[0].numel() != n or ent[0].device != x.device:
+        buf = torch.empty(n, dtype=x.dtype, device=x.device)
+        ev = torch.cuda.Event()
+        ev.record(cur)
+        ent = _JOINT_GRADS[st.data_ptr()] = (buf, cur, ev, set())
+    if x.storage_offset() in ent[3]:
+        return torch.empty(x.shape, dtype=x.dtype, device=x.device), None
+    ent[3].add(x.storage_offset())
+    if ent[1] != cur:
+        cur.wait_event(ent[2])
+        ent[0].record_stream(cur)
+    return ent[0].as_strided(x.shape, x.stride(), x.storage_offset()), rmap
+
+
+def _joint_rows(ts, seg_lens, S_ld: int, W: int, first: int = 0):
+    r0 = sum(seg_lens[:first])
+    t0 = ts[first]
+    if t0 is None or t0.dim() != 3:
+        return None
+    Bn = t0.shape[0]
+    base = t0.storage_offset() - r0 * W
+    for t, L in zip(ts[first:], seg_lens[first:]):
+        if (t is None or t.dtype != t0.dtype or t.dim() != 3 or tuple(t.shape) != (Bn, L, W) or t.stride() != (S_ld * W, W, 1)
+                or t.untyped_storage().data_ptr() != t0.untyped_storage().data_ptr() or t.storage_offset() != base + r0 * W):
+            return None
+        r0 += L
+    if base < 0 or t0.untyped_storage().nbytes() < (base + Bn * S_ld * W) * t0.element_size():
+        return None
+    return t0.as_strided((Bn, S_ld, W), (S_ld * W, W, 1), base)
 
 
 def transpose(x: torch.Tensor) -> torch.Tensor:
@@ -549,7 +608,8 @@
 class LinearMultiFn(torch.autograd.Function):
 
     @staticmethod
-    def forward(ctx, x, n: int, *wb):
+    def forward(ctx, x, n: int, wgrad_as: int, *wb):
+        ctx.wgrad_as = wgrad_as
         _chk(x, BF16, "linear_multi.x")
         ws, bs = wb[:n], wb[n:]
         widths = tuple(int(w.shape[0]) for w in ws)
@@ -604,23 +664,23 @@
             else:
                 gemm(dy, wcat, dx, M=M, N=K, K=Nt, a_kc=True, b_kc=False, lda=Nt, ldb=K, ldc=K)
         dws, dbs = [None] * n, [None] * n
-        if any(ctx.needs_input_grad[2 + i] for i in range(n)):
+        if any(ctx.needs_input_grad[3 + i] for i in range(n)):
             dsts = [_grad_dst(w, BF16) for w in ws]
             dwcat = _as_rows(dsts)
             tmp = dwcat is None
             if tmp:
                 dwcat = torch.empty((Nt, K), dtype=BF16, device=dev)
-            gemm(dy, x, dwcat, M=Nt, N=K, K=M, a_kc=False, b_kc=False, lda=Nt, ldb=K, ldc=K, split_k=pick_split_k_wgrad(Nt, K, M))
+            gemm(dy, x, dwcat, M=Nt, N=K, K=M, a_kc=False, b_kc=False, lda=Nt, ldb=K, ldc=K, split_k=pick_split_k_wgrad(Nt + ctx.wgrad_as, K, M))
             r = 0
             for i, (w, dst) in enumerate(zip(ws, dsts)):
                 if tmp:
                     dst.copy_(dwcat[r : r + widths[i]])
                 r += widths[i]
                 dws[i] = _grad_ret(w, dst)
-        if bs[0] is not None and any(ctx.needs_input_grad[2 + n + i] for i in range(n)):
+        if bs[0] is not None and any(ctx.needs_input_grad[3 + n + i] for i in range(n)):
             offs = [sum(widths[:i]) for i in range(n)]
             dbs = _bias_grads(dy, M, Nt, Nt, [(b, offs[i], widths[i]) for i, b in enumerate(bs)])
-        return (dx, None, *dws, *dbs)
+        return (dx, None, None, *dws, *dbs)
 
     @staticmethod
     def _backward_separate(ctx, x, ws, douts):
@@ -643,15 +703,15 @@
                 else:
                     gemm(dy, w, dx, M=M, N=K, K=N, a_kc=True, b_kc=False, lda=N, ldb=K, ldc=K, accumulate=not first)
                 first = False
-            if ctx.needs_input_grad[2 + i]:
+            if ctx.needs_input_grad[3 + i]:
                 dw = _grad_dst(w, BF16)
                 gemm(dy, x, dw, M=N, N=K, K=M, a_kc=False, b_kc=False, lda=N, ldb=K, ldc=K, split_k=pick_split_k_wgrad(N, K, M), nt_out=True)
                 dws[i] = _grad_ret(w, dw)
-            if b is not None and ctx.needs_input_grad[2 + n + i]:
+            if b is not None and ctx.needs_input_grad[3 + n + i]:
                 (dbs[i],) = _bias_grads(dy, M, N, N, [(b, 0, N)])
         if dx is not None and first:
             dx.zero_()
-        return (dx, None, *dws, *dbs)
+        return (dx, None, None, *dws, *dbs)
 
 
 def _as_rows(ts):
@@ -665,10 +725,10 @@
     return t0.as_strided((sum(t.shape[0] for t in ts), *t0.shape[1:]), t0.stride(), t0.storage_offset())
 
 
-def linear_multi(x, weights, biases=None):
+def linear_multi(x, weights, biases=None, wgrad_as: int = 0):
     n = len(weights)
     biases = list(biases) if biases is not None else [None] * n
-    return LinearMultiFn.apply(x, n, *weights, *biases)
+    return LinearMultiFn.apply(x, n, int(wgrad_as), *weights, *biases)
 
 
 class LinearF32Fn(torch.autograd.Function):
@@ -1280,32 +1340,51 @@
 
 
 def _joint_attention_grads(cfg, pos, inv_freq, dq_all, dk_all, dv_all):
-    Bn, S, S_ld, H, HD, seg_lens, scale, recompute = cfg
+    Bn, S, S_ld, H, HD, seg_lens, scale, recompute, q_seg0 = cfg
     dev = dq_all.device
     grads, parts = [], []
     r0 = 0
-    for Li in seg_lens:
-        W3 = (H + 2) * HD
-        dq, dk, dv = fused_columns(Bn * Li, (H * HD, HD, HD), dev)
-        parts.append((dq_all, r0 * H * HD, dq, 0, (S_ld * H * HD, H * HD), (Li * W3, W3), Bn, Li, H * HD, 2, r0))
+    for i, Li in enumerate(seg_lens):
+        if i < q_seg0:
+            W3 = 2 * HD
+            dq = None
+            dk, dv = fused_columns(Bn * Li, (HD, HD), dev)
+        else:
+            W3 = (H + 2) * HD
+            dq, dk, dv = fused_columns(Bn * Li, (H * HD, HD, HD), dev)
+            parts.append((dq_all, r0 * H * HD, dq, 0, (S_ld * H * HD, H * HD), (Li * W3, W3), Bn, Li, H * HD, 2, r0))
         parts.append((dk_all, r0 * HD, dk, 0, (dk_all.stride(0), HD), (Li * W3, W3), Bn, Li, HD, 2, r0))
         parts.append((dv_all, r0 * HD, dv, 0, (dv_all.stride(0), HD), (Li * W3, W3), Bn, Li, HD, 0, 0))
         grads += [dq, dk, dv]
         r0 += Li
     pack_rows(parts, HD, pos, S, inv_freq)
-    return (None, None, None, None, None, None, None, *grads)
+    return (None, None, None, None, None, None, None, None, None, *grads)
+
+
+_JOINT_IN_PLACE = True
+
+
+def set_joint_in_place(on: bool) -> bool:
+    global _JOINT_IN_PLACE
+    old, _JOINT_IN_PLACE = _JOINT_IN_PLACE, bool(on)
+    return old
+
+
+def joint_attention_recomputes(S: int) -> bool:
+    return not _ATTN_STORE_P and S <= 2048
 
 
 class JointAttentionFn(torch.autograd.Function):
 
     @staticmethod
-    def forward(ctx, pos, qcode, kcode, inv_freq, H: int, HD: int, seg_lens: tuple, *qkv):
+    def forward(ctx, pos, qcode, kcode, inv_freq, H: int, HD: int, seg_lens: tuple, in_place: bool, q_seg0: int, *qkv):
         nseg = len(seg_lens)
         qs, ks, vs = qkv[0::3], qkv[1::3], qkv[2::3]
-        dev = qs[0].device
+        dev = ks[0].device
         S = sum(seg_lens)
-        Bn = qs[0].shape[0] // seg_lens[0]
+        Bn = ks[0].shape[0] // seg_lens[0]
         S_ld = round_up(S, 8)
+        rq0 = sum(seg_lens[:q_seg0])
         q_all = torch.empty((Bn, S_ld, H * HD), dtype=BF16, device=dev)
         k_all = torch.empty((Bn, S_ld, HD), dtype=BF16, device=dev)
         v_all = torch.empty((Bn, S_ld, HD), dtype=BF16, device=dev)
@@ -1313,7 +1392,8 @@
         r0 = 0
         for i in range(nseg):
             Li = seg_lens[i]
-            parts.append((qs[i], 0, q_all, r0 * H * HD, (Li * qs[i].stride(0), qs[i].stride(0)), (S_ld * H * HD, H * HD), Bn, Li, H * HD, 1, r0))
+            if i >= q_seg0:
+                parts.append((qs[i], 0, q_all, r0 * H * HD, (Li * qs[i].stride(0), qs[i].stride(0)), (S_ld * H * HD, H * HD), Bn, Li, H * HD, 1, r0))
             parts.append((ks[i], 0, k_all, r0 * HD, (Li * ks[i].stride(0), ks[i].stride(0)), (S_ld * HD, HD), Bn, Li, HD, 1, r0))
             parts.append((vs[i], 0, v_all, r0 * HD, (Li * vs[i].stride(0), vs[i].stride(0)), (S_ld * HD, HD), Bn, Li, HD, 0, 0))
             r0 += Li
@@ -1323,45 +1403,70 @@
             parts.append((None, 0, v_all, S * HD, (0, 0), (S_ld * HD, HD), Bn, S_ld - S, HD, 3, 0))
         pack_rows(parts, HD, pos, S, inv_freq)
         scale = HD**-0.5
-        recompute = not _ATTN_STORE_P and S <= 2048
-        att, probs = mqa_attention_fwd(q_all, k_all, v_all, qcode, kcode, Bn, S, 0, S, S_ld, H, HD, scale, want_lse=recompute)
+        recompute = joint_attention_recomputes(S)
+        if q_seg0 and not recompute:
+            raise ValueError("joint_attention: a query window (q_seg0 > 0) needs the recompute form (joint_attention_recomputes)")
+        att, probs = mqa_attention_fwd(q_all, k_all, v_all, qcode, kcode, Bn, S - rq0, rq0, S, S_ld, H, HD, scale, want_lse=recompute)
         outs, parts = [], []
         r0 = 0
         for i in range(nseg):
             Li = seg_lens[i]
-            o = torch.empty((Bn * Li, H * HD), dtype=BF16, device=dev)
-            parts.append((att, r0 * H * HD, o, 0, (S_ld * H * HD, H * HD), (Li * H * HD, H * HD), Bn, Li, H * HD, 0, 0))
-            outs.append(o)
+            if i < q_seg0:
+                outs.append(None)
+            elif in_place:
+                outs.append(att[:, r0 : r0 + Li])
+            else:
+                o = torch.empty((Bn * Li, H * HD), dtype=BF16, device=dev)
+                parts.append((att, r0 * H * HD, o, 0, (S_ld * H * HD, H * HD), (Li * H * HD, H * HD), Bn, Li, H * HD, 0, 0))
+                outs.append(o)
             r0 += Li
-        pack_rows(parts, HD)
+        if parts:
+            pack_rows(parts, HD)
         ctx.save_for_backward(q_all, k_all, v_all, probs, pos, inv_freq, att, qcode, kcode)
-        ctx.cfg = (Bn, S, S_ld, H, HD, seg_lens, scale, recompute)
+        ctx.cfg = (Bn, S, S_ld, H, HD, seg_lens, scale, recompute, q_seg0)
         return tuple(outs)
 
     @staticmethod
     def backward(ctx, *douts):
         q_all, k_all, v_all, probs, pos, inv_freq, att, qcode, kcode = ctx.saved_tensors
-        Bn, S, S_ld, H, HD, seg_lens, scale, recompute = ctx.cfg
+        Bn, S, S_ld, H, HD, seg_lens, scale, recompute, q_seg0 = ctx.cfg
         dev = q_all.device
-        M = S * H
+        rq0 = sum(seg_lens[:q_seg0])
+        M = (S - rq0) * H
+        q_off = rq0 * H * HD
         dq_all = torch.empty((Bn, S_ld, H * HD), dtype=BF16, device=dev)
         if recompute:
             pd = torch.empty((2, Bn, M, S_ld), dtype=BF16, device=dev)
             lse, probs, dscores = probs, pd[0], pd[1]
-        datt = torch.empty((Bn, S_ld, H * HD), dtype=BF16, device=dev)
+        shared = _JOINT_GRADS.pop(att.untyped_storage().data_ptr(), None)
+        datt = _joint_rows(douts, seg_lens, S_ld, H * HD, q_seg0)
         parts = []
-        r0 = 0
-        for i, Li in enumerate(seg_lens):
-            parts.append((douts[i].contiguous(), 0, datt, r0 * H * HD, (Li * H * HD, H * HD), (S_ld * H * HD, H * HD), Bn, Li, H * HD, 0, 0))
-            r0 += Li
+        if datt is not None:
+            if shared is not None and shared[1] != torch.cuda.current_stream(dev):
+                shared[0].record_stream(torch.cuda.current_stream(dev))
+        else:
+            datt = torch.empty((Bn, S_ld, H * HD), dtype=BF16, device=dev)
+            r0 = rq0
+            for i, Li in enumerate(seg_lens):
+                if i < q_seg0:
+                    continue
+                g = douts[i]
+                if g.dim() == 3 and g.stride(2) == 1 and g.stride(1) == H * HD:
+                    sst = (g.stride(0), H * HD)
+                else:
+                    g, sst = g.contiguous(), (Li * H * HD, H * HD)
+                parts.append((g, 0, datt, r0 * H * HD, sst, (S_ld * H * HD, H * HD), Bn, Li, H * HD, 0, 0))
+                r0 += Li
+        del shared
         if S_ld > S:
             parts.append((None, 0, datt, S * H * HD, (0, 0), (S_ld * H * HD, H * HD), Bn, S_ld - S, H * HD, 3, 0))
-        pack_rows(parts, HD)
+        if parts:
+            pack_rows(parts, HD)
         if recompute:
             d = AttnBwdDesc()
-            d.dO, d.O, d.Q, d.K, d.V = datt.data_ptr(), att.data_ptr(), q_all.data_ptr(), k_all.data_ptr(), v_all.data_ptr()
-            d.lse, d.qcode, d.kcode = lse.data_ptr(), _p(qcode), _p(kcode)
-            d.P, d.dS, d.dQ = probs.data_ptr(), dscores.data_ptr(), dq_all.data_ptr()
+            d.dO, d.O, d.Q, d.K, d.V = datt.data_ptr() + 2 * q_off, att.data_ptr() + 2 * q_off, q_all.data_ptr() + 2 * q_off, k_all.data_ptr(), v_all.data_ptr()
+            d.lse, d.qcode, d.kcode = lse.data_ptr(), (None if qcode is None else qcode.data_ptr() + 4 * rq0), _p(kcode)
+            d.P, d.dS, d.dQ = probs.data_ptr(), dscores.data_ptr(), dq_all.data_ptr() + 2 * q_off
             d.batch, d.rows, d.Sk, d.HD, d.H = Bn, M, S, HD, H
             d.ldo, d.ldk, d.ldv, d.ldp = HD, HD, HD, S_ld
             d.sO, d.sK, d.sV, d.sP, d.s_lse = S_ld * H * HD, S_ld * HD, S_ld * HD, M * S_ld, lse.stride(0)
@@ -1373,7 +1478,7 @@
             dkv = torch.empty((2, Bn, S_ld, HD), dtype=BF16, device=dev)
             gemm(pd, datt, dkv, M=S_ld, N=HD, K=M, a_kc=False, b_kc=False, lda=S_ld, ldb=HD, ldc=HD, batch=2 * Bn, batch_inner=Bn,
                  sA=(Bn * M * S_ld, M * S_ld), sB=((q_all.data_ptr() - datt.data_ptr()) // 2, S_ld * H * HD),
-                 sC=(Bn * S_ld * HD, S_ld * HD), split_k=_attn_bwd_split(2 * Bn, S_ld, HD, M))
+                 sC=(Bn * S_ld * HD, S_ld * HD), split_k=_attn_bwd_split(2 * Bn, S_ld, HD, M), b_off_elems=q_off)
             dv_all, dk_all = dkv[0], dkv[1]
             return _joint_attention_grads(ctx.cfg, pos, inv_freq, dq_all, dk_all, dv_all)
         kv_split = _attn_bwd_split(Bn, S_ld, HD, M)
@@ -1391,8 +1496,10 @@
         return _joint_attention_grads(ctx.cfg, pos, inv_freq, dq_all, dk_all, dv_all)
 
 
-def joint_attention(pos, qcode, kcode, inv_freq, H, HD, seg_lens, qkv):
-    return JointAttentionFn.apply(pos, qcode, kcode, inv_freq, H, HD, tuple(seg_lens), *qkv)
+def joint_attention(pos, qcode, kcode, inv_freq, H, HD, seg_lens, qkv, in_place=False, q_seg0: int = 0):
+    if in_place is None:
+        in_place = _JOINT_IN_PLACE
+    return JointAttentionFn.apply(pos, qcode, kcode, inv_freq, H, HD, tuple(seg_lens), bool(in_place), int(q_seg0), *qkv)
 
 
 _SIGLIP_BWD_FUSED = True
```
